# coralogix/arrow-ballista

Measured on AMD Instinct MI355X. Metric: tpch_sf100_q3_lineitem_rows_per_sec, higher is better.
Workload: dtype i128; 1 GPU; TPC-H SF100 q3 (BASELINE configs[2]): filter x3 + hash join customer|x|orders + hash join |x| lineitem + aggregate + sort, one task on 1 x MI355X; lineitem_rows=600037902, lineitem_rows_per_gpu=600037902, orders_rows_per_gpu=150009476, customer_rows_per_gpu=15000000, input=Arrow-physical columns resident in HBM, parallelism=single partition

## Files before the change

### arrow-ballista_amd/csrc/agg_compile.cpp

```cpp
#include "agg_compile.h"
#include <algorithm>
#include <cctype>
#include <cstdio>
#include <functional>

namespace gpuq {

gpuq_field_info make_field(const std::string& name, const DType& t, bool nullable) {
  gpuq_field_info f{};
  std::snprintf(f.name, sizeof(f.name), "%s", name.c_str());
  f.type = t.id; f.precision = t.p; f.scale = t.s; f.nullable = nullable;
  f.repr = (t.id == T_UTF8) ? GPUQ_REPR_PACKED15 : GPUQ_REPR_ARROW;
  f.width = (t.id == T_BOOL) ? 0 : type_width(t);
  return f;
}

KeySpec make_keyspec(const std::vector<int>& regs, const std::vector<DType>& types, bool null_word) {
  if (regs.size() > (size_t)MAX_KEYS) throw Unsupported("more than " + std::to_string(MAX_KEYS) + " key columns");
  KeySpec K{};
  K.n_keys = (int)regs.size(); K.null_word = null_word ? 1 : 0;
  int w = 0;
  for (size_t k = 0; k < regs.size(); ++k) {
    K.key_reg[k] = regs[k];
    const bool wide = types[k].id == T_DECIMAL128 || types[k].id == T_UTF8;
// ... 325 lines not shown
  {{"AVG"},                                     parts<Avg>(),         1,    false,  false,     false},
  {{"MIN"},                                     parts<MinMax>(),      1,    true,   false,     false},
  {{"MAX"},                                     parts<MinMax>(),      1,    false,  false,     false},
  {{"VARIANCE", "VAR", "VAR_SAMP"},             parts<Variance>(),    1,    false,  false,     false},
  {{"VARIANCE_POP", "VAR_POP"},                 parts<Variance>(),    1,    false,  true,      false},
  {{"STDDEV", "STDDEV_SAMP"},                   parts<Variance>(),    1,    false,  false,     true},
  {{"STDDEV_POP"},                              parts<Variance>(),    1,    false,  true,      true},
  {{"COVARIANCE", "COVAR", "COVAR_SAMP"},       parts<Covariance>(),  2,    false,  false,     false},
  {{"COVARIANCE_POP", "COVAR_POP"},             parts<Covariance>(),  2,    false,  true,      false},
  {{"CORRELATION", "CORR"},                     parts<Correlation>(), 2,    false,  false,     false},
};
const AggFn* find_agg_fn(const std::string& upper_name) {
  for (const AggFn& f : AGG_FNS) for (const char* n : f.names) if (upper_name == n) return &f;
  return nullptr;
}

}

AggCompiled compile_aggregate(const Schema& in, const Json& d) {
  AggCompiled R;
  R.mode = d.get_str("mode", "Single");
  const bool is_final = (R.mode == "Final" || R.mode == "FinalPartitioned");
  const bool emit_state = (R.mode == "Partial");
  if (!is_final && !emit_state && R.mode != "Single") throw std::runtime_error("unknown aggregate mode '" + R.mode + "'");
  R.strategy = d.get_str("strategy", "auto");
  R.expected_groups = d.get_i64("expected_groups", 0);
  Scan s(in);
  ExprCompiler& ec = s.ec;
  if (d.has("predicate")) ec.add_predicate(ec.from_json(d.at("predicate")));
  std::vector<NodeP> declared; std::vector<std::string> declared_names;
  if (d.has("group_expr")) for (const Json& g : d.at("group_expr").a) {
    declared.push_back(ec.from_json(g.at("expr"))); declared_names.push_back(g.get_str("name", "group" + std::to_string(declared.size() - 1)));
  }
  const GroupKeys keys(ec, declared, declared_names);
  R.refuse = keys.refuse;
  s.ungrouped = keys.nodes.empty();
  States states{ec, keys.declared(), in.fields.size()};
  std::vector<AggPlan> plans;
  for (const Json& a : d.at("aggr_expr").a) {
    s.fn = a.at("fn").str(); s.desc = &a;
    AggPlan pl; pl.name = a.get_str("name", s.fn);
    for (auto& ch : s.fn) ch = (char)std::toupper(ch);
    if (a.get_bool("distinct", false)) throw Unsupported("DISTINCT aggregates are not supported on device");
    pl.fn = find_agg_fn(s.fn);
    if (!is_final) {
      NodeP arg = a.has("expr") ? ec.from_json(a.at("expr")) : nullptr;
      if (a.has("filter") && !a.at("filter").is_null()) {
        NodeP p = ec.from_json(a.at("filter"));
        if (p->type.id != T_BOOL) throw std::runtime_error("aggregate FILTER must be boolean");
        if (!arg) arg = ec.lit_int(I64, 1);
        arg = ec.select(p, arg, ec.lit_null(arg->type));
        if (a.has("expr2")) throw Unsupported("FILTER on a two-argument aggregate");
      }
      if (!arg && !(pl.fn && pl.fn->args == 0)) throw std::runtime_error(s.fn + " needs an argument");
      if (!pl.fn) throw Unsupported("aggregate function " + s.fn);
      pl.fn->parts.from_args(s, pl, arg);
    } else {
      if (!pl.fn) throw Unsupported("aggregate function " + s.fn);
      pl.fn->parts.from_states(s, pl, states);
    }
    plans.push_back(pl);
  }
  std::vector<AccDef>& accs = s.accs;
  if (accs.empty()) s.count(nullptr);
  std::vector<int> key_slots, acc_slots(accs.size(), -1);
  for (auto& k : keys.nodes) key_slots.push_back(ec.add_output(k));
  for (size_t i = 0; i < accs.size(); ++i) if (accs[i].arg) acc_slots[i] = ec.add_output(accs[i].arg);
  R.prog = ec.finish();
  const int nk = (int)keys.nodes.size();
  R.agg.n_keys = nk; R.agg.n_accs = (int)accs.size();
  std::vector<int> kregs; bool any_null_key = false;
  for (int k = 0; k < nk; ++k) {
    const NodeP& n = keys.nodes[k];
    R.agg.key_reg[k] = R.prog.out_reg[key_slots[k]]; kregs.push_back(R.agg.key_reg[k]);
    R.key_types.push_back(n->type); any_null_key = any_null_key || n->nullable;
    if (n->type.id == T_BOOL || n->type.id == T_NULL) throw Unsupported("group-by key of type " + n->type.to_string());
  }
  for (size_t i = 0; i < accs.size(); ++i) {
    R.agg.acc_kind[i] = accs[i].kind; R.agg.acc_reg[i] = accs[i].arg ? R.prog.out_reg[acc_slots[i]] : 0;
    R.acc_types.push_back(accs[i].type);
    R.acc_bits.push_back(accs[i].arg ? R.prog.out_bits[acc_slots[i]] : 1);
  }
  R.keys = make_keyspec(kregs, R.key_types, any_null_key);

  for (int k = 0; k < nk; ++k) { Field f; f.name = keys.names[k]; f.type = keys.nodes[k]->type; f.nullable = keys.nodes[k]->nullable; f.raw128 = 1; R.post_schema.fields.push_back(f); }
  for (size_t i = 0; i < accs.size(); ++i) { Field f; f.name = "acc" + std::to_string(i); f.type = accs[i].type; f.nullable = false; f.raw128 = 1; R.post_schema.fields.push_back(f); }
  std::function<void(size_t, size_t, bool)> emit = [&](size_t lo, size_t hi, bool with_keys) {
    ExprCompiler pc(R.post_schema);
    std::vector<std::string> names; CompiledProgram cp;
    try {
      if (with_keys) keys.project(pc, names);
      Post p{pc, nk, accs, names};
      for (size_t pi = lo; pi < hi; ++pi) (emit_state ? plans[pi].fn->parts.states : plans[pi].fn->parts.value)(p, plans[pi]);
      cp = pc.finish();
    }
    catch (const Unsupported&) { throw; }
    catch (const std::runtime_error&) {
      if (hi - lo + (with_keys ? 1 : 0) <= 1) throw;
      if (with_keys && hi > lo) { emit(lo, lo, true); emit(lo, hi, false); }
      else { const size_t mid = lo + (hi - lo) / 2; emit(lo, mid, with_keys); emit(mid, hi, false); }
      return;
    }
    if (cp.out_reg.empty()) return;
    const int first_out = (int)R.out_fields.size();
    for (size_t i = 0; i < cp.out_type.size(); ++i) R.out_fields.push_back(make_field(names[i], cp.out_type[i], cp.out_nullable[i]));
    R.posts.push_back({std::move(cp), first_out});
  };
  emit(0, plans.size(), true);
  return R;
}

}
```

### arrow-ballista_amd/csrc/capi.cpp

```cpp
#include "../../include/gpuq.h"
#include "expr_compile.h"
#include "agg_compile.h"
#include "gpuq_kernels.h"
#include "jit_runtime.h"
#include "devbuf.h"
#include "gpuq_internal.h"
#include <hip/hip_runtime.h>
#include <algorithm>
#include <memory>
#include <mutex>
#include <cctype>
#include <cstdio>
#include <cstdlib>
#include <cstring>
#include <string>
#include <tuple>
#include <map>
#include <deque>
#include <functional>
#include <vector>

using namespace gpuq;

namespace {
// ... 316 lines not shown
      op->kind = K_SORT;
      ExprCompiler ec(op->in_schema);
      const auto& es = d.at("expr").a;
      if (es.empty() || es.size() > (size_t)MAX_SORT_KEYS) throw Unsupported("sort needs 1.." + std::to_string(MAX_SORT_KEYS) + " keys");
      std::vector<NodeP> ks;
      for (const Json& e : es) { NodeP n = ec.from_json(e.at("expr")); ks.push_back(n); ec.add_output(n); }
      op->prog = ec.finish(); upload_code(op->prog, op->code_dev);
      op->sort.n_keys = (int)ks.size();
      for (size_t k = 0; k < ks.size(); ++k) {
        const bool asc = es[k].get_bool("asc", true);
        op->sort.reg[k] = op->prog.out_reg[k]; op->sort.desc[k] = asc ? 0 : 1;
        op->sort.nulls_first[k] = es[k].get_bool("nulls_first", !asc) ? 1 : 0;
        op->sort.kind[k] = ks[k]->type.is_float() ? 1 : (ks[k]->type.id == T_UTF8 ? 2 : 0);
      }
      op->sort_key0 = ks[0]->type;
      op->fetch = d.get_i64("fetch", -1);
    } else if (kind == "partition") {
      op->kind = K_PARTITION;
      ExprCompiler ec(op->in_schema);
      std::vector<NodeP> ks;
      for (const Json& e : d.at("hash_expr").a) { NodeP n = ec.from_json(e); ks.push_back(n); ec.add_output(n); }
      if (ks.empty()) throw std::runtime_error("partition needs at least one hash expression");
      op->prog = ec.finish(); upload_code(op->prog, op->code_dev);
      std::vector<int> regs; for (size_t k = 0; k < ks.size(); ++k) { regs.push_back(op->prog.out_reg[k]); op->key_types.push_back(ks[k]->type); }
      op->keys = make_keyspec(regs, op->key_types, false);
      const i64 np = d.at("partition_count").i64();
      if (np < 1 || np > 65536) throw std::runtime_error("partition_count out of range (1..65536)");
      op->nparts = (uint32_t)np;
    } else throw std::runtime_error("unknown op '" + kind + "'");
}

int gpuq_op_create(gpuq_ctx* ctx, const char* json, gpuq_op** out) {
  gpuq_op* op = nullptr;
  int rc = guarded(ctx, [&]() {
    check_ctx(ctx);
    if (!json || !out) throw std::runtime_error("json/out is NULL");
    Json d = JsonParser(json).parse();
    op = new gpuq_op(); op->ctx = ctx;
    op->flags_dev.ensure(256); HIPCHECK(hipMemset(op->flags_dev.p, 0, 256));
    g_upload = true;
    compile_op(op, d);
    *out = op;
  });
  if (rc != GPUQ_OK) { delete op; if (out) *out = nullptr; }
  return rc;
}

static const char* op_name(int op) {
  static const char* n[] = {"NOP","IMM","MOV","ADD","SUB","MUL","MULW","NEG","DIV","MOD","EQ","NE","LT","LE","GT","GE","FADD","FSUB","FMUL","FDIV","FNEG","FSQRT",
    "FEQ","FNE","FLT","FLE","FGT","FGE","I2F","F2I","AND","OR","NOT","ISNULL","ISNOTNULL","SELECT","SHL","BOR","NULLIF0","COALESCE0"};
  return (op >= 0 && op < (int)(sizeof(n) / sizeof(n[0]))) ? n[op] : "?";
}
static std::string describe_program(const CompiledProgram& p, const Schema& sc) {
  std::string r = "{\"columns\":[";
  for (size_t i = 0; i < p.col_field.size(); ++i) { if (i) r += ","; r += "\"" + sc.fields[p.col_field[i]].name + "\""; }
  r += "],\"pred_reg\":" + std::to_string(p.pred_reg) + ",\"insns\":[";
  for (int i = 0; i < p.n_insns; ++i) {
    const DevInsn& in = p.code.insns[i];
    if (i) r += ",";
    r += std::string("\"") + op_name(in.op) + " r" + std::to_string(in.dst) + " r" + std::to_string(in.a) + " r" + std::to_string(in.b) + " #" + std::to_string(in.imm) + "\"";
  }
  r += "],\"out_reg\":[";
  for (size_t i = 0; i < p.out_reg.size(); ++i) { if (i) r += ","; r += std::to_string(p.out_reg[i]); }
  r += "],\"out_type\":[";
  for (size_t i = 0; i < p.out_type.size(); ++i) { if (i) r += ","; r += "\"" + p.out_type[i].to_string() + "\""; }
  return r + "]}";
}

int gpuq_compile_check(const char* json, char* buf, size_t cap) {
  gpuq_op* op = nullptr;
  int rc = guarded(nullptr, [&]() {
    if (!json) throw std::runtime_error("json is NULL");
    Json d = JsonParser(json).parse();
    op = new gpuq_op();
    g_upload = false;
    compile_op(op, d);
    g_upload = true;
    std::string r = "{\"program\":" + describe_program(op->prog, op->in_schema);
    if (op->kind == K_AGG) {
      r += ",\"post\":" + describe_program(op->posts.front().prog, op->post_schema) + ",\"post_programs\":" + std::to_string(op->posts.size()) + ",\"posts\":[";
      for (size_t i = 0; i < op->posts.size(); ++i) { if (i) r += ","; r += describe_program(op->posts[i].prog, op->post_schema); }
      r += "],\"acc_kinds\":[";
      for (int a = 0; a < op->agg.n_accs; ++a) { if (a) r += ","; r += std::to_string(op->agg.acc_kind[a]); }
      r += "]";
    }
    r += ",\"outputs\":[";
    for (size_t i = 0; i < op->out_fields.size(); ++i) {
      const gpuq_field_info& f = op->out_fields[i];
      if (i) r += ",";
      DType t; t.id = f.type; t.p = f.precision; t.s = f.scale;
      r += std::string("{\"name\":\"") + f.name + "\",\"type\":\"" + t.to_string() + "\",\"nullable\":" + (f.nullable ? "true" : "false") + "}";
    }
    r += "]}";
    if (buf && cap) { std::snprintf(buf, cap, "%s", r.c_str()); if (r.size() + 1 > cap) throw Capacity("describe buffer too small"); }
  });
  g_upload = true;
  delete op;
  return rc;
}
int gpuq_compile_jit_source(const char* json, int kernel_id, char* buf, size_t cap) {
  gpuq_op* op = nullptr;
  int rc = guarded(nullptr, [&]() {
    if (!json) throw std::runtime_error("json is NULL");
    Json d = JsonParser(json).parse();
    op = new gpuq_op();
    g_upload = false;
    compile_op(op, d);
    g_upload = true;
    std::string eval = op->prog.jit_src;
    if (kernel_id == GPUQ_SINK_AGG_TINY && op->kind == K_AGG) eval += agg_tiny_spec(op, (int)d.get_i64("jit_gmax", 4));
    const std::string src = jit_full_source(eval, kernel_id);
    if (src.size() + 1 > cap) throw Capacity("source needs " + std::to_string(src.size() + 1) + " bytes");
    std::memcpy(buf, src.c_str(), src.size() + 1);
  });
  g_upload = true;
  delete op;
  return rc;
}
void gpuq_op_free(gpuq_op* op) { delete op; }
int gpuq_op_num_outputs(gpuq_op* op) { return op ? (int)op->out_fields.size() : 0; }
int gpuq_op_output_field(gpuq_op* op, int i, gpuq_field_info* out) {
  if (!op || !out || i < 0 || i >= (int)op->out_fields.size()) return GPUQ_ERR_INVALID;
  *out = op->out_fields[i]; return GPUQ_OK;
}
int gpuq_op_check(gpuq_op* op, void* stream) {
  if (!op) return GPUQ_ERR_INVALID;
  return guarded(op->ctx, [&]() { check_ctx(op->ctx); const uint32_t f = read_flags(op, use_stream(stream)); if (f) { reset_flags(op, use_stream(stream)); raise_flags(f); } });
}
int gpuq_op_set_deferred(gpuq_op* op, int on) { if (!op) return GPUQ_ERR_INVALID; op->deferred = on != 0; op->defer_client = true; return GPUQ_OK; }
int gpuq_op_can_defer(gpuq_op* op) {
  if (!op) return 0;
  switch (op->kind) {
    case K_FILTER: case K_PROJECT: case K_JOIN_PROBE: return 1;
    case K_JOIN_BUILD: return op->learned.jb.valid ? 1 : 0;
    case K_AGG: return op->learned.ag.valid ? 1 : 0;
    case K_SORT: return op->learned.so.valid ? 1 : 0;
    default: return 0;
  }
}
int gpuq_ops_settle(gpuq_ctx* ctx, void* stream, gpuq_op* const* ops, int n_ops, const uint64_t* const* words, int n_words, uint64_t* words_out) {
  return guarded(ctx, [&]() {
    check_ctx(ctx);
    if (n_ops < 0 || n_words < 0 || (n_ops && !ops) || (n_words && (!words || !words_out))) throw std::runtime_error("settle: bad arguments");
    hipStream_t s = use_stream(stream);
    const int total = n_ops + n_words;
    struct Blocks { u64* host = nullptr; DevBuf dev; size_t cap = 0; };
    thread_local Blocks B;
    if ((size_t)total > B.cap) {
      if (B.host) (void)hipHostFree(B.host);
      B.cap = (size_t)std::max(total, 256); B.host = nullptr;
      HIPCHECK(hipHostMalloc((void**)&B.host, B.cap * 8, hipHostMallocDefault));
    }
    u64* dev = (u64*)B.dev.ensure(B.cap * 8);
    for (int base = 0; base < total; base += 64) {
      GatherWords g{}; g.n = std::min(64, total - base);
      for (int i = 0; i < g.n; ++i) { const int k = base + i; g.src[i] = k < n_ops ? (const u64*)ops[k]->flags_dev.p : (const u64*)words[k - n_ops]; if (!g.src[i]) throw std::runtime_error("settle: NULL word"); }
      launch_gather_words(s, g, dev + base);
    }
    HIPCHECK(hipGetLastError());
    if (total > 0) HIPCHECK(hipMemcpyAsync(B.host, dev, (size_t)total * 8, hipMemcpyDeviceToHost, s));
    HIPCHECK(hipStreamSynchronize(s));
    for (int i = 0; i < n_words; ++i) words_out[i] = B.host[n_ops + i];
    bool retry = false;
    for (int i = 0; i < n_ops; ++i) {
      const uint32_t f = (uint32_t)B.host[i];
      if (f) reset_flags(ops[i], s);
      static const bool trace = getenv("GPUQ_TRACE_DEFER") != nullptr;
      const uint32_t expected = ops[i]->learned.expect_flags;
      if (trace && (f & ~expected)) fprintf(stderr, "[gpuq] settle: operator %d of %d (kind %d) raised status 0x%x (expected 0x%x)\n", i, n_ops, (int)ops[i]->kind, f, expected);
      if (f & ~expected) { retry = true; ops[i]->learned.forget(); }
    }
    if (retry) throw Retry("an assumption of a deferred run did not hold");
  });
}
int gpuq_op_profile(gpuq_op* op, int enable, float* kernel_ms_out, int* launches_out) {
  if (!op) return GPUQ_ERR_INVALID;
  return guarded(op->ctx, [&]() {
    if (op->ev_pending) { float ms = 0; HIPCHECK(hipEventSynchronize(op->ev1)); HIPCHECK(hipEventElapsedTime(&ms, op->ev0, op->ev1)); op->kernel_ms += ms; op->ev_pending = false; }
    if (op->ev_total_pending) { float ms = 0; HIPCHECK(hipEventSynchronize(op->ev3)); HIPCHECK(hipEventElapsedTime(&ms, op->ev2, op->ev3)); op->total_ms += ms; op->ev_total_pending = false; }
    if (kernel_ms_out) *kernel_ms_out = op->kernel_ms;
    if (launches_out) *launches_out = op->launches;
    op->last_total_ms = op->total_ms;
    op->kernel_ms = 0; op->total_ms = 0; op->launches = 0; if (enable >= 0) op->profile = enable != 0;
  });
}
int gpuq_op_profile_total(gpuq_op* op, float* total_ms_out) {
  if (!op || !total_ms_out) return GPUQ_ERR_INVALID;
  *total_ms_out = op->last_total_ms;
  return GPUQ_OK;
}

int gpuq_filter_run(gpuq_op* op, void* stream, const gpuq_input* in, int payload_via, uint32_t* sel_out, uint64_t* count_out) {
  if (!op) return GPUQ_ERR_INVALID;
  return guarded(op->ctx, [&]() {
    check_ctx(op->ctx);
    if (op->kind != K_FILTER) throw std::runtime_error("not a filter operator");
    hipStream_t s = use_stream(stream);
    ProfTotal ptot(op, s);
    DevProgram P = bind_program(op->prog, op->in_schema, op->code_dev.as<DevCode>(), op->flags_dev.as<uint32_t>(), in);
    if (payload_via < 0 || payload_via > in->n_via) throw std::runtime_error("payload_via out of range");
    const i64 n = in->n_rows;
    if (n == 0) { if (count_out) HIPCHECK(hipMemsetAsync(count_out, 0, 8, s)); return; }
    const i64 nwords = (n + 63) >> 6;
    const i64 maxb = (i64)op->ctx->cus * 8;
    i64 wpb = (nwords + maxb - 1) / maxb; if (wpb < 16) wpb = 16;
    const int nblocks = (int)((nwords + wpb - 1) / wpb);
    u64* bitmap = (u64*)op->ws[0].ensure((size_t)nwords * 8);
    uint32_t* counts = (uint32_t*)op->ws[1].ensure((size_t)nblocks * 4 + 16);
    u64* total = count_out ? (u64*)count_out : (u64*)op->ws[2].ensure(8);
    { SinkJit jit(op, op->prog, GPUQ_SINK_FILTER_BITMAP, n); ProfScope ps(op, s); launch_filter_bitmap(s, jit.fn, P, n, bitmap, counts, nblocks, wpb); }
    launch_scan_block_counts(s, counts, nblocks, total);
    if (sel_out) launch_compact(s, bitmap, counts, nblocks, wpb, n, payload_via > 0 ? in->via[payload_via - 1] : nullptr, sel_out);
    HIPCHECK(hipGetLastError());
  });
}

int gpuq_project_run(gpuq_op* op, void* stream, const gpuq_input* in, gpuq_column* outs, int n_outs) {
  if (!op) return GPUQ_ERR_INVALID;
  return guarded(op->ctx, [&]() {
    check_ctx(op->ctx);
    if (op->kind != K_PROJECT) throw std::runtime_error("not a project operator");
    hipStream_t s = use_stream(stream);
    ProfTotal ptot(op, s);
    DevProgram P = bind_program(op->prog, op->in_schema, op->code_dev.as<DevCode>(), op->flags_dev.as<uint32_t>(), in);
    OutSpec O = make_outspec(op->prog, outs, n_outs, op->out_fields);
    for (int i = 0; i < n_outs; ++i) outs[i].length = in->n_rows;
    { SinkJit jit(op, op->prog, GPUQ_SINK_PROJECT, in->n_rows); ProfScope ps(op, s); launch_project(s, jit.fn, P, in->n_rows, O); }
    HIPCHECK(hipGetLastError());
    if (op->prog.checks_overflow && !op->deferred) { const uint32_t f = read_flags(op, s); if (f) { reset_flags(op, s); raise_flags(f); } }
  });
}

static u64 agg_slot_pct(const bool from_last_run) {
  static const long env = []() { const char* e = std::getenv("GPUQ_AGG_SLOT_PCT"); const long x = e ? std::atol(e) : 0; return (x >= 110 && x <= 800) ? x : 0; }();
  return env ? (u64)env : (from_last_run ? 130u : 200u);
}
static int aggregate_run_impl(gpuq_op* op, void* stream, const gpuq_input* in, gpuq_column* outs, int n_outs, int64_t cap, int64_t* n_groups_out, const uint64_t** ndev_out) {
  if (!op) return GPUQ_ERR_INVALID;
  if (ndev_out) *ndev_out = nullptr;
  return guarded(op->ctx, [&]() {
    check_ctx(op->ctx);
    if (op->kind != K_AGG) throw std::runtime_error("not an aggregate operator");
    if (!op->refuse.empty()) throw Unsupported(op->refuse);
    hipStream_t s = use_stream(stream);
    ProfTotal ptot(op, s);
    DevProgram P = bind_program(op->prog, op->in_schema, op->code_dev.as<DevCode>(), op->flags_dev.as<uint32_t>(), in);
    const i64 n = in->n_rows;
    const int nk = op->agg.n_keys, na = op->agg.n_accs, kstride = nk > 0 ? nk : 1;
    uint32_t ng = 0;
    AggOut raw{};
    auto alloc_raw = [&](i64 rcap) {
      raw.cap = (int32_t)rcap;
      raw.keys = (u64*)op->ws[0].ensure((size_t)rcap * kstride * 16);
      raw.key_nulls = (uint32_t*)op->ws[1].ensure((size_t)rcap * 4);
      raw.cells = (u64*)op->ws[2].ensure((size_t)rcap * na * 16);
      raw.n_groups = op->flags_dev.as<uint32_t>() + 2;
      HIPCHECK(hipMemsetAsync(raw.n_groups, 0, 8, s));
    };
    auto read_ng = [&]() { uint32_t v[3] = {0, 0, 0}; read_status(op, s, v, 3); return v[2]; };
    if (n_outs != (int)op->out_fields.size()) throw std::runtime_error("expected " + std::to_string(op->out_fields.size()) + " output columns, got " + std::to_string(n_outs));
    bool posted = false;
    auto run_post = [&](uint32_t rows, const uint32_t* rows_dev) {
      const size_t colbytes = (size_t)std::max<uint32_t>(rows, 1) * 16, vbytes = ((size_t)rows + 63) / 64 * 8 + 8;
      char* soa_mem = (char*)op->ws[6].ensure((size_t)(nk + na) * colbytes + (size_t)nk * vbytes);
      AggSoA soa{};
      std::vector<gpuq_column> pcols(nk + na);
      for (int k = 0; k < nk; ++k) {
        soa.key_col[k] = (ulonglong2*)(soa_mem + (size_t)k * colbytes);
        soa.key_valid[k] = (u64*)(soa_mem + (size_t)(nk + na) * colbytes + (size_t)k * vbytes);
        const DType& t = op->key_types[k];
        pcols[k] = gpuq_column{t.id, t.p, t.s, 0, soa.key_col[k], nullptr, op->post_schema.fields[k].nullable ? (const uint8_t*)soa.key_valid[k] : nullptr, (int64_t)rows};
      }
      for (int a = 0; a < na; ++a) {
        soa.acc_col[a] = (ulonglong2*)(soa_mem + (size_t)(nk + a) * colbytes);
        const DType& t = op->acc_types[a];
        pcols[nk + a] = gpuq_column{t.id, t.p, t.s, 0, soa.acc_col[a], nullptr, nullptr, (int64_t)rows};
      }
      launch_agg_emit(s, raw, nk, na, rows, soa, rows_dev);
      gpuq_input pin{}; pin.cols = pcols.data(); pin.n_cols = nk + na; pin.n_rows = rows; pin.n_via = 0;
      for (auto& pc : op->posts) {
        DevProgram PP = bind_program(pc.prog, op->post_schema, pc.code.as<DevCode>(), op->flags_dev.as<uint32_t>(), &pin);
        PP.n_dev = (const u64*)rows_dev;
        const int no = (int)pc.prog.out_reg.size();
        std::vector<gpuq_field_info> fi(op->out_fields.begin() + pc.first_out, op->out_fields.begin() + pc.first_out + no);
        OutSpec O = make_outspec(pc.prog, outs + pc.first_out, no, fi);
        { SinkJit jit(op, pc.prog, GPUQ_SINK_PROJECT, rows); launch_project(s, jit.fn, PP, rows, O); }
      }
    };
    auto launch_tiny = [&](const int gmax, const bool reset) {
      int nb = 0; const size_t wsb = agg_tiny_workspace_bytes(gmax, nk, na, &nb);
      void* wsp = op->ws[4].ensure(wsb);
      alloc_raw(64);
      if (reset) reset_flags(op, s);
      const std::string spec = agg_tiny_spec(op, gmax);
      { SinkJit jit(op, op->prog, GPUQ_SINK_AGG_TINY, n, spec); ProfScope ps(op, s); launch_agg_tiny(s, jit.fn, P, n, op->agg, gmax, wsp); }
      launch_agg_tiny_merge(s, P, n, op->agg, gmax, wsp, raw);
    };
    HashTable T{};
    T.key_words = op->keys.key_words; T.slot_words = 1 + T.key_words + 2 * na;
    auto launch_table = [&](const u64 est, const u64 slot_pct, const bool use_lds, const bool reset) {
      T.n_slots = next_pow2(est * slot_pct / 100);
      T.slots = (u64*)op->ws[5].ensure((size_t)T.n_slots * T.slot_words * 8);
      launch_ht_init(s, T, &op->agg);
      if (reset) reset_flags(op, s);
      if (use_lds) {
        int n_fsum = 0; for (int a = 0; a < na; ++a) n_fsum += op->agg.acc_kind[a] == ACC_FSUM;
        u64* fstage = nullptr;
        const size_t fbytes = (size_t)T.n_slots * (size_t)n_fsum * (size_t)agg_lds_grid(n) * 8;
        if (n_fsum > 0 && fbytes <= ((size_t)256 << 20)) { fstage = (u64*)op->ws[8].ensure(fbytes); HIPCHECK(hipMemsetAsync(fstage, 0, fbytes, s)); }
        SinkJit jit(op, op->prog, GPUQ_SINK_AGG_LDS, n); ProfScope ps(op, s); launch_agg_lds(s, jit.fn, P, n, op->keys, op->agg, T, fstage, n_fsum);
      }
      else { SinkJit jit(op, op->prog, GPUQ_SINK_AGG_HASH, n); ProfScope ps(op, s); launch_agg_hash(s, jit.fn, P, n, op->keys, op->agg, T); }
    };
    auto run_radix = [&](const std::string& strat, const i64 known_groups) -> bool {
      const int slot_words = 1 + op->keys.key_words + 2 * na;
      uint32_t capslots = 64; while ((size_t)capslots * 2 * slot_words * 8 <= 60 * 1024) capslots *= 2;
      if ((size_t)capslots * slot_words * 8 <= 60 * 1024 && n < (1ll << 31)) {
        const u64 est = op->expected_groups > 0 ? (u64)op->expected_groups : (known_groups > 0 ? (u64)known_groups + (u64)known_groups / 4 : (u64)n);
        const u64 per_bucket = std::max<u64>(1, (u64)capslots / 2);
        u64 nbk = next_pow2(std::max<u64>(1, (est + per_bucket - 1) / per_bucket)); if (nbk > (1ull << 24)) nbk = 1ull << 24;
        if (n >= (1ll << 20) && nbk < 2048) nbk = 2048;
        int bits = 0; while ((1ull << bits) < nbk) ++bits;
        DevBuf b_bid, b_bid2, b_ids, b_hist, b_look, b_bounds;
        u64* bid = (u64*)b_bid.ensure((size_t)n * 8); u64* bid2 = (u64*)b_bid2.ensure((size_t)n * 8);
        uint32_t* ids = (uint32_t*)b_ids.ensure((size_t)n * 4 + 16);
        u64* ghist = (u64*)b_hist.ensure((size_t)sort_max_passes() * 256 * 8);
        const size_t lwb = onesweep_ws_bytes(n);
        void* lws = b_look.ensure(lwb);
        uint32_t* bounds = (uint32_t*)b_bounds.ensure((size_t)(nbk + 2) * 4);
        reset_flags(op, s);
        { SinkJit jit(op, op->prog, GPUQ_SINK_AGG_BUCKET_ID, n); launch_agg_bucket_id(s, jit.fn, P, n, op->keys, nbk - 1, bid, nullptr); }
        const int npass = std::max(1, (bits + 7) / 8);
        launch_radix_ghist(s, bid, n, 32, npass, ghist);
        for (int p = 0; p < npass; ++p) {
          launch_onesweep_pass(s, bid, nullptr, n, 32 + 8 * p, ghist + (size_t)p * 256, lws, lwb, bid2, ids, p + 1 == npass ? 2 : 0);
          std::swap(bid, bid2);
        }
        launch_bucket_bounds(s, bid, n, nbk, bounds, 32);
        alloc_raw((i64)std::min<u64>((u64)std::max<i64>(n, 1), std::max<u64>(est + est / 4, 1ull << 20)));
        { SinkJit jit(op, op->prog, GPUQ_SINK_AGG_BUCKET, n); ProfScope ps(op, s); launch_agg_bucket(s, jit.fn, P, op->keys, op->agg, ids, bounds, (uint32_t)nbk, capslots, slot_words, raw); }
        HIPCHECK(hipGetLastError());
        uint32_t fw[4] = {0, 0, 0, 0};
        read_status(op, s, fw, 4);
        if (fw[0] & ~(FLAG_TABLE_FULL | FLAG_GROUP_OVERFLOW)) { reset_flags(op, s); raise_flags(fw[0] & ~(FLAG_TABLE_FULL | FLAG_GROUP_OVERFLOW)); }
        if (!(fw[0] & (FLAG_TABLE_FULL | FLAG_GROUP_OVERFLOW))) { ng = fw[2]; return true; }
        if (strat == "radix" && op->expected_groups > 0 && est < (u64)n) throw Capacity("radix aggregate: a bucket overflowed; raise expected_groups or use strategy hash/auto");
        reset_flags(op, s);
      } else if (strat == "radix") throw Unsupported("radix aggregate: the group state does not fit an LDS table");
      return false;
    };
    auto finish_on_device = [&]() {
      run_post((uint32_t)raw.cap, raw.n_groups);
      HIPCHECK(hipGetLastError());
      for (int i = 0; i < n_outs; ++i) outs[i].length = raw.cap;
      if (n_groups_out) *n_groups_out = raw.cap;
      *ndev_out = (const uint64_t*)raw.n_groups;
    };
    auto& L = op->learned;
    if (ndev_out && op->deferred && L.ag.valid) {
      if (L.ag.path == 1) {
        if (cap >= 64) { launch_tiny(L.ag.gmax, false); finish_on_device(); return; }
      } else if (L.ag.path == 2) {
        const u64 est = std::min<u64>(std::max<u64>(L.ag.est, 64), (u64)(L.ag.groups + L.ag.groups / 4 + 64));
        const i64 rcap = std::min<i64>(L.ag.groups + L.ag.groups / 4 + 1024, cap);
        if (rcap >= 1 && rcap <= 0x7FFFFFFFll) {
          launch_table(est, agg_slot_pct(true), L.ag.use_lds, false);
          alloc_raw(rcap);
          launch_agg_hash_extract(s, op->keys, op->agg, T, raw, op->flags_dev.as<uint32_t>());
          finish_on_device();
          return;
        }
      }
    }
    if (in->n_rows_dev) throw std::runtime_error("aggregate: a device-side row count needs a deferred operator with a completed synchronous run (gpuq_op_can_defer)");
    L.ag.valid = false;
    int path_done = 0, gmax_done = 0; u64 est_done = 0; bool lds_done = false;
    bool done = false;
    std::string strat = op->strategy;
    if (nk == 0) strat = "tiny";
    if (strat == "auto" && n <= 16384) strat = "hash";
    i64 known_groups = op->expected_groups > 0 ? op->expected_groups : L.ag.groups;
    bool many_groups = false;
    if (strat == "auto" && nk > 0 && known_groups < 0 && n >= (1ll << 20)) {
      const i64 nsample = 1ll << 20, stride = std::max<i64>(1, n / nsample);
      const u64 nbits = 1ull << 24;
      uint32_t* bm = (uint32_t*)op->ws[7].ensure(nbits / 8 + 64);
      unsigned long long* cnt = (unsigned long long*)((char*)bm + nbits / 8);
      HIPCHECK(hipMemsetAsync(bm, 0, nbits / 8 + 64, s));
      launch_key_sample(s, P, n, op->keys, stride, nsample, bm, nbits, cnt + 1);
      launch_popcount_bits(s, (const uint8_t*)bm, (i64)nbits, cnt);
      unsigned long long* pd = (unsigned long long*)op->pinned();
      unsigned long long host2[2] = {0, 0};
      unsigned long long* dst = pd ? pd : host2;
      HIPCHECK(hipMemcpyAsync(dst, cnt, 16, hipMemcpyDeviceToHost, s));
      HIPCHECK(hipStreamSynchronize(s));
      const i64 distinct = (i64)dst[0], passed = (i64)dst[1];
      if (passed >= 4096) {
        if (distinct * 4 <= passed) known_groups = std::max<i64>(1, distinct);
        else many_groups = true;
      }
    }
    if (strat == "auto" && nk > 0 && (many_groups || known_groups > (i64)agg_tiny_max_groups(na))) {
    } else if (strat == "auto" || strat == "tiny") {
      const int fit_big = agg_tiny_max_groups(na);
      if (fit_big < 1) { if (strat == "tiny") throw Unsupported("too many accumulators for the LDS aggregate"); }
      else {
        int fit_small = 0; for (int g = 1; g <= fit_big; ++g) { int nb; (void)nb; if ((size_t)g * na * 2048 + 4096 <= 64 * 1024) fit_small = g; }
        std::vector<int> tries;
        if (nk == 0) tries = {1};
        else { if (fit_small > 4) { tries.push_back(4); } if (fit_small >= 2) tries.push_back(fit_small); if (fit_big > fit_small) tries.push_back(fit_big); }
        if (nk > 0 && known_groups > 0) while (tries.size() > 1 && (i64)tries.front() < known_groups) tries.erase(tries.begin());
        for (int gmax : tries) {
          launch_tiny(gmax, true);
          HIPCHECK(hipGetLastError());
          const bool ahead = (i64)raw.cap <= cap;
          if (ahead) run_post((uint32_t)raw.cap, raw.n_groups);
          uint32_t fw[4] = {0, 0, 0, 0};
          read_status(op, s, fw, 4);
          const uint32_t f = fw[0];
          if (f & ~FLAG_GROUP_OVERFLOW) { reset_flags(op, s); raise_flags(f & ~FLAG_GROUP_OVERFLOW); }
          if (!(f & FLAG_GROUP_OVERFLOW)) { ng = fw[2]; done = true; posted = ahead; path_done = 1; gmax_done = gmax; break; }
        }
        if (!done && strat == "tiny") throw Capacity("more groups than the LDS aggregate holds; use strategy hash/auto");
      }
    }
    const bool remembered_hash = op->expected_groups <= 0 && L.ag.path == 2;
    if (!done && (strat == "radix" || (strat == "auto" && !remembered_hash && ((n >= (1ll << 22) && op->expected_groups >= (1ll << 20)) ||
                                                            (n >= (1ll << 20) && known_groups >= 4096))))) { done = run_radix(strat, known_groups); if (done) path_done = 3; }
    if (!done) {
      const i64 known = known_groups >= 0 ? (op->expected_groups > 0 ? known_groups : std::max<i64>(known_groups + known_groups / 4, 64)) : -1;
      u64 est = known > 0 ? (u64)std::min<i64>(known, std::max<i64>(n, 1)) : (u64)std::min<i64>(std::max<i64>(n, 1), 1ll << 24);
      if (est < 64) est = 64;
      const uint32_t lslots = agg_lds_slots(T);
      const bool use_lds = strat == "lds" || (strat == "auto" && lslots > 0 && n >= (1ll << 17) && known > 0 && known <= (i64)lslots * 4);
      if (strat == "lds" && !lslots) throw Unsupported("lds aggregate: the group state does not fit an LDS table");
      for (;;) {
        launch_table(est, agg_slot_pct(known_groups >= 0 && op->expected_groups <= 0 && est == (u64)known), use_lds, true);
        HIPCHECK(hipGetLastError());
        const uint32_t f = (n <= (1ll << 20) && est >= (u64)n) ? 0u : read_flags(op, s);
        if (f & FLAG_TABLE_FULL) { if (est >= (u64)std::max<i64>(n, 1024)) throw std::runtime_error("hash aggregate: table full at maximum size"); est = std::min<u64>(est * 4, (u64)std::max<i64>(n, 1024)); continue; }
        if (f) { reset_flags(op, s); raise_flags(f); }
        break;
      }
      path_done = 2; est_done = est; lds_done = use_lds;
      if (n <= (1ll << 20)) {
        alloc_raw(std::max<i64>(n, 1));
        launch_agg_hash_extract(s, op->keys, op->agg, T, raw, op->flags_dev.as<uint32_t>());
        HIPCHECK(hipGetLastError());
        const bool ahead = (i64)raw.cap <= cap;
        if (ahead) run_post((uint32_t)raw.cap, raw.n_groups);
        uint32_t fw[4] = {0, 0, 0, 0};
        read_status(op, s, fw, 4);
        if (fw[0]) { reset_flags(op, s); raise_flags(fw[0]); }
        ng = fw[2];
        posted = ahead;
      } else {
        bool done = false;
        if (L.ag.groups > 0) {
          alloc_raw(L.ag.groups + L.ag.groups / 4 + 1024);
          launch_agg_hash_extract(s, op->keys, op->agg, T, raw, op->flags_dev.as<uint32_t>());
          HIPCHECK(hipGetLastError());
          uint32_t fw[4] = {0, 0, 0, 0};
          read_status(op, s, fw, 4);
          ng = fw[2];
          if (fw[0] & ~FLAG_GROUP_OVERFLOW) { reset_flags(op, s); raise_flags(fw[0]); }
          done = !(fw[0] & FLAG_GROUP_OVERFLOW);
          if (!done) { reset_flags(op, s); HIPCHECK(hipMemsetAsync(raw.n_groups, 0, 4, s)); }
        } else {
          alloc_raw(1);
          raw.cap = 0;
          launch_agg_hash_extract(s, op->keys, op->agg, T, raw, op->flags_dev.as<uint32_t>());
          ng = read_ng();
          reset_flags(op, s);
        }
        if (!done) {
          alloc_raw(std::max<i64>(ng, 1));
          launch_agg_hash_extract(s, op->keys, op->agg, T, raw, op->flags_dev.as<uint32_t>());
          HIPCHECK(hipGetLastError());
          ng = read_ng();
        }
      }
    }
    L.ag = {path_done == 1 || path_done == 2, path_done, gmax_done, est_done, lds_done, (i64)ng};
    if (L.ag.valid) L.expect_flags = 0;
    if (n_groups_out) *n_groups_out = ng;
    if ((i64)ng > cap) throw Capacity("aggregate produced " + std::to_string(ng) + " groups, output capacity is " + std::to_string(cap));
    for (int i = 0; i < n_outs; ++i) outs[i].length = ng;
    if (!posted) {
      run_post(ng, nullptr);
      HIPCHECK(hipGetLastError());
      HIPCHECK(hipStreamSynchronize(s));
    }
  });
}

int gpuq_aggregate_run(gpuq_op* op, void* stream, const gpuq_input* in, gpuq_column* outs, int n_outs, int64_t cap, int64_t* n_groups_out) {
  return aggregate_run_impl(op, stream, in, outs, n_outs, cap, n_groups_out, nullptr);
}
int gpuq_aggregate_run_deferred(gpuq_op* op, void* stream, const gpuq_input* in, gpuq_column* outs, int n_outs, int64_t cap, int64_t* n_bound_out, const uint64_t** n_groups_dev_out) {
  if (!n_groups_dev_out) return GPUQ_ERR_INVALID;
  return aggregate_run_impl(op, stream, in, outs, n_outs, cap, n_bound_out, n_groups_dev_out);
}

namespace {
bool probe_keys_local(gpuq_op* op, hipStream_t s, const DevProgram& P, i64 n, const HashTable& T) {
  u64* c = (u64*)op->ws[7].ensure(32);
  HIPCHECK(hipMemsetAsync(c, 0, 16, s));
  const i64 nwords = (n + 63) >> 6;
  const i64 nsample = std::min<i64>(nwords, 4096);
  launch_join_locality(s, P, n, op->keys, T, nwords / nsample, nsample, c);
  HIPCHECK(hipGetLastError());
  u64 got[2] = {0, 0};
  HIPCHECK(hipMemcpyAsync(got, c, 16, hipMemcpyDeviceToHost, s));
  HIPCHECK(hipStreamSynchronize(s));
  return got[0] == 0 || got[1] * 2 >= got[0];
}
}
static int join_build_impl(gpuq_op* op, void* stream, const gpuq_input* in, int payload_via, int64_t build_rows_bound, gpuq_join_table* semi_table,
                           uint32_t* semi_hits_out, uint64_t* rows_out, gpuq_join_table** out) {
  if (!op) return GPUQ_ERR_INVALID;
  gpuq_join_table* t = nullptr;
  int rc = guarded(op->ctx, [&]() {
    check_ctx(op->ctx);
    if (op->kind != K_JOIN_BUILD) throw std::runtime_error("not a join_build operator");
    if (!out) throw std::runtime_error("out is NULL");
    hipStream_t s = use_stream(stream);
    ProfTotal ptot(op, s);
    SemiProbe semi{}; const SemiProbe* semi_p = nullptr;
    if (semi_table) {
      if (!op->has_semi) throw std::runtime_error("join build: the descriptor has no \"semi_on\" keys");
      if (semi_table->has_dups) throw std::runtime_error("join build: the semi table holds duplicate keys (a row could survive more than once)");
      if (op->semi_keys.n_keys != semi_table->keys.n_keys || op->semi_keys.key_words != semi_table->keys.key_words) throw std::runtime_error("semi keys do not match the semi table's keys (count / width)");
      for (int k = 0; k < op->semi_keys.n_keys; ++k) if (op->semi_keys.key_wide[k] != semi_table->keys.key_wide[k]) throw std::runtime_error("semi key " + std::to_string(k) + " width class differs from the table's key; cast one side");
      if (payload_via != 0) throw std::runtime_error("join build over a semi table: payload_via must be 0 (the build row is the position)");
      semi.T = semi_table->T; semi.K = op->semi_keys; semi.null_eq = semi_table->null_eq; semi.on = 1; semi.hit_out = semi_hits_out; semi.rows_out = (u64*)rows_out;
      semi_p = &semi;
    } else if (op->has_semi) throw std::runtime_error("join build: this operator was compiled with \"semi_on\" keys: call gpuq_join_build_run_semi");
    DevProgram P = bind_program(op->prog, op->in_schema, op->code_dev.as<DevCode>(), op->flags_dev.as<uint32_t>(), in);
    if (payload_via < 0 || payload_via > in->n_via) throw std::runtime_error("payload_via out of range");
    const i64 n = in->n_rows;
    if (build_rows_bound < n && payload_via == 0) build_rows_bound = n;
    if (build_rows_bound < 0 || build_rows_bound > 0xFFFFFFFEll) throw std::runtime_error("build_rows_bound out of range");
    t = new gpuq_join_table(); t->ctx = op->ctx; t->keys = op->keys; t->null_eq = op->null_eq; t->bound = build_rows_bound;
    t->T.key_words = op->keys.key_words; t->T.slot_words = 1 + t->T.key_words;
    static const bool spec_on = []() { const char* e = getenv("GPUQ_JOIN_SPECULATE"); return !(e && e[0] == '0'); }();
    const int dense_mode = op->ctx->join_dense; const i64 dense_ratio = op->ctx->join_dense_ratio;
    const bool narrow_key = dense_mode && n > 0 && op->keys.n_keys == 1 && !op->keys.key_wide[0] && !op->keys.null_word;
    auto semi_spec = [&](const HashTable& T2, const uint32_t* present_) -> std::string {
      if (!semi_p) return std::string();
      const KeySpec& A = op->semi_keys; const KeySpec& B = op->keys;
      const bool narrow = A.n_keys == 1 && A.key_words == 1 && !A.null_word && B.n_keys == 1 && B.key_words == 1 && !B.null_word;
      if (narrow && T2.dense && !present_ && payload_via == 0)
        return "#define GPUQ_JIT_SEMI 2\nconstexpr int JIT_KEY_REG0 = " + std::to_string(A.key_reg[0]) + ";\nconstexpr int JIT_KEY2_REG = " + std::to_string(B.key_reg[0]) + ";\n";
      return "#define GPUQ_JIT_SEMI 1\n";
    };
    auto attempt = [&](const int mode) -> bool {
    const bool guess = mode == 1, memo = mode == 2;
    auto& jb = op->learned.jb;
    bool dense = false, sparse_bits = false; i64 kmin = 0; u64 krange = 0;
    if (memo) { dense = jb.dense; sparse_bits = jb.sparse_bits; kmin = jb.kmin; krange = jb.krange; }
// ... 987 lines not shown
```

### arrow-ballista_amd/csrc/gpuq_kernels.h

```cpp
#pragma once
#include "gpuq_dev.h"
#ifndef GPUQ_JIT
#include <type_traits>
#include "devbuf.h"
#endif

namespace gpuq {

constexpr int MAX_OUTS = 16;
struct OutCol {
  void* data;
  u64* validity;
  int32_t reg;
  int32_t cls;
};
struct OutSpec { int32_t n_out; int32_t pad; OutCol cols[MAX_OUTS]; };

constexpr int MAX_ACCS = 12;
constexpr int MAX_KEYS = 4;
enum AccKind : int32_t { ACC_SUM = 0, ACC_COUNT = 1, ACC_COUNT_STAR = 2, ACC_MIN = 3, ACC_MAX = 4, ACC_FSUM = 5, ACC_FMIN = 6, ACC_FMAX = 7 };
struct AggSpec {
  int32_t n_keys, n_accs;
  int32_t key_reg[MAX_KEYS];
  int32_t acc_kind[MAX_ACCS];
  int32_t acc_reg[MAX_ACCS];
};

struct AggOut {
  u64* keys; uint32_t* key_nulls; u64* cells; uint32_t* n_groups; int32_t cap; int32_t pad;
};



constexpr int MAX_KW = 2 * MAX_KEYS + 1;
struct KeySpec {
  int32_t n_keys;
  int32_t key_reg[MAX_KEYS];
  int32_t key_wide[MAX_KEYS];
  int32_t null_word;
  int32_t key_words;
  int32_t word_reg[MAX_KW];
  int32_t word_half[MAX_KW];
};
struct HashTable {
  u64* slots;
  u64 n_slots;
  int32_t slot_words;
  int32_t key_words;
  uint32_t* dense;
  i64 dense_min;
  u64 dense_range;
  uint32_t* dense_bits;
};
struct SemiProbe { HashTable T; KeySpec K; int32_t null_eq; int32_t on; uint32_t* hit_out; u64* rows_out; };
enum JoinType : int32_t { JT_INNER = 0, JT_LEFT = 1, JT_RIGHT = 2, JT_FULL = 3, JT_LEFT_SEMI = 4, JT_LEFT_ANTI = 5, JT_RIGHT_SEMI = 6, JT_RIGHT_ANTI = 7 };


constexpr uint32_t NIL = 0xFFFFFFFFu;
__device__ __forceinline__ uint32_t tag_of(u64 h) { return (uint32_t)(h >> 32) | 2u; }

__device__ __forceinline__ u64 acc_identity(const int kind, const int half) {
  switch (kind) {
    case ACC_MIN: return half ? 0 : 0x7FFFFFFFFFFFFFFFull;
    case ACC_MAX: return half ? ~0ull : 0x8000000000000000ull;
    case ACC_FMIN: return half ? 0 : 0x7FF0000000000000ull;
    case ACC_FMAX: return half ? 0 : 0xFFF0000000000000ull;
    default: return 0;
  }
}
__device__ __forceinline__ u64 slot_word_identity(const AggSpec& A, const int w, const int cell0) {
  const int a = (w - cell0) >> 1;
  return (w >= cell0 && a < A.n_accs) ? acc_identity(A.acc_kind[a], (w - cell0) & 1) : 0;
}
__device__ __forceinline__ void lds_table_init(u64* slots, const uint32_t cap, const int slot_words, const int cell0, const AggSpec& A, const uint32_t nthreads) {
  for (uint32_t i = threadIdx.x; i < cap * (uint32_t)slot_words; i += nthreads) slots[i] = slot_word_identity(A, (int)(i % (uint32_t)slot_words), cell0);
}
__device__ __forceinline__ bool acc_operand(const AggSpec& A, const int a, GPUQ_REGS_CPARAM, u64& vlo, u64& vhi) {
  const int kind = A.acc_kind[a];
  vlo = 1; vhi = 0;
  if (kind == ACC_COUNT_STAR) return true;
  const int r = __builtin_amdgcn_readfirstlane(A.acc_reg[a]);
  if (kind != ACC_COUNT) { vlo = rlo[r]; vhi = rhi[r]; }
  return !((rnulls >> r) & 1);
}
__device__ __forceinline__ bool acc_wide_minmax(const int kind, const u64 vlo, const u64 vhi) {
  return (kind == ACC_MIN || kind == ACC_MAX) && (i64)vhi != ((i64)vlo >> 63);
}
__device__ __forceinline__ void acc_combine(const int kind, u64& lo, u64& hi, const u64 olo, const u64 ohi) {
  switch (kind) {
    case ACC_SUM: case ACC_COUNT: case ACC_COUNT_STAR: { const u64 s = lo + olo; hi = hi + ohi + (s < lo ? 1 : 0); lo = s; break; }
    case ACC_MIN: if ((i64)olo < (i64)lo) lo = olo; break;
    case ACC_MAX: if ((i64)olo > (i64)lo) lo = olo; break;
    case ACC_FSUM: lo = (u64)__double_as_longlong(__longlong_as_double((i64)lo) + __longlong_as_double((i64)olo)); break;
    case ACC_FMIN: if (f64_total_key(olo) < f64_total_key(lo)) lo = olo; break;
    case ACC_FMAX: if (f64_total_key(olo) > f64_total_key(lo)) lo = olo; break;
    default: break;
  }
}
template <int SCOPE>
__device__ __forceinline__ void acc_fold(u64* c, const int kind, const u64 vlo, const u64 vhi) {
  switch (kind) {
    case ACC_COUNT: case ACC_COUNT_STAR: if (vlo) __hip_atomic_fetch_add(c, vlo, __ATOMIC_RELAXED, SCOPE); break;
    case ACC_SUM: {
      if (!(vlo | vhi)) break;
      const u64 old = __hip_atomic_fetch_add(c, vlo, __ATOMIC_RELAXED, SCOPE);
      const u64 carry = (old + vlo < old) ? 1 : 0;
      if (vhi + carry) __hip_atomic_fetch_add(c + 1, vhi + carry, __ATOMIC_RELAXED, SCOPE);
      break;
    }
    case ACC_MIN: __hip_atomic_fetch_min((i64*)c, (i64)vlo, __ATOMIC_RELAXED, SCOPE); break;
    case ACC_MAX: __hip_atomic_fetch_max((i64*)c, (i64)vlo, __ATOMIC_RELAXED, SCOPE); break;
    case ACC_FSUM: unsafeAtomicAdd((double*)c, __longlong_as_double((i64)vlo)); break;
    case ACC_FMIN: case ACC_FMAX: {
      u64 cur = __hip_atomic_load(c, __ATOMIC_RELAXED, SCOPE);
      for (;;) {
        const bool better = (kind == ACC_FMIN) ? (f64_total_key(vlo) < f64_total_key(cur)) : (f64_total_key(vlo) > f64_total_key(cur));
        if (!better || __hip_atomic_compare_exchange_strong(c, &cur, vlo, __ATOMIC_RELAXED, __ATOMIC_RELAXED, SCOPE)) break;
      }
      break;
    }
    default: break;
  }
}
__device__ __forceinline__ u64 acc_result_hi(const int kind, const u64 lo, const u64 hi) {
  return (kind == ACC_MIN || kind == ACC_MAX) ? (u64)((i64)lo >> 63) : hi;
// ... 57 lines not shown
  int32_t n_keys;
  int32_t reg[MAX_SORT_KEYS];
  int32_t desc[MAX_SORT_KEYS];
  int32_t nulls_first[MAX_SORT_KEYS];
  int32_t kind[MAX_SORT_KEYS];
};
constexpr int SORT_MAX_PASSES = 16;
struct SortPack {
  u64 base_lo[MAX_SORT_KEYS], base_hi[MAX_SORT_KEYS];
  int32_t shift[MAX_SORT_KEYS];
  int32_t null_bit[MAX_SORT_KEYS];
  int32_t rshift[MAX_SORT_KEYS];
  int32_t vbits[MAX_SORT_KEYS];
  int32_t check;
  int32_t total_bits;
};

struct AggSoA {
  ulonglong2* key_col[MAX_KEYS]; u64* key_valid[MAX_KEYS];
  ulonglong2* acc_col[MAX_ACCS];
};



struct GatherWords { int32_t n; int32_t pad; const u64* src[64]; };

#define GPUQ_SINK_FILTER_BITMAP 1
#define GPUQ_SINK_PROJECT 2
#define GPUQ_SINK_AGG_TINY 3
#define GPUQ_SINK_AGG_HASH 4
#define GPUQ_SINK_JOIN_BUILD 5
#define GPUQ_SINK_JOIN_PROBE 6
#define GPUQ_SINK_JOIN_PROBE_UNIQUE 7
#define GPUQ_SINK_SORT_MINMAX 8
#define GPUQ_SINK_SORT_PACK 9
#define GPUQ_SINK_PART_PID 10
#define GPUQ_SINK_AGG_BUCKET_ID 11
#define GPUQ_SINK_AGG_BUCKET 12
#define GPUQ_SINK_AGG_LDS 13
#define GPUQ_SINK_JOIN_KEYRANGE 14
#define GPUQ_SINK_RJ_PACK 15

#ifndef GPUQ_JIT
struct SinkInfo { int id; const char* file; const char* entry; };
constexpr SinkInfo GPUQ_SINKS[] = {
    {GPUQ_SINK_FILTER_BITMAP, "kernels_scan.hip", "gpuq_jit_filter_bitmap"},
    {GPUQ_SINK_PROJECT, "kernels_scan.hip", "gpuq_jit_project"},
    {GPUQ_SINK_AGG_TINY, "kernels_scan.hip", "gpuq_jit_agg_tiny"},
    {GPUQ_SINK_AGG_HASH, "kernels_hash.hip", "gpuq_jit_agg_hash"},
    {GPUQ_SINK_JOIN_BUILD, "kernels_hash.hip", "gpuq_jit_join_build"},
    {GPUQ_SINK_JOIN_PROBE, "kernels_hash.hip", "gpuq_jit_join_probe"},
    {GPUQ_SINK_JOIN_PROBE_UNIQUE, "kernels_hash.hip", "gpuq_jit_join_probe_unique"},
    {GPUQ_SINK_SORT_MINMAX, "kernels_sort.hip", "gpuq_jit_sort_minmax"},
    {GPUQ_SINK_SORT_PACK, "kernels_sort.hip", "gpuq_jit_sort_pack"},
    {GPUQ_SINK_PART_PID, "kernels_sort.hip", "gpuq_jit_part_pid"},
    {GPUQ_SINK_AGG_BUCKET_ID, "kernels_hash.hip", "gpuq_jit_agg_bucket_id"},
    {GPUQ_SINK_AGG_BUCKET, "kernels_hash.hip", "gpuq_jit_agg_bucket"},
    {GPUQ_SINK_AGG_LDS, "kernels_hash.hip", "gpuq_jit_agg_lds"},
    {GPUQ_SINK_JOIN_KEYRANGE, "kernels_hash.hip", "gpuq_jit_join_keyrange"},
    {GPUQ_SINK_RJ_PACK, "kernels_hash.hip", "gpuq_jit_rj_pack"},
};
void launch_gather_words(hipStream_t s, const GatherWords& g, u64* out);
void set_num_cus(int n);
int num_cus();
void launch_filter_bitmap(hipStream_t s, void* jit_fn, const DevProgram& P, i64 n, u64* bitmap, uint32_t* block_counts, int nblocks, i64 words_per_block);
void launch_scan_block_counts(hipStream_t s, uint32_t* block_counts, int nblocks, u64* total_out);
void launch_compact(hipStream_t s, const u64* bitmap, const uint32_t* block_offsets, int nblocks, i64 words_per_block, i64 n,
                    const uint32_t* sel_in, uint32_t* sel_out);
void launch_project(hipStream_t s, void* jit_fn, const DevProgram& P, i64 n, const OutSpec& O);
int agg_tiny_max_groups(int n_accs);
size_t agg_tiny_workspace_bytes(int gmax, int n_keys, int n_accs, int* nblocks_out);
void launch_agg_tiny(hipStream_t s, void* jit_fn, const DevProgram& P, i64 n, const AggSpec& A, int gmax, void* workspace);
void launch_agg_tiny_merge(hipStream_t s, const DevProgram& P, i64 n, const AggSpec& A, int gmax, void* workspace, const AggOut& out);
void launch_ht_init(hipStream_t s, const HashTable& T, const AggSpec* A);
void launch_agg_hash(hipStream_t s, void* jit_fn, const DevProgram& P, i64 n, const KeySpec& K, const AggSpec& A, const HashTable& T);
void launch_key_sample(hipStream_t s, const DevProgram& P, i64 n, const KeySpec& K, i64 stride, i64 nsample, uint32_t* bitmap, u64 nbits, unsigned long long* passed);
uint32_t agg_lds_slots(const HashTable& T);
int agg_lds_grid(i64 n);
void launch_agg_lds(hipStream_t s, void* jit_fn, const DevProgram& P, i64 n, const KeySpec& K, const AggSpec& A, const HashTable& T, u64* fstage, int n_fsum);
void launch_agg_bucket_id(hipStream_t s, void* jit_fn, const DevProgram& P, i64 n, const KeySpec& K, u64 bucket_mask, u64* bid, uint32_t* ids);
void launch_bucket_bounds(hipStream_t s, const u64* sorted_bid, i64 n, u64 nbuckets, uint32_t* bounds, int shift);
void launch_agg_bucket(hipStream_t s, void* jit_fn, const DevProgram& P, const KeySpec& K, const AggSpec& A, const uint32_t* ids, const uint32_t* bounds, uint32_t nbuckets,
                       uint32_t cap, int slot_words, const AggOut& out);
void launch_agg_hash_extract(hipStream_t s, const KeySpec& K, const AggSpec& A, const HashTable& T, const AggOut& out, uint32_t* flags);
bool launch_join_build(hipStream_t s, void* jit_fn, const DevProgram& P, i64 n, const KeySpec& K, const HashTable& T, uint32_t* next, uint32_t* present,
                       int payload_via, int null_equals_null, const SemiProbe* semi = nullptr);
void launch_join_keyrange(hipStream_t s, void* jit_fn, const DevProgram& P, i64 n, const KeySpec& K, int null_equals_null, u64* out, i64 wstep = 1);
void launch_join_probe_unique(hipStream_t s, void* jit_fn, const DevProgram& P, i64 n, const KeySpec& K, const HashTable& T, int join_type, int null_equals_null, int payload_via,
                              uint32_t* seg_build, uint32_t* seg_probe, uint32_t* seg_counts, int nsegs, i64 wpw, uint32_t* visited);
void launch_copy_segments(hipStream_t s, const uint32_t* seg_build, const uint32_t* seg_probe, const uint32_t* seg_offsets, int nsegs, i64 wpw, i64 n,
                          const u64* total, uint32_t* out_build, uint32_t* out_probe, u64 out_cap, uint32_t* flags);
void launch_join_locality(hipStream_t s, const DevProgram& P, i64 n, const KeySpec& K, const HashTable& T, i64 stride, i64 nsample, u64* out);
struct RjGeomHost { uint32_t nparts, shift; i64 tile; int32_t nblocks; };
void rj_geometry(i64 n, u64 range, int slice_log2, RjGeomHost* g);
size_t rj_hist_entries(const RjGeomHost& g);
void launch_rj_partition(hipStream_t s, void* jit_fn, const DevProgram& P, i64 n, const KeySpec& K, const HashTable& T, int payload_via, const RjGeomHost& g,
                         u64* rec, u64* rec_out, int32_t* hist, void* scan_ws, size_t scan_ws_bytes);
int rj_probe_geometry(i64 n, i64* wpw_out);
void launch_rj_probe(hipStream_t s, const u64* rec, const int32_t* n_live, const HashTable& T, int join_type, uint32_t* seg_build, uint32_t* seg_probe,
                     uint32_t* seg_counts, int nblocks, i64 wpw);
void launch_bitmap_select(hipStream_t s, const u64* present, const u64* visited, int matched, i64 nwords, i64 n, u64* bitmap,
                          uint32_t* block_counts, int nblocks, i64 wpb);
void launch_join_probe(hipStream_t s, void* jit_fn, const DevProgram& P, i64 n, const KeySpec& K, const HashTable& T, const uint32_t* next,
                       int join_type, int payload_via, int null_equals_null, uint32_t* out_build, uint32_t* out_probe,
                       u64 out_cap, u64* out_count, uint32_t* visited);
int sort_minmax_blocks(i64 n);
void launch_sort_minmax(hipStream_t s, void* jit_fn, const DevProgram& P, i64 n, const SortSpec& S, u64* out, int nblocks, i64 wstep = 1);
int sort_max_passes();
void launch_sort_pack(hipStream_t s, void* jit_fn, const DevProgram& P, i64 n, const SortSpec& S, const SortPack& K, u64* key_lo, u64* key_hi, uint32_t* ids, u64* hist, int hist_passes);
void launch_part_pid(hipStream_t s, void* jit_fn, const DevProgram& P, i64 n, const KeySpec& K, uint32_t nparts, u64* pid_out, uint32_t* ids);
void launch_part_offsets(hipStream_t s, const u64* pid, i64 n, uint32_t nparts, uint32_t* counts_ws, u64* offsets_out, int shift);
void launch_counts_to_ghist(hipStream_t s, const uint32_t* counts, uint32_t np, u64* ghist);
void launch_gather_u64(hipStream_t s, const u64* src, const uint32_t* idx, i64 n, u64* dst);
int sort_small_max();
int sort_direct_max();
void launch_sort_direct(hipStream_t s, const DevProgram& P, i64 n, const SortSpec& S, uint32_t* perm);
void launch_sort_small(hipStream_t s, const u64* klo, const u64* khi, const uint32_t* ids, i64 n, uint32_t* out);
size_t onesweep_ws_bytes(i64 n);
int onesweep_max_passes();
size_t merge_splits_entries(i64 max_len, int n_pairs);
void launch_merge_pairs(hipStream_t s, const u64* klo, const u64* khi, const uint32_t* ids, const i64* pairs, int n_pairs, i64 max_len, i64* splits,
                        u64* klo_out, u64* khi_out, uint32_t* ids_out);
void launch_radix_ghist(hipStream_t s, const u64* keys, i64 n, int shift0, int npasses, u64* ghist);
void launch_onesweep_pass(hipStream_t s, const u64* keys, const uint32_t* vals, i64 n, int shift, u64* gexcl, void* ws, size_t ws_bytes,
                          u64* keys_out, uint32_t* vals_out, int ids_only );
void launch_agg_emit(hipStream_t s, const AggOut& raw, int n_keys, int n_accs, uint32_t n_groups, const AggSoA& soa, const uint32_t* n_groups_dev = nullptr);
void launch_concat_bitmap(hipStream_t s, u64* dst, i64 dst_bit_offset, const uint8_t* src, i64 src_bit_offset, i64 n_bits);
void launch_unpack_utf8_lengths(hipStream_t s, const ulonglong2* packed, i64 n, int32_t* lens_out, uint32_t* too_long);
constexpr int LIKE_MAX_TOKENS = 256;
constexpr int LIKE_MAX_SEGS = 8;
struct LikePattern {
  int32_t n; int32_t regex_mode; uint16_t tok[LIKE_MAX_TOKENS];
  int32_t n_seg, anchored_start, anchored_end, pad;
  int32_t seg_off[LIKE_MAX_SEGS], seg_len[LIKE_MAX_SEGS];
  unsigned long long seg_first8[LIKE_MAX_SEGS], seg_mask8[LIKE_MAX_SEGS];
};
void launch_like_utf8(hipStream_t s, const uint8_t* data, const int32_t* offsets, const uint8_t* validity, const uint32_t* idx, i64 n, const LikePattern& pat, int negated,
                      u64* bits_out, u64* valid_out);
void launch_mark_rows(hipStream_t s, const uint32_t* rows, i64 n, uint8_t* bitmap);
void launch_utf8_compare(hipStream_t s, const uint8_t* adata, const int32_t* aoffs, const uint8_t* avalid, const uint32_t* aidx, const uint8_t* bdata, const int32_t* boffs,
                         const uint8_t* bvalid, const uint32_t* bidx, int32_t blen, i64 n, int op, u64* bits_out, u64* valid_out);
void launch_sort_decode(hipStream_t s, const u64* recs, int rec_shift, i64 n, const SortPack& K, int desc, int nulls_first, int width, void* out, u64* valid_out);
void launch_cross_pairs(hipStream_t s, i64 n_left, i64 n_right, uint32_t* left_rows, uint32_t* right_rows);
void launch_offsets_rebase(hipStream_t s, const int32_t* src, i64 n, int32_t delta, int32_t* dst);
void launch_take_utf8_lengths(hipStream_t s, const int32_t* offsets, const uint8_t* validity, const uint32_t* idx, i64 n, int32_t* lens, u64* valid_out);
void launch_take_utf8_bytes(hipStream_t s, const uint8_t* data, const int32_t* offsets, const uint32_t* idx, i64 n, const int32_t* out_offsets, uint8_t* out, i64 total_bytes);
void launch_unpack_utf8_bytes(hipStream_t s, const ulonglong2* packed, i64 n, const int32_t* offsets, uint8_t* data_out);
void launch_exclusive_scan_i32(hipStream_t s, int32_t* data, i64 n, void* workspace, size_t ws_bytes);
size_t exclusive_scan_ws_bytes(i64 n);
struct Lz4Block { int64_t src; int64_t slot; int32_t len; int32_t pad; };
constexpr int LZ4_UNIT_BLOCK = 0, LZ4_UNIT_STORED = 1, LZ4_UNIT_FRAME_BLOCKS = 2;
constexpr int LZ4_UNIT_BLOCK_CHECKSUM = 1;
struct Lz4Unit { int64_t src, dst, src_len, dst_len; int32_t mode, flags; };
constexpr int64_t LZ4_BLOCK_BYTES = 65536;
inline int64_t lz4_slot_bytes(int64_t len) { return ((len + len / 255 + 16) + 15) & ~(int64_t)15; }
void launch_lz4_compress(hipStream_t s, const uint8_t* src, uint8_t* slots, const Lz4Block* blocks, int n_blocks, int32_t* csize);
void launch_lz4_layout(hipStream_t s, const Lz4Block* blocks, const int32_t* csize, const int32_t* buf_first_block, int n_buffers, int64_t* buf_off, int64_t* buf_len,
                       int64_t* blk_dst);
void launch_lz4_pack(hipStream_t s, const uint8_t* src, const uint8_t* slots, const Lz4Block* blocks, int n_blocks, const int32_t* csize, const int32_t* blk_buffer,
                     const int32_t* buf_first_block, const int64_t* buf_off, const int64_t* buf_len, const int64_t* blk_dst, uint8_t* body);
void launch_lz4_decode(hipStream_t s, const uint8_t* src, int64_t src_bytes, uint8_t* dst, const Lz4Unit* units, int n_units, uint32_t* status);
struct Utf8Piece { const int32_t* tmp; int64_t n; int32_t* dst; int64_t at, dl, start, used; int32_t first, pad; };
void launch_utf8_piece_starts(hipStream_t s, Utf8Piece* pieces, int n_pieces, uint32_t* gap);
void launch_utf8_piece_offsets(hipStream_t s, const Utf8Piece* pieces, int n_pieces, int64_t max_rows);
void launch_utf8_piece_validate(hipStream_t s, const Utf8Piece* pieces, int n_pieces, int64_t max_rows, uint32_t* status);
void launch_utf8_piece_compact(hipStream_t s, const Utf8Piece* pieces, int n_pieces, int64_t max_bytes, const uint8_t* from, uint8_t* to);
struct UnpackJob { int64_t src, dst, src_len, dst_len, raw_prefix; int32_t mode, pad; int64_t s_off, c_off, f_off, p_base; };
// ... 58 lines not shown
```

### arrow-ballista_amd/csrc/kernels_hash.hip

```cpp
#include "gpuq_kernels.h"

namespace gpuq {

constexpr int HBLOCK = 256;
constexpr int HWAVES = HBLOCK / 64;

__device__ __forceinline__ int hlane() { return threadIdx.x & 63; }
__device__ __forceinline__ int hwave() { return threadIdx.x >> 6; }

__device__ __forceinline__ u64 a_load(const u64* p) { return __hip_atomic_load(p, __ATOMIC_RELAXED, __HIP_MEMORY_SCOPE_AGENT); }
__device__ __forceinline__ void a_store(u64* p, u64 v) { __hip_atomic_store(p, v, __ATOMIC_RELAXED, __HIP_MEMORY_SCOPE_AGENT); }
__device__ __forceinline__ u64 a_cas(u64* p, u64 expected, u64 desired) {
  __hip_atomic_compare_exchange_strong(p, &expected, desired, __ATOMIC_RELAXED, __ATOMIC_RELAXED, __HIP_MEMORY_SCOPE_AGENT);
  return expected;
}
__device__ __forceinline__ u64 a_add(u64* p, u64 v) { return __hip_atomic_fetch_add(p, v, __ATOMIC_RELAXED, __HIP_MEMORY_SCOPE_AGENT); }

__device__ __forceinline__ bool make_key(const KeySpec& K, GPUQ_REGS_CPARAM, u64 (&kw)[MAX_KW], u64& hash) {
  uint32_t knull = 0;
  u64 h = 0x243F6A8885A308D3ull;
#pragma unroll
  for (int k = 0; k < MAX_KEYS; ++k) {
    if (k < K.n_keys) {
      const int r = __builtin_amdgcn_readfirstlane(K.key_reg[k]);
      const bool isn = (rnulls >> r) & 1;
      const u64 lo = isn ? 0 : rlo[r], hi = isn ? 0 : rhi[r];
      knull |= (uint32_t)isn << k;
      h = hash_combine(h, lo, K.key_wide[k] ? hi : 0, isn);
    }
  }
#pragma unroll
  for (int q = 0; q < MAX_KW; ++q) {
    kw[q] = 0;
    if (q < K.key_words) {
      const int half = __builtin_amdgcn_readfirstlane(K.word_half[q]);
      if (half == 2) kw[q] = knull;
      else {
        const int r = __builtin_amdgcn_readfirstlane(K.word_reg[q]);
        const bool isn = (rnulls >> r) & 1;
        const u64 vl = rlo[r], vh = rhi[r];
        const u64 v = (vl & ((u64)half - 1)) | (vh & (0 - (u64)half));
        kw[q] = isn ? 0 : v;
      }
    }
  }
  hash = h;
  return knull != 0;
}

__device__ __forceinline__ u64 ht_find_or_insert(const HashTable& T, const u64 (&kw)[MAX_KW], u64 h, uint32_t payload, bool& inserted) {
  const u64 mask = T.n_slots - 1;
  u64 s = h & mask;
  const uint32_t tag = tag_of(h);
  inserted = false;
  u64 probes = 0;
  while (probes < T.n_slots) {
    u64* slot = T.slots + s * (u64)T.slot_words;
    u64 w0 = a_load(slot);
    uint32_t st = (uint32_t)w0;
    if (st == 0u) {
      const u64 old = a_cas(slot, 0ull, 1ull);
      if (old == 0ull) {
#pragma unroll
        for (int q = 0; q < MAX_KW; ++q) if (q < T.key_words) a_store(slot + 1 + q, kw[q]);
        asm volatile("s_waitcnt vmcnt(0)" ::: "memory");
        a_store(slot, ((u64)payload << 32) | tag);
        inserted = true;
        return s;
      }
      st = (uint32_t)old;
    }
    if (st == 1u) { __builtin_amdgcn_s_sleep(1); continue; }
    if (st == tag) {
      bool eq = true;
#pragma unroll
      for (int q = 0; q < MAX_KW; ++q) if (q < T.key_words) eq = eq && (a_load(slot + 1 + q) == kw[q]);
      if (eq) return s;
    }
    s = (s + 1) & mask;
    ++probes;
  }
  return ~0ull;
}

__device__ __forceinline__ bool ht_find(const HashTable& T, const u64 (&kw)[MAX_KW], u64 h, uint32_t& payload) {
  const u64 mask = T.n_slots - 1;
  u64 s = h & mask;
  const uint32_t tag = tag_of(h);
  for (u64 probes = 0; probes < T.n_slots; ++probes) {
    const u64* slot = T.slots + s * (u64)T.slot_words;
    u64 w0, k0 = 0;
    if (T.slot_words == 2) { const ulonglong2 v = *(const ulonglong2*)slot; w0 = v.x; k0 = v.y; }
    else w0 = slot[0];
    const uint32_t st = (uint32_t)w0;
    if (st == 0u) return false;
    if (st == tag) {
      bool eq = true;
      if (T.slot_words == 2) eq = (k0 == kw[0]);
      else {
#pragma unroll
        for (int q = 0; q < MAX_KW; ++q) if (q < T.key_words) eq = eq && (slot[1 + q] == kw[q]);
      }
      if (eq) { payload = (uint32_t)(w0 >> 32); return true; }
    }
    s = (s + 1) & mask;
  }
  return false;
}

#ifndef GPUQ_JIT
__global__ void __launch_bounds__(HBLOCK) k_ht_init(const HashTable T, const AggSpec A, const int has_agg) {
  const u64 total = T.n_slots * (u64)T.slot_words;
  const int cell0 = 1 + T.key_words;
  for (u64 i = (u64)blockIdx.x * HBLOCK + threadIdx.x; i < total; i += (u64)gridDim.x * HBLOCK) {
    T.slots[i] = has_agg ? slot_word_identity(A, (int)(i % (u64)T.slot_words), cell0) : 0;
  }
}
#endif

#ifndef GPUQ_ROWS_U
#define GPUQ_ROWS_U 2
#endif
template <int MAXC, class Body>
__device__ __forceinline__ void for_rows_in_flight(const DevProgram& P, const i64 n, const i64 w_first, const i64 w_stride, Body body, const i64 w_end = -1) {
  const i64 nw_all = (n + 63) >> 6;
  const i64 nwords = (w_end >= 0 && w_end < nw_all) ? w_end : nw_all;
#ifdef GPUQ_JIT
  constexpr int U = GPUQ_ROWS_U;
  for (i64 w0 = w_first; w0 < nwords; w0 += w_stride * U) {
    JitPre jq[U]; JitRaw jw[U]; i64 posc[U]; bool ex[U];
#pragma unroll
    for (int u = 0; u < U; ++u) {
      const i64 w = w0 + (i64)u * w_stride;
      const i64 pos = (w << 6) + hlane();
      ex[u] = w < nwords && pos < n;
      posc[u] = ex[u] ? pos : n - 1;
      gpuq_jit_pre(P, posc[u], jq[u]);
    }
#pragma unroll
    for (int u = 0; u < U; ++u) gpuq_jit_load(P, posc[u], jq[u], jw[u]);
#pragma unroll
    for (int u = 0; u < U; ++u) {
      const i64 w = w0 + (i64)u * w_stride;
      if (w >= nwords) break;
      GPUQ_REGS_DECL;
      const bool pass = gpuq_jit_compute(P, posc[u], jw[u], GPUQ_REGS);
      body(w, (w << 6) + hlane(), ex[u] && pass, GPUQ_REGS);
    }
  }
#else
  for (i64 w = w_first; w < nwords; w += w_stride) {
    const i64 pos = (w << 6) + hlane();
    bool active = pos < n;
    GPUQ_REGS_DECL;
    if (active) active = GPUQ_EVAL(MAXC, P, pos);
    body(w, pos, active, GPUQ_REGS);
  }
#endif
}

template <int MAXC>
__device__ __forceinline__ void k_agg_hash_body(const DevProgram P, const i64 n_arg, const KeySpec K, const AggSpec A, const HashTable T) {
  const i64 n = rows_of(P, n_arg);
  const i64 nwords = (n + 63) >> 6;
  const int cell0 = 1 + T.key_words;
  bool combine = true;
  for (int a = 0; a < A.n_accs; ++a) combine = combine && A.acc_kind[a] != ACC_FMIN && A.acc_kind[a] != ACC_FMAX;
  const int lane = hlane();
  for_rows_in_flight<MAXC>(P, n, (i64)blockIdx.x * HWAVES + hwave(), (i64)gridDim.x * HWAVES, [&](const i64, const i64, const bool active, GPUQ_REGS_PARAM) {
    if (__ballot(active) == 0) return;
    u64 kw[MAX_KW]; u64 h = 0;
#pragma unroll
    for (int q = 0; q < MAX_KW; ++q) kw[q] = 0;
    if (active) make_key(K, GPUQ_REGS, kw, h);
    bool head = true;
    if (combine) {
      const int pa = __shfl_up((int)active, 1);
      const u64 ph = __shfl_up(h, 1);
      bool eq = (pa != 0) & (lane > 0) & (ph == h);
#pragma unroll
      for (int q = 0; q < MAX_KW; ++q) { const u64 pk = __shfl_up(kw[q], 1); if (q < T.key_words) eq = eq & (pk == kw[q]); }
      head = !(active & eq);
    }
    const int nh = __shfl_down((int)head, 1);
    const bool next_head = (lane == 63) | (nh != 0);
    const bool tail = active & next_head;
    u64 s = ~0ull;
    if (tail) {
      bool inserted;
      s = ht_find_or_insert(T, kw, h, 0u, inserted);
      if (s == ~0ull) atomicOr(P.flags, FLAG_TABLE_FULL);
    }
    u64* cells = T.slots + (s == ~0ull ? 0 : s) * (u64)T.slot_words + cell0;
    const bool upd = tail && s != ~0ull;
    for (int a = 0; a < A.n_accs; ++a) {
      const int kind = A.acc_kind[a];
      u64 vlo, vhi;
      bool any = acc_operand(A, a, GPUQ_REGS, vlo, vhi) && active;
      const bool wide = any && acc_wide_minmax(kind, vlo, vhi);
      if (__ballot(wide)) { if (wide) atomicOr(P.flags, FLAG_WIDE_MINMAX); continue; }
      if (!any) { vlo = acc_identity(kind, 0); vhi = acc_identity(kind, 1); }
      if (combine) {
        bool f = head;
#pragma unroll
        for (int off = 1; off < 64; off <<= 1) {
          const u64 ulo = __shfl_up(vlo, off), uhi = __shfl_up(vhi, off);
          const bool uf = __shfl_up((int)f, off) != 0, uany = __shfl_up((int)any, off) != 0;
          if (lane >= off && !f) {
            acc_combine(kind, vlo, vhi, ulo, uhi);
            any = any || uany;
            f = uf;
          }
        }
      }
      if (upd && any) acc_fold<__HIP_MEMORY_SCOPE_AGENT>(cells + 2 * a, kind, vlo, vhi);
    }
  });
}
#ifndef GPUQ_JIT
template <int MAXC>
__global__ void __launch_bounds__(HBLOCK) k_agg_hash(const DevProgram P, const i64 n, const KeySpec K, const AggSpec A, const HashTable T) { k_agg_hash_body<MAXC>(P, n, K, A, T); }
#elif GPUQ_JIT_KERNEL == GPUQ_SINK_AGG_HASH
extern "C" __global__ void __launch_bounds__(HBLOCK) gpuq_jit_entry(const DevProgram P, const i64 n, const KeySpec K, const AggSpec A, const HashTable T) { k_agg_hash_body<0>(P, n, K, A, T); }
#endif

#ifndef GPUQ_JIT
__global__ void __launch_bounds__(HBLOCK) k_agg_hash_extract(const KeySpec K, const AggSpec A, const HashTable T, const AggOut out,
                                                             uint32_t* __restrict__ flags) {
  constexpr int XSUB = 16;
  const int cell0 = 1 + T.key_words;
  const u64 chunk_slots = 64ull * XSUB;
  const u64 nchunks = (T.n_slots + chunk_slots - 1) / chunk_slots;
  const u64 wave0 = (u64)blockIdx.x * HWAVES + hwave(), nwaves = (u64)gridDim.x * HWAVES;
  const u64 ltmask = (1ull << hlane()) - 1;
  for (u64 c = wave0; c < nchunks; c += nwaves) {
    u64 masks[XSUB]; uint32_t total = 0;
#pragma unroll
    for (int j = 0; j < XSUB; ++j) {
      const u64 s = c * chunk_slots + (u64)j * 64 + hlane();
      const bool live = s < T.n_slots && ((uint32_t)T.slots[s * (u64)T.slot_words]) >= 2u;
      masks[j] = __ballot(live); total += (uint32_t)__popcll(masks[j]);
    }
    if (total == 0) continue;
    uint32_t base = 0;
    if (hlane() == 0) base = atomicAdd(out.n_groups, total);
    base = __shfl(base, 0);
    if (out.cap == 0) continue;
    if (base + total > (uint32_t)out.cap && hlane() == 0) atomicOr(flags, FLAG_GROUP_OVERFLOW);
#pragma unroll
    for (int j = 0; j < XSUB; ++j) {
      const u64 m = masks[j];
      if ((m >> hlane()) & 1) {
        const u64 s = c * chunk_slots + (u64)j * 64 + hlane();
        const u64* slot = T.slots + s * (u64)T.slot_words;
        const uint32_t g = base + (uint32_t)__popcll(m & ltmask);
        if (g < (uint32_t)out.cap) emit_group(slot, cell0, K, A, out, g);
      }
      base += (uint32_t)__popcll(m);
    }
  }
}
#endif

template <int MAXC>
__device__ __forceinline__ void k_agg_bucket_id_body(const DevProgram P, const i64 n_arg, const KeySpec K, const u64 bucket_mask,
                                                         u64* __restrict__ bid, uint32_t* __restrict__ ids) {
  const i64 n = rows_of(P, n_arg);
  const i64 nwords = (n + 63) >> 6;
  for (i64 w = (i64)blockIdx.x * HWAVES + hwave(); w < nwords; w += (i64)gridDim.x * HWAVES) {
    const i64 pos = (w << 6) + hlane();
    if (pos >= n) continue;
    GPUQ_REGS_DECL;
    const bool pass = GPUQ_EVAL(MAXC, P, pos);
    u64 kw[MAX_KW]; u64 h = 0;
#pragma unroll
    for (int q = 0; q < MAX_KW; ++q) kw[q] = 0;
    if (pass) make_key(K, GPUQ_REGS, kw, h);
    if (!ids) bid[pos] = ((h & bucket_mask) << 32) | (u64)(pass ? (uint32_t)pos : NIL);
    else { bid[pos] = h & bucket_mask; ids[pos] = pass ? (uint32_t)pos : NIL; }
  }
}
#ifndef GPUQ_JIT
template <int MAXC>
__global__ void __launch_bounds__(HBLOCK) k_agg_bucket_id(const DevProgram P, const i64 n, const KeySpec K, const u64 bucket_mask,
                                                          u64* __restrict__ bid, uint32_t* __restrict__ ids) { k_agg_bucket_id_body<MAXC>(P, n, K, bucket_mask, bid, ids); }
__global__ void __launch_bounds__(HBLOCK) k_bucket_bounds(const u64* __restrict__ sorted_bid, const i64 n, const u64 nbuckets, uint32_t* __restrict__ bounds, const int shift) {
  for (u64 b = (u64)blockIdx.x * HBLOCK + threadIdx.x; b <= nbuckets; b += (u64)gridDim.x * HBLOCK) {
    i64 lo = 0, hi = n;
    while (lo < hi) { const i64 mid = (lo + hi) >> 1; if ((sorted_bid[mid] >> shift) < b) lo = mid + 1; else hi = mid; }
    bounds[b] = (uint32_t)lo;
  }
}
#elif GPUQ_JIT_KERNEL == GPUQ_SINK_AGG_BUCKET_ID
extern "C" __global__ void __launch_bounds__(HBLOCK) gpuq_jit_entry(const DevProgram P, const i64 n, const KeySpec K, const u64 bucket_mask,
                                                          u64* __restrict__ bid, uint32_t* __restrict__ ids) { k_agg_bucket_id_body<0>(P, n, K, bucket_mask, bid, ids); }
#endif

#ifndef GPUQ_JIT
template <int MAXC>
__global__ void __launch_bounds__(HBLOCK) k_key_sample(const DevProgram P, const i64 n, const KeySpec K, const i64 stride, const i64 nsample,
                                                       unsigned int* __restrict__ bitmap, const u64 bit_mask, unsigned long long* __restrict__ passed) {
  __shared__ unsigned int block_passed;
  if (threadIdx.x == 0) block_passed = 0;
  __syncthreads();
  const i64 nwords = (nsample + 63) >> 6;
  for (i64 w = (i64)blockIdx.x * HWAVES + hwave(); w < nwords; w += (i64)gridDim.x * HWAVES) {
    const i64 i = (w << 6) + hlane();
    i64 pos = i * stride; if (pos >= n) pos = n - 1;
    bool active = i < nsample;
    GPUQ_REGS_DECL;
    if (active) active = GPUQ_EVAL(MAXC, P, pos);
    const u64 m = __ballot(active);
    if (m && hlane() == 0) atomicAdd(&block_passed, (unsigned int)__popcll(m));
    if (!active) continue;
    u64 kw[MAX_KW]; u64 h = 0;
#pragma unroll
    for (int q = 0; q < MAX_KW; ++q) kw[q] = 0;
    make_key(K, GPUQ_REGS, kw, h);
    const u64 bit = mix64(h) & bit_mask;
    const unsigned int want = 1u << (bit & 31);
    if (!(__hip_atomic_load(bitmap + (bit >> 5), __ATOMIC_RELAXED, __HIP_MEMORY_SCOPE_AGENT) & want)) atomicOr(bitmap + (bit >> 5), want);
  }
  __syncthreads();
  if (threadIdx.x == 0 && block_passed) atomicAdd(passed, (unsigned long long)block_passed);
}
#endif

constexpr uint32_t LDS_PROBES = 32;

template <int MAXC>
__device__ __forceinline__ void k_agg_lds_body(const DevProgram P, const i64 n_arg, const KeySpec K, const AggSpec A, const HashTable T, const uint32_t lcap,
                                               u64* __restrict__ fstage, const int n_fsum) {
  const i64 n = rows_of(P, n_arg);
  extern __shared__ __attribute__((aligned(16))) u64 lslots[];
  __shared__ uint32_t lfull;
  const int key_words = K.key_words;
  const int lw = T.slot_words + 1, lcell0 = 2 + key_words, gcell0 = 1 + key_words;
  lds_table_init(lslots, lcap, lw, lcell0, A, HBLOCK);
  if (threadIdx.x == 0) lfull = 0;
// ... 883 lines not shown
#pragma unroll
      for (int u = 0; u < U; ++u) { const u64 idx = r[u] >> 32; bw[u] = act[u] ? dbits[idx >> 5] : 0u; }
#pragma unroll
      for (int u = 0; u < U; ++u) { const u64 idx = r[u] >> 32; hit[u] = NIL; if (act[u] && ((bw[u] >> (idx & 31)) & 1u)) hit[u] = dense[idx]; }
    } else {
#pragma unroll
      for (int u = 0; u < U; ++u) { hit[u] = NIL; if (act[u]) hit[u] = dense[r[u] >> 32]; }
    }
#pragma unroll
    for (int u = 0; u < U; ++u) cnt += emit_pairs(act[u] && hit[u] != NIL, hit[u], (uint32_t)r[u], seg_base, cnt, join_type == JT_RIGHT_SEMI ? nullptr : seg_build, seg_probe);
  }
  if (hlane() == 0) seg_counts[seg] = cnt;
}
#endif

#ifndef GPUQ_JIT
template <int MAXC>
__global__ void __launch_bounds__(HBLOCK) k_join_locality(const DevProgram P, const i64 n, const KeySpec K, const HashTable T, const i64 stride, const i64 nsample,
                                                          u64* __restrict__ out) {
  const int kr = __builtin_amdgcn_readfirstlane(K.key_reg[0]);
  u64 pairs = 0, near = 0;
  for (i64 sidx = (i64)blockIdx.x * HWAVES + hwave(); sidx < nsample; sidx += (i64)gridDim.x * HWAVES) {
    const i64 pos = ((sidx * stride) << 6) + hlane();
    bool active = pos < n;
    GPUQ_REGS_DECL;
    if (active) active = GPUQ_EVAL(MAXC, P, pos);
    active = active && !((rnulls >> kr) & 1);
    const u64 idx = active ? rlo[kr] - (u64)T.dense_min : 0;
    active = active && idx < T.dense_range;
    const u64 nidx = __shfl_down(idx, 1);
    const int nact = __shfl_down((int)active, 1);
    const bool pair = active && nact && hlane() < 63;
    const u64 d = nidx > idx ? nidx - idx : idx - nidx;
    pairs += (u64)__popcll(__ballot(pair));
    near += (u64)__popcll(__ballot(pair && d < (1ull << 14)));
  }
  if (hlane() == 0 && pairs) { atomicAdd((unsigned long long*)out, (unsigned long long)pairs); atomicAdd((unsigned long long*)out + 1, (unsigned long long)near); }
}
#endif

#ifndef GPUQ_JIT
static int hgrid(i64 n, int blocks_per_cu) {
  const i64 nwords = (n + 63) >> 6;
  i64 need = (nwords + HWAVES - 1) / HWAVES;
  if (need < 1) need = 1;
  const i64 cap = (i64)num_cus() * blocks_per_cu;
  return (int)(need < cap ? need : cap);
}

void launch_ht_init(hipStream_t s, const HashTable& T, const AggSpec* A) {
  AggSpec dummy{};
  const u64 total = T.n_slots * (u64)T.slot_words;
  u64 need = (total + HBLOCK - 1) / HBLOCK;
  const u64 cap = (u64)num_cus() * 16;
  const int grid = (int)(need < cap ? (need ? need : 1) : cap);
  hipLaunchKernelGGL(k_ht_init, dim3(grid), dim3(HBLOCK), 0, s, T, A ? *A : dummy, A ? 1 : 0);
}
void launch_agg_hash(hipStream_t s, void* jit_fn, const DevProgram& P, i64 n, const KeySpec& K, const AggSpec& A, const HashTable& T) {
  if (n <= 0) return;
  launch_sink(jit_fn, P.n_cols, GPUQ_PICK(k_agg_hash), dim3(hgrid(n, 8)), dim3(HBLOCK), 0, s, P, n, K, A, T);
}
void launch_key_sample(hipStream_t s, const DevProgram& P, i64 n, const KeySpec& K, i64 stride, i64 nsample, uint32_t* bitmap, u64 nbits, unsigned long long* passed) {
  if (n <= 0 || nsample <= 0) return;
  launch_sink(nullptr, P.n_cols, GPUQ_PICK(k_key_sample), dim3(hgrid(nsample, 8)), dim3(HBLOCK), 0, s, P, n, K, stride, nsample, bitmap, nbits - 1, passed);
}
uint32_t agg_lds_slots(const HashTable& T) {
  const size_t bytes = (size_t)(T.slot_words + 1) * 8;
  uint32_t cap = 1; while ((size_t)cap * 2 * bytes <= 32768) cap *= 2;
  return cap >= 128 ? cap : 0;
}
int agg_lds_grid(i64 n) { return hgrid(n, 4); }
void launch_agg_lds(hipStream_t s, void* jit_fn, const DevProgram& P, i64 n, const KeySpec& K, const AggSpec& A, const HashTable& T, u64* fstage, int n_fsum) {
  if (n <= 0) return;
  const uint32_t lcap = agg_lds_slots(T);
  const size_t lds = (size_t)lcap * (T.slot_words + 1) * 8;
  const int grid = agg_lds_grid(n);
  launch_sink(jit_fn, P.n_cols, GPUQ_PICK(k_agg_lds), dim3(grid), dim3(HBLOCK), lds, s, P, n, K, A, T, lcap, fstage, n_fsum);
  if (fstage && n_fsum > 0) {
    const u64 items = T.n_slots * (u64)n_fsum;
    const u64 need = (items + HWAVES - 1) / HWAVES, cap = (u64)num_cus() * 8;
    hipLaunchKernelGGL(k_fsum_stage_reduce, dim3((unsigned)(need < cap ? (need ? need : 1) : cap)), dim3(HBLOCK), 0, s, T, A, (const u64*)fstage, n_fsum, (uint32_t)grid);
  }
}
void launch_agg_hash_extract(hipStream_t s, const KeySpec& K, const AggSpec& A, const HashTable& T, const AggOut& out, uint32_t* flags) {
  u64 need = (T.n_slots + (u64)HBLOCK * 16 - 1) / ((u64)HBLOCK * 16);
  const u64 cap = (u64)num_cus() * 16;
  const int grid = (int)(need < cap ? (need ? need : 1) : cap);
  hipLaunchKernelGGL(k_agg_hash_extract, dim3(grid), dim3(HBLOCK), 0, s, K, A, T, out, flags);
}
void launch_agg_bucket_id(hipStream_t s, void* jit_fn, const DevProgram& P, i64 n, const KeySpec& K, u64 bucket_mask, u64* bid, uint32_t* ids) {
  if (n <= 0) return;
  launch_sink(jit_fn, P.n_cols, GPUQ_PICK(k_agg_bucket_id), dim3(hgrid(n, 8)), dim3(HBLOCK), 0, s, P, n, K, bucket_mask, bid, ids);
}
void launch_bucket_bounds(hipStream_t s, const u64* sorted_bid, i64 n, u64 nbuckets, uint32_t* bounds, int shift) {
  const u64 need = (nbuckets + 1 + HBLOCK - 1) / HBLOCK;
  hipLaunchKernelGGL(k_bucket_bounds, dim3((unsigned)(need < 4096 ? need : 4096)), dim3(HBLOCK), 0, s, sorted_bid, n, nbuckets, bounds, shift);
}
void launch_agg_bucket(hipStream_t s, void* jit_fn, const DevProgram& P, const KeySpec& K, const AggSpec& A, const uint32_t* ids, const uint32_t* bounds, uint32_t nbuckets,
                       uint32_t cap, int slot_words, const AggOut& out) {
  const size_t lds = (size_t)cap * slot_words * 8;
  u64 grid = nbuckets; const u64 gcap = (u64)num_cus() * 8; if (grid > gcap) grid = gcap; if (grid < 1) grid = 1;
  launch_sink(jit_fn, P.n_cols, GPUQ_PICK(k_agg_bucket), dim3((unsigned)grid), dim3(HBLOCK), lds, s, P, K, A, ids, bounds, nbuckets, cap, slot_words, out);
}
bool launch_join_build(hipStream_t s, void* jit_fn, const DevProgram& P, i64 n, const KeySpec& K, const HashTable& T, uint32_t* next, uint32_t* present,
                       int payload_via, int null_equals_null, const SemiProbe* semi) {
  if (n <= 0) return true;
  SemiProbe S{}; if (semi) S = *semi;
  if (semi && !jit_fn && P.n_cols > 8) return false;
  const auto semi_pick = [](auto M) { return &k_join_build<(decltype(M)::value < 8 ? decltype(M)::value : 8), true>; };
  const auto plain_pick = [](auto M) { return &k_join_build<decltype(M)::value, false>; };
  const dim3 grid(hgrid(n, 8)), block(HBLOCK);
  if (semi) launch_sink(jit_fn, P.n_cols, semi_pick, grid, block, 0, s, P, n, K, T, next, present, payload_via, null_equals_null, S);
  else launch_sink(jit_fn, P.n_cols, plain_pick, grid, block, 0, s, P, n, K, T, next, present, payload_via, null_equals_null, S);
  return true;
}

#ifndef GPUQ_JIT
__global__ void __launch_bounds__(HBLOCK) k_bitmap_select(const u64* __restrict__ present, const u64* __restrict__ visited, const int matched,
                                                          const i64 nwords, const i64 n, u64* __restrict__ bitmap,
                                                          uint32_t* __restrict__ block_counts, const i64 wpb) {
  __shared__ uint32_t wc[HWAVES];
  const i64 w0 = (i64)blockIdx.x * wpb;
  i64 w1 = w0 + wpb; if (w1 > nwords) w1 = nwords;
  uint32_t cnt = 0;
  for (i64 w = w0 + threadIdx.x; w < w1; w += HBLOCK) {
    u64 m = present[w] & (matched ? visited[w] : ~visited[w]);
    if (w == nwords - 1 && (n & 63)) m &= (1ull << (n & 63)) - 1;
    bitmap[w] = m; cnt += (uint32_t)__popcll(m);
  }
  for (int off = 32; off > 0; off >>= 1) cnt += __shfl_xor(cnt, off);
  if (hlane() == 0) wc[hwave()] = cnt;
  __syncthreads();
  if (threadIdx.x == 0) { uint32_t t = 0; for (int k = 0; k < HWAVES; ++k) t += wc[k]; block_counts[blockIdx.x] = t; }
}
#endif
void launch_bitmap_select(hipStream_t s, const u64* present, const u64* visited, int matched, i64 nwords, i64 n, u64* bitmap,
                          uint32_t* block_counts, int nblocks, i64 wpb) {
  hipLaunchKernelGGL(k_bitmap_select, dim3(nblocks), dim3(HBLOCK), 0, s, present, visited, matched, nwords, n, bitmap, block_counts, wpb);
}
void launch_join_probe(hipStream_t s, void* jit_fn, const DevProgram& P, i64 n, const KeySpec& K, const HashTable& T, const uint32_t* next,
                       int join_type, int payload_via, int null_equals_null, uint32_t* out_build, uint32_t* out_probe,
                       u64 out_cap, u64* out_count, uint32_t* visited) {
  if (n <= 0) return;
  launch_sink(jit_fn, P.n_cols, GPUQ_PICK(k_join_probe), dim3(hgrid(n, 8)), dim3(HBLOCK), 0, s, P, n, K, T, next, join_type, payload_via, null_equals_null, out_build, out_probe,
              out_cap, out_count, visited);
}

void launch_join_keyrange(hipStream_t s, void* jit_fn, const DevProgram& P, i64 n, const KeySpec& K, int null_equals_null, u64* out, i64 wstep) {
  if (n <= 0) return;
  if (wstep < 1) wstep = 1;
  const int grid = hgrid((n + wstep - 1) / wstep, 8);
  launch_sink(jit_fn, P.n_cols, GPUQ_PICK(k_join_keyrange), dim3(grid), dim3(HBLOCK), 0, s, P, n, K, null_equals_null, out, wstep);
}
void launch_join_probe_unique(hipStream_t s, void* jit_fn, const DevProgram& P, i64 n, const KeySpec& K, const HashTable& T, int join_type, int null_equals_null, int payload_via,
                              uint32_t* seg_build, uint32_t* seg_probe, uint32_t* seg_counts, int nsegs, i64 wpw, uint32_t* visited) {
  const int nblocks = (nsegs + HWAVES - 1) / HWAVES;
  launch_sink(jit_fn, P.n_cols, GPUQ_PICK(k_join_probe_unique), dim3(nblocks), dim3(HBLOCK), 0, s, P, n, K, T, join_type, null_equals_null, payload_via, seg_build, seg_probe, seg_counts,
              nsegs, wpw, visited);
}
void launch_copy_segments(hipStream_t s, const uint32_t* seg_build, const uint32_t* seg_probe, const uint32_t* seg_offsets, int nsegs, i64 wpw, i64 n,
                          const u64* total, uint32_t* out_build, uint32_t* out_probe, u64 out_cap, uint32_t* flags) {
  (void)n;
  i64 need = ((i64)nsegs + HWAVES - 1) / HWAVES; const i64 cap = (i64)num_cus() * 8;
  hipLaunchKernelGGL(k_copy_segments, dim3((unsigned)(need < cap ? (need ? need : 1) : cap)), dim3(HBLOCK), 0, s, seg_build, seg_probe, seg_offsets, nsegs, wpw, total,
                     out_build, out_probe, out_cap, flags);
}

void launch_join_locality(hipStream_t s, const DevProgram& P, i64 n, const KeySpec& K, const HashTable& T, i64 stride, i64 nsample, u64* out) {
  if (n <= 0 || nsample <= 0) return;
  const int grid = (int)std::min<i64>((nsample + HWAVES - 1) / HWAVES, (i64)num_cus() * 4);
  launch_sink(nullptr, P.n_cols, GPUQ_PICK(k_join_locality), dim3(grid), dim3(HBLOCK), 0, s, P, n, K, T, stride < 1 ? 1 : stride, nsample, out);
// ... 36 lines not shown
```

### arrow-ballista_amd/csrc/plan_exec.cpp

```cpp
#include "../../include/gpuq.h"
#include "devbuf.h"
#include "expr_compile.h"
#include "json.h"
#include <algorithm>
#include <atomic>
#include <thread>
#include <cerrno>
#include <chrono>
#include <random>
#include <sys/stat.h>
#include <functional>
#include <cstdio>
#include <cstring>
#include <map>
#include <memory>
#include <set>
#include <string>
#include <vector>

using namespace gpuq;

namespace {

constexpr uint32_t NULL_ROW_ID = 0xFFFFFFFFu;
typedef std::shared_ptr<DevBuf> BufP;

Json jstr(const std::string& s) { Json j; j.kind = Json::STR; j.s = s; return j; }
Json jnum(long long v) { Json j; j.kind = Json::NUM; j.s = std::to_string(v); return j; }
Json jbool(bool b) { Json j; j.kind = Json::BOOL; j.b = b; return j; }
Json jarr(std::vector<Json> a = {}) { Json j; j.kind = Json::ARR; j.a = std::move(a); return j; }
Json jobj(std::vector<std::pair<std::string, Json>> o = {}) { Json j; j.kind = Json::OBJ; j.o = std::move(o); return j; }
Json jcol(const std::string& name, int index) { return jobj({{"column", jobj({{"name", jstr(name)}, {"index", jnum(index)}})}}); }
Json jand(const Json& l, const Json& r) { return jobj({{"binary_expr", jobj({{"l", l}, {"r", r}, {"op", jstr("AND")}})}}); }

struct PField { std::string name; Json type; bool nullable = true; };
typedef std::vector<PField> PSchema;

int type_id_of(const Json& t, int& p, int& s) { DType d = dtype_from_json(t); p = d.p; s = d.s; return d.id; }
Json type_json_of(int tid, int p, int s) {
  switch (tid) {
    case T_BOOL: return jstr("Boolean"); case T_INT32: return jstr("Int32"); case T_INT64: return jstr("Int64"); case T_DATE32: return jstr("Date32");
    case T_FLOAT64: return jstr("Float64"); case T_UTF8: return jstr("Utf8"); case T_UINT32: return jstr("UInt32"); case T_UINT64: return jstr("UInt64");
    case T_INT8: return jstr("Int8"); case T_INT16: return jstr("Int16"); case T_UINT8: return jstr("UInt8"); case T_UINT16: return jstr("UInt16");
    case T_FLOAT32: return jstr("Float32"); case T_DATE64: return jstr("Date64");
    case T_DECIMAL128: return jobj({{"Decimal128", jarr({jnum(p), jnum(s)})}});
    case T_TIMESTAMP: { static const char* u[4] = {"Second", "Millisecond", "Microsecond", "Nanosecond"}; return jobj({{"Timestamp", jarr({jstr(u[p & 3]), Json()})}}); }
  }
  throw std::runtime_error("plan: type id " + std::to_string(tid) + " has no name");
}

struct PCol { std::string name; Json type; bool nullable = true; gpuq_column c{}; };
struct PTable {
  std::vector<PCol> cols; int64_t n = 0;
  std::vector<const uint32_t*> via; std::vector<int> sides; bool dense = false;
  std::vector<BufP> keep;
  int64_t record_cap = 0;
  const uint64_t* n_dev = nullptr; BufP n_keep;
  bool is_view() const { return !via.empty(); }
  void own(const PTable& o) { keep.insert(keep.end(), o.keep.begin(), o.keep.end()); }
  void count_from(const PTable& o) { n_dev = o.n_dev; n_keep = o.n_keep; }
};

Json table_fields(const PTable& t) {
  Json f = jarr();
  for (size_t i = 0; i < t.cols.size(); ++i) {
    const PCol& c = t.cols[i];
    std::vector<std::pair<std::string, Json>> o = {{"name", jstr(c.name)}, {"type", c.type}, {"nullable", jbool(c.nullable)}, {"side", jnum(t.sides[i])}};
    if (c.c.repr == GPUQ_REPR_PACKED15) o.push_back({"raw128", jnum(1)});
    if (t.sides[i] > 0 && t.dense) o.push_back({"dense", jnum(1)});
    f.a.push_back(jobj(o));
  }
  return f;
}
PSchema plain_schema(const PTable& t) {
  PSchema s;
  for (size_t i = 0; i < t.cols.size(); ++i) s.push_back({t.cols[i].name, t.cols[i].type, t.cols[i].nullable || (t.sides[i] > 0 && !t.dense)});
  return s;
}
std::string table_sig(const PTable& t) {
  std::string r = std::to_string(t.via.size()) + (t.dense ? "d" : "s");
  for (size_t i = 0; i < t.cols.size(); ++i)
    r += "|" + t.cols[i].name + ":" + t.cols[i].type.dump() + (t.cols[i].nullable ? "?" : "") + std::to_string(t.sides[i]) + "r" + std::to_string(t.cols[i].c.repr);
  return r;
}

Json rewrite_columns(const Json& e, const std::function<Json(const Json&)>& fn) {
  if (e.is_obj()) {
    if (e.o.size() == 1 && e.o[0].first == "column" && e.o[0].second.is_obj() && e.o[0].second.find("name")) return fn(e.o[0].second);
    Json r = jobj();
    for (auto& kv : e.o) r.o.emplace_back(kv.first, rewrite_columns(kv.second, fn));
    return r;
  }
  if (e.is_arr()) { Json r = jarr(); for (auto& v : e.a) r.a.push_back(rewrite_columns(v, fn)); return r; }
  return e;
}
typedef std::map<std::string, Json> ColMap;
Json inline_projection(const Json& e, const ColMap* m) {
  if (!m) return e;
  return rewrite_columns(e, [&](const Json& c) { auto it = m->find(c.at("name").str()); return it != m->end() ? it->second : jobj({{"column", c}}); });
}
template <class Names> Json rebind(const Json& e, const Names& names) {
  return rewrite_columns(e, [&](const Json& c) {
    const std::string& n = c.at("name").str();
    for (size_t i = 0; i < names.size(); ++i) if (names[i] == n) return jcol(n, (int)i);
    throw std::runtime_error("plan: column '" + n + "' not found in the input schema");
  });
}
std::vector<std::string> names_of(const PTable& t) { std::vector<std::string> v; for (auto& c : t.cols) v.push_back(c.name); return v; }
bool has_like(const Json& e) {
  if (e.is_obj()) { for (auto& kv : e.o) if (kv.first == "like_expr" || has_like(kv.second)) return true; return false; }
  if (e.is_arr()) { for (auto& v : e.a) if (has_like(v)) return true; }
  return false;
}
Json lower_long_string_eq(const Json& e) {
  if (e.is_obj()) {
    if (e.o.size() == 1 && e.o[0].first == "binary_expr" && e.o[0].second.is_obj()) {
      const Json& b = e.o[0].second;
      const std::string op = b.get_str("op", "");
      if ((op == "=" || op == "!=" || op == "Eq" || op == "NotEq") && b.find("l") && b.find("r")) {
        auto is_col = [](const Json& v) { return v.is_obj() && v.o.size() == 1 && v.o[0].first == "column"; };
        auto long_lit = [](const Json& v) {
          if (!(v.is_obj() && v.o.size() == 1 && v.o[0].first == "literal" && v.o[0].second.is_obj())) return false;
          const Json& l = v.o[0].second;
          return l.get_str("type", "") == "Utf8" && l.find("value") && !l.at("value").is_null() && l.at("value").str().size() > 15;
        };
        const Json* c = nullptr; const Json* l = nullptr;
        if (is_col(b.at("l")) && long_lit(b.at("r"))) { c = &b.at("l"); l = &b.at("r"); }
        else if (is_col(b.at("r")) && long_lit(b.at("l"))) { c = &b.at("r"); l = &b.at("l"); }
        if (c) {
          std::string pat;
          for (char ch : l->o[0].second.at("value").str()) { if (ch == '%' || ch == '_') pat += '\\'; pat += ch; }
          return jobj({{"like_expr", jobj({{"negated", jbool(op == "!=" || op == "NotEq")}, {"case_insensitive", jbool(false)}, {"expr", *c},
                                           {"pattern", jobj({{"literal", jobj({{"type", jstr("Utf8")}, {"value", jstr(pat)}})}})}})}});
        }
      }
    }
    Json r = jobj();
    for (auto& kv : e.o) r.o.emplace_back(kv.first, lower_long_string_eq(kv.second));
    return r;
  }
  if (e.is_arr()) { Json r = jarr(); for (auto& v : e.a) r.a.push_back(lower_long_string_eq(v)); return r; }
  return e;
}
// ... 234 lines not shown
    c.c.type = T_BOOL; c.c.repr = GPUQ_REPR_ARROW; c.c.data = bits->p; c.c.validity = valid ? (const uint8_t*)valid->p : nullptr; c.c.length = t.n;
    out.cols.push_back(c); out.sides.push_back(0);
    out.keep.push_back(bits); if (valid) out.keep.push_back(valid);
  }
  return out;
}

bool is_long_string_failure(const std::exception& e) { return std::string(e.what()).find("longer than 15 bytes reached") != std::string::npos; }
int long_key_column(const PTable& t, const Json& e) {
  if (!(e.is_obj() && e.o.size() == 1 && e.o[0].first == "column" && e.o[0].second.is_obj() && e.o[0].second.find("name"))) return -1;
  const std::string& n = e.o[0].second.at("name").str();
  for (size_t i = 0; i < t.cols.size(); ++i)
    if (t.cols[i].name == n) return (t.cols[i].c.type == T_UTF8 && t.cols[i].c.repr == GPUQ_REPR_ARROW) ? (int)i : -1;
  return -1;
}
struct Utf8DictGuard { gpuq_utf8_dict* d = nullptr; ~Utf8DictGuard() { if (d) gpuq_utf8_dict_free(d); } };
void append_code_column(Exec& x, PTable& t, int ci, gpuq_utf8_dict* dict, bool insert, const std::string& name) {
  const PCol& c = t.cols[(size_t)ci]; const int sd = t.sides[(size_t)ci];
  const size_t nb = (size_t)((t.n + 63) / 64) * 8 + 8;
  BufP codes = dev_alloc((size_t)std::max<int64_t>(t.n, 1) * 8 + 16), valid = dev_alloc(nb);
  HIPCHECK(hipMemsetAsync(valid->p, 0, nb, (hipStream_t)x.stream));
  const int rc = gpuq_utf8_intern(dict, x.stream, &c.c, sd > 0 ? t.via[(size_t)sd - 1] : nullptr, t.n, insert ? 1 : 0, (int64_t*)codes->p, (uint8_t*)valid->p);
  check(x, rc);
  PCol k; k.name = name; k.type = jstr("Int64"); k.nullable = true;
  k.c.type = T_INT64; k.c.repr = GPUQ_REPR_ARROW; k.c.data = codes->p; k.c.validity = (const uint8_t*)valid->p; k.c.length = t.n;
  t.cols.push_back(k); t.sides.push_back(0); t.keep.push_back(codes); t.keep.push_back(valid); t.record_cap = 0;
}
void strip_code_columns(PTable& t) {
  for (size_t i = t.cols.size(); i-- > 0;)
    if (t.cols[i].name.rfind("__code_", 0) == 0) { t.cols.erase(t.cols.begin() + (long)i); t.sides.erase(t.sides.begin() + (long)i); t.record_cap = 0; }
}

template <class F> auto retry_long_cmp(const int tag, F&& run) -> decltype(run(tag, false)) {
  try { return run(tag, false); }
  catch (const Unsupported& e) { if (!is_long_string_failure(e)) throw; }
  return run(tag + 64, true);
}
static PTable project_impl(Exec& x, const PTable& t_in, const std::vector<Json>& exprs_in, const std::vector<std::string>& names, const void* site, int tag, const bool long_cmp) {
  std::vector<Json> exprs = exprs_in;
  bool any_like = false; for (auto& e : exprs) any_like = any_like || has_like(e);
  PTable t_res = t_in; if (any_like || long_cmp) resolve(x, t_res);
  PTable t = lower_like(x, t_res, exprs);
  if (long_cmp) t = lower_strcmp(x, t, exprs);
  gpuq_op* op = cached_op(x, site, tag, table_sig(t), [&]() {
    Json ex = jarr();
    const auto nm = names_of(t);
    for (size_t i = 0; i < exprs.size(); ++i) ex.a.push_back(jobj({{"expr", rebind(exprs[i], nm)}, {"name", jstr(names[i])}}));
    return jobj({{"op", jstr("project")}, {"input", jobj({{"fields", table_fields(t)}})}, {"exprs", ex}});
  });
  const bool deferred = prep(x, op, t);
  std::vector<gpuq_column> carr;
  PTable out = alloc_outputs(op, t.n, carr);
  out.count_from(t);
  InputC ic; make_input(t, ic);
  check(x, gpuq_project_run(op, x.stream, &ic.in, carr.data(), (int)carr.size()));
  if (deferred) return out;
  bool has_utf8 = false, computed = false;
  for (auto& c : t.cols) has_utf8 = has_utf8 || c.c.type == T_UTF8;
  for (auto& e : exprs) computed = computed || !(e.is_obj() && e.o.size() == 1 && (e.o[0].first == "column" || e.o[0].first == "literal"));
  if (has_utf8 && computed) check(x, gpuq_op_check(op, x.stream));
  return out;
}
PTable project(Exec& x, const PTable& t_in, const std::vector<Json>& exprs_in, const std::vector<std::string>& names, const void* site, int tag) {
  return retry_long_cmp(tag, [&](int tg, bool long_cmp) { return project_impl(x, t_in, exprs_in, names, site, tg, long_cmp); });
}

const uint32_t* take_u32(Exec& x, const uint32_t* vec, int64_t vec_len, const uint32_t* idx, int64_t n, std::vector<BufP>& keep, const PTable* count = nullptr) {
  PTable src; src.n = n; src.via.push_back(idx); src.sides.push_back(1);
  if (count) src.count_from(*count);
  PCol c; c.name = "v"; c.type = jstr("UInt32"); c.nullable = false; c.c.type = T_UINT32; c.c.data = vec; c.c.length = vec_len;
  src.cols.push_back(c);
  static const int take_site = 0;
  const Json v = jcol("v", 0);
  const Json e = jobj({{"case_", jobj({{"expr", Json()}, {"when_then_expr", jarr({jobj({{"when_expr", jobj({{"is_null_expr", jobj({{"expr", v}})}})},
                      {"then_expr", jobj({{"literal", jobj({{"type", jstr("UInt32")}, {"value", jstr(std::to_string(NULL_ROW_ID))}})}})}})})}, {"else_expr", v}})}});
  PTable out = project(x, src, {e}, {"v"}, &take_site, 0);
  keep.insert(keep.end(), out.keep.begin(), out.keep.end());
  return (const uint32_t*)out.cols[0].c.data;
}

PTable materialize(Exec& x, const PTable& t, bool force = false);

void prune_columns(PTable& t, const std::set<std::string>& keep) {
  for (size_t i = t.cols.size(); i-- > 0;)
    if (!keep.count(t.cols[i].name)) { t.cols.erase(t.cols.begin() + (long)i); t.sides.erase(t.sides.begin() + (long)i); t.record_cap = 0; }
}
PTable select_view(Exec& x, const PTable& t, const uint32_t* idx, int64_t n, const BufP& idx_owner, const PTable* count = nullptr) {
  PTable out; out.n = n; out.own(t); if (idx_owner) out.keep.push_back(idx_owner);
  if (count) out.count_from(*count);
  if (!t.is_view()) {
    out.cols = t.cols; out.via = {idx}; out.sides.assign(t.cols.size(), 1);
    return out;
  }
  bool has0 = false; for (int s : t.sides) has0 = has0 || s == 0;
  if ((int)t.via.size() + (has0 ? 1 : 0) > 3) {
    PTable m = materialize(x, t);
    out.own(m); out.cols = m.cols; out.via = {idx}; out.sides.assign(m.cols.size(), 1);
    return out;
  }
  out.cols = t.cols;
  if (has0) out.via.push_back(idx);
  for (const uint32_t* v : t.via) out.via.push_back(take_u32(x, v, t.n, idx, n, out.keep, count));
  const int shift = has0 ? 1 : 0;
  for (int s : t.sides) out.sides.push_back(s == 0 ? 1 : s + shift);
  return out;
}

PCol take_utf8(Exec& x, const PCol& c, const uint32_t* idx, int64_t n, bool nullable, std::vector<BufP>& keep) {
  BufP offs = dev_alloc((size_t)(n + 4) * 4), valid = dev_alloc((size_t)((n + 63) / 64) * 8 + 8);
  int64_t dl = 0;
  int rc = gpuq_take_utf8(x.ctx, x.stream, &c.c, idx, n, (int32_t*)offs->p, (uint8_t*)valid->p, nullptr, 0, &dl);
  if (rc != GPUQ_OK && rc != GPUQ_ERR_CAPACITY) check(x, rc);
  BufP data = dev_alloc((size_t)dl + 16);
  if (dl > 0) check(x, gpuq_take_utf8(x.ctx, x.stream, &c.c, idx, n, (int32_t*)offs->p, (uint8_t*)valid->p, (uint8_t*)data->p, dl + 16, &dl));
  PCol o = c;
  o.nullable = nullable; o.c.repr = GPUQ_REPR_ARROW; o.c.data = data->p; o.c.offsets = (const int32_t*)offs->p;
  o.c.validity = nullable ? (const uint8_t*)valid->p : nullptr; o.c.length = n;
  keep.push_back(offs); keep.push_back(data); keep.push_back(valid);
  return o;
}

PTable materialize(Exec& x, const PTable& t_in, bool force) {
  if (!t_in.is_view() && !force) return t_in;
  const bool pack_strings = force;
  PTable t = t_in;
  if (t.n_dev) {
    bool strings = force;
    for (auto& c : t.cols) strings = strings || (c.c.offsets && !pack_strings);
    if (strings) resolve(x, t);
  }
  PTable out; out.n = t.n; out.count_from(t);
  out.cols.resize(t.cols.size()); out.sides.assign(t.cols.size(), 0);
  std::vector<size_t> fixed;
  for (size_t i = 0; i < t.cols.size(); ++i) {
    const PCol& c = t.cols[i];
    if (c.c.offsets && !pack_strings) {
      if (!t.is_view()) out.cols[i] = c;
      else out.cols[i] = take_utf8(x, c, t.sides[i] > 0 ? t.via[(size_t)t.sides[i] - 1] : nullptr, t.n, c.nullable || (t.sides[i] > 0 && !t.dense), out.keep);
    } else fixed.push_back(i);
  }
  for (size_t a = 0; a < fixed.size(); a += 12) {
    PTable sub; sub.n = t.n; sub.via = t.via; sub.dense = t.dense; sub.count_from(t);
    std::vector<Json> ex; std::vector<std::string> nm;
    const size_t hi = std::min(a + 12, fixed.size());
    for (size_t k = a; k < hi; ++k) { sub.cols.push_back(t.cols[fixed[k]]); sub.sides.push_back(t.sides[fixed[k]]); }
    for (size_t i = 0; i < sub.cols.size(); ++i) { ex.push_back(jcol(sub.cols[i].name, (int)i)); nm.push_back(sub.cols[i].name); }
    static const int mat_site = 0;
    gpuq_op* op = cached_op(x, &mat_site, 0, table_sig(sub), [&]() {
      Json exj = jarr();
      for (size_t i = 0; i < ex.size(); ++i) exj.a.push_back(jobj({{"expr", ex[i]}, {"name", jstr(nm[i])}}));
      return jobj({{"op", jstr("project")}, {"input", jobj({{"fields", table_fields(sub)}})}, {"exprs", exj}});
    });
    prep(x, op, sub);
    if (!sub.n_dev && t.n_dev) { t.n = sub.n; t.count_from(sub); out.n = sub.n; out.count_from(sub); }
    std::vector<gpuq_column> carr;
    PTable part = alloc_outputs(op, sub.n, carr);
    InputC ic; make_input(sub, ic);
    check(x, gpuq_project_run(op, x.stream, &ic.in, carr.data(), (int)carr.size()));
    for (size_t k = a; k < hi; ++k) out.cols[fixed[k]] = part.cols[k - a];
    out.own(part);
  }
  out.own(t);
  return out;
}

static int64_t filter_sel_impl(Exec& x, const PTable& source_in, const Json& predicate_in, const void* site, int tag, BufP& sel_out, const bool long_cmp) {
// ... 100 lines not shown
      groups.push_back(jarr({jobj({{"expr", jcol(name, (int)w.cols.size() - 1)}, {"asc", jbool(asc)}, {"nulls_first", jbool(s.get_bool("nulls_first", !asc))}})}));
    }
  }
  flush();
  PermOut out;
  for (size_t gi = groups.size(); gi-- > 0;) {
    if (!out.p) { BufP p = sort_perm(x, w, groups[gi], site, tag * 64 + 8 + (int)gi); out.p = (const uint32_t*)p->p; out.keep.push_back(p); continue; }
    PTable view = select_view(x, w, out.p, w.n, nullptr);
    BufP p2 = sort_perm(x, view, groups[gi], site, tag * 64 + 8 + (int)gi);
    out.keep.push_back(p2);
    for (auto& b : view.keep) out.keep.push_back(b);
    out.p = take_u32(x, out.p, w.n, (const uint32_t*)p2->p, w.n, out.keep);
  }
  for (auto& b : w.keep) out.keep.push_back(b);
  return out;
}

static bool is_wide_sort_key(const std::exception& e) { return std::string(e.what()).find("composite sort key needs") != std::string::npos; }
PTable sort_table(Exec& x, const PTable& t_in, const Json& sort_exprs, int64_t fetch, const void* site, int tag) {
  PTable t = t_in; bool wide = false;
  try {
    SortedKey sk;
    if (sort_exprs.a.size() == 1 && !t.is_view() && t.n >= (1 << 20)) {
      const Json& e = sort_exprs.a[0].at("expr");
      if (e.is_obj() && e.o.size() == 1 && e.o[0].first == "column" && e.o[0].second.find("name")) {
        const std::string& nm = e.o[0].second.at("name").str();
        for (size_t i = 0; i < t.cols.size(); ++i) if (t.cols[i].name == nm) {
          const int ty = t.cols[i].c.type;
          if (ty == T_INT8 || ty == T_INT16 || ty == T_INT32 || ty == T_INT64 || ty == T_UINT8 || ty == T_UINT16 || ty == T_UINT32 || ty == T_DATE32 || ty == T_DATE64 ||
              ty == T_TIMESTAMP || ty == T_DECIMAL128) sk.col = (int)i;
          break;
        }
      }
    }
    BufP perm = sort_perm(x, t, sort_exprs, site, tag, sk.col >= 0 ? &sk : nullptr);
    const int64_t k = (fetch < 0 || fetch > t.n) ? t.n : fetch;
    PTable out = select_view(x, t, (const uint32_t*)perm->p, k, perm, t.n_dev ? &t : nullptr);
    if (sk.decoded) {
      PCol& kc = out.cols[(size_t)sk.col];
      kc.c.data = sk.data->p; kc.c.validity = sk.valid ? (const uint8_t*)sk.valid->p : nullptr; kc.c.length = k;
      kc.nullable = sk.valid != nullptr;
      out.sides[(size_t)sk.col] = 0;
      out.keep.push_back(sk.data); if (sk.valid) out.keep.push_back(sk.valid);
      out.record_cap = 0;
    }
    return out;
  } catch (const Unsupported& e) { if (!is_long_string_failure(e) && !is_wide_sort_key(e)) throw; wide = is_wide_sort_key(e); }
  resolve(x, t);
  const int64_t k = (fetch < 0 || fetch > t.n) ? t.n : fetch;
  PermOut po = sort_perm_long(x, t, sort_exprs, site, tag, wide ? 1 : 4);
  PTable out = select_view(x, t, po.p, k, nullptr);
  for (auto& b : po.keep) out.keep.push_back(b);
  return out;
}

PTable concat_tables(Exec& x, std::vector<PTable> parts);

PTable merge_table(Exec& x, const PTable& t_in, const std::vector<int64_t>& run_offsets, const Json& sort_exprs, int64_t fetch, const void* site, int tag) {
  if (run_offsets.size() <= 2) return sort_table(x, t_in, sort_exprs, fetch, site, tag);
  PTable t = t_in; resolve(x, t);
  gpuq_op* op = cached_op(x, site, tag, table_sig(t), [&]() {
    const auto nm = names_of(t);
    Json ex = jarr();
    for (auto& s : sort_exprs.a) {
      const bool asc = s.get_bool("asc", true);
      ex.a.push_back(jobj({{"expr", rebind(s.at("expr"), nm)}, {"asc", jbool(asc)}, {"nulls_first", jbool(s.get_bool("nulls_first", !asc))}}));
    }
    return jobj({{"op", jstr("sort")}, {"input", jobj({{"fields", table_fields(t)}})}, {"expr", ex}});
  });
  BufP perm = dev_alloc((size_t)std::max<int64_t>(t.n, 1) * 4 + 16);
  InputC ic; make_input(t, ic);
  check(x, gpuq_merge_run(op, x.stream, &ic.in, run_offsets.data(), (int)run_offsets.size() - 1, (uint32_t*)perm->p));
  const int64_t k = (fetch < 0 || fetch > t.n) ? t.n : fetch;
  return select_view(x, t, (const uint32_t*)perm->p, k, perm);
}

struct Metrics { int64_t output_rows = 0, elapsed_ns = 0; };
struct PNode {
  std::string kind; Metrics m; int id = 0;
  std::string label(const char* what) const { return std::string(what) + "_n" + std::to_string(id); }
  virtual ~PNode() {}
  virtual std::vector<PNode*> children() { return {}; }
  virtual int partitions() { auto c = children(); return c.empty() ? 1 : c[0]->partitions(); }
  virtual PSchema schema() { auto c = children(); if (c.empty()) throw std::runtime_error("plan: node without a schema"); return c[0]->schema(); }
  virtual PTable execute(int part, Exec& x) = 0;
  typedef std::set<std::string> Names;
  virtual void require(const Names* need) { (void)need; for (PNode* c : children()) c->require(nullptr); }
  PTable timed(Exec& x, std::chrono::steady_clock::time_point t0, PTable t) {
    m.elapsed_ns += std::chrono::duration_cast<std::chrono::nanoseconds>(std::chrono::steady_clock::now() - t0).count();
    m.output_rows += t.n;
    if (t.n_dev) x.fixes.push_back({t.n_dev, t.n, &m.output_rows, t.n_keep});
    return t;
  }
};
typedef std::unique_ptr<PNode> PNodeP;
PNodeP build_node(const Json& j);

struct MemoryExec : PNode {
  PSchema schema_; std::vector<int> parts; bool dense = false;
  PSchema schema() override { return schema_; }
  int partitions() override { return (int)parts.size(); }
  PTable execute(int part, Exec& x) override {
    if (part < 0 || part >= (int)parts.size()) throw std::runtime_error("MemoryExec: partition out of range");
    const int slot = parts[(size_t)part];
    if (slot < 0 || slot >= x.n_inputs) throw std::runtime_error("MemoryExec: input " + std::to_string(slot) + " was not supplied");
    const gpuq_input& in = x.inputs[slot];
    if (in.n_cols != (int)schema_.size()) throw std::runtime_error("MemoryExec: input has " + std::to_string(in.n_cols) + " columns, schema_ has " + std::to_string(schema_.size()));
    PTable t; t.n = in.n_rows; t.dense = dense;
    for (int k = 0; k < in.n_via; ++k) t.via.push_back(in.via[k]);
    for (int i = 0; i < in.n_cols; ++i) {
      PCol c; c.name = schema_[(size_t)i].name; c.type = schema_[(size_t)i].type; c.nullable = schema_[(size_t)i].nullable; c.c = in.cols[i];
      int p, s; const int tid = type_id_of(c.type, p, s);
      if (c.c.type != tid) throw std::runtime_error("MemoryExec: column '" + c.name + "' does not have the declared type");
      t.cols.push_back(c);
    }
    t.sides = sides.empty() ? std::vector<int>(t.cols.size(), in.n_via > 0 ? 1 : 0) : sides;
    m.output_rows += t.n;
    return t;
  }
  std::vector<int> sides;
};

Json schema_fields(const PSchema& s) {
  Json f = jarr();
  for (auto& c : s) f.a.push_back(jobj({{"name", jstr(c.name)}, {"type", c.type}, {"nullable", jbool(c.nullable)}, {"side", jnum(0)}}));
  return f;
}
std::vector<std::string> schema_names(const PSchema& s) { std::vector<std::string> v; for (auto& c : s) v.push_back(c.name); return v; }
Json type_json_from_string(const std::string& t) {
  if (t.rfind("Decimal128", 0) == 0) {
    long long p = 38, sc = 0; std::sscanf(t.c_str(), "Decimal128(%lld, %lld)", &p, &sc);
    if (t.find(',') != std::string::npos && t.find(", ") == std::string::npos) std::sscanf(t.c_str(), "Decimal128(%lld,%lld)", &p, &sc);
    return jobj({{"Decimal128", jarr({jnum(p), jnum(sc)})}});
  }
  return jstr(t);
}
PSchema compiled_outputs(const Json& desc) {
  std::vector<char> buf(1 << 20);
  const int rc = gpuq_compile_check(desc.dump().c_str(), buf.data(), buf.size());
  if (rc != GPUQ_OK) { const char* m = gpuq_last_error(nullptr); throw std::runtime_error(std::string("plan schema: ") + (m ? m : "descriptor does not compile")); }
  const Json r = JsonParser(buf.data()).parse();
  PSchema out;
  for (auto& o : r.at("outputs").a) out.push_back({o.at("name").str(), type_json_from_string(o.at("type").str()), o.get_bool("nullable", true)});
  return out;
}

void collect_columns(const Json& e, std::set<std::string>& out) {
  (void)rewrite_columns(e, [&](const Json& c) { out.insert(c.at("name").str()); return jobj({{"column", c}}); });
}
struct PassThrough : PNode {
  PNodeP input;
  std::vector<PNode*> children() override { return {input.get()}; }
  void require(const Names* need) override { input->require(need); }
  PTable execute(int part, Exec& x) override { return input->execute(part, x); }
};

struct FilterExec : PNode {
  PNodeP input; Json predicate;
  std::vector<PNode*> children() override { return {input.get()}; }
  void require(const Names* need) override { if (!need) { input->require(nullptr); return; } Names n = *need; collect_columns(predicate, n); input->require(&n); }
  PTable execute(int part, Exec& x) override;
};
struct ProjectionExec : PNode {
  PNodeP input; std::vector<Json> exprs; std::vector<std::string> names;
  std::vector<PNode*> children() override { return {input.get()}; }
  void require(const Names*) override { Names n; for (auto& e : exprs) collect_columns(e, n); input->require(&n); }
  PSchema schema() override {
    const PSchema in = input->schema(); const auto nm = schema_names(in);
    std::vector<Json> ex = exprs;
    for (auto& e : ex) e = rewrite_like(e, [&](const Json& v) { return jobj({{"is_not_null_expr", jobj({{"expr", jobj({{"not_expr", jobj({{"expr", jobj({{"is_null_expr", jobj({{"expr", v.at("expr")}})}})}})}})}})}}); });
    Json exj = jarr();
    for (size_t i = 0; i < ex.size(); ++i) exj.a.push_back(jobj({{"expr", rebind(ex[i], nm)}, {"name", jstr(names[i])}}));
    PSchema out = compiled_outputs(jobj({{"op", jstr("project")}, {"input", jobj({{"fields", schema_fields(in)}})}, {"exprs", exj}}));
    for (size_t i = 0; i < exprs.size() && i < out.size(); ++i) if (has_like(exprs[i])) out[i].nullable = true;
    return out;
  }
  PTable execute(int part, Exec& x) override;
};

struct Fused { PNode* src = nullptr; bool has_pred = false; Json pred; bool has_map = false; ColMap map; };
Fused fuse(PNode* n) {
  if (auto* p = dynamic_cast<PassThrough*>(n)) return fuse(p->input.get());
  if (auto* f = dynamic_cast<FilterExec*>(n)) {
    if (has_like(f->predicate)) { Fused r; r.src = n; return r; }
    Fused r = fuse(f->input.get());
    const Json mine = inline_projection(f->predicate, r.has_map ? &r.map : nullptr);
    r.pred = r.has_pred ? jand(r.pred, mine) : mine; r.has_pred = true;
    return r;
  }
  if (auto* p = dynamic_cast<ProjectionExec*>(n)) {
    for (auto& e : p->exprs) if (has_like(e)) { Fused r; r.src = n; return r; }
    Fused r = fuse(p->input.get());
    ColMap nm;
    for (size_t i = 0; i < p->exprs.size(); ++i) nm[p->names[i]] = inline_projection(p->exprs[i], r.has_map ? &r.map : nullptr);
    r.map = std::move(nm); r.has_map = true;
    return r;
  }
  Fused r; r.src = n; return r;
}

PTable FilterExec::execute(int part, Exec& x) {
  Fused f;
  if (has_like(predicate)) {
    f = fuse(input.get());
    const Json mine = inline_projection(predicate, f.has_map ? &f.map : nullptr);
    f.pred = f.has_pred ? jand(f.pred, mine) : mine; f.has_pred = true;
  } else f = fuse(this);
  PTable t = f.src->execute(part, x);
  auto t0 = std::chrono::steady_clock::now();
  if (!f.has_map) return timed(x, t0, filter_table(x, t, f.pred, this, 0));
  PTable v = filter_table(x, t, f.pred, this, 0);
  std::vector<Json> ex; std::vector<std::string> nm;
  for (auto& kv : f.map) { nm.push_back(kv.first); ex.push_back(kv.second); }
  return timed(x, t0, project(x, v, ex, nm, this, 1));
}
PTable ProjectionExec::execute(int part, Exec& x) {
  Fused f = fuse(input.get());
  PTable t = f.src->execute(part, x);
  auto t0 = std::chrono::steady_clock::now();
  if (f.has_pred) t = filter_table(x, t, f.pred, this, 0);
  std::vector<Json> ex;
  for (auto& e : exprs) ex.push_back(inline_projection(e, f.has_map ? &f.map : nullptr));
  std::vector<int> pick;
  for (auto& e : ex) {
    int ci = -1;
    if (e.is_obj() && e.o.size() == 1 && e.o[0].first == "column" && e.o[0].second.is_obj() && e.o[0].second.find("name")) {
      const std::string& n = e.o[0].second.at("name").str();
      for (size_t i = 0; i < t.cols.size(); ++i) if (t.cols[i].name == n) { ci = (int)i; break; }
    }
    if (ci < 0) { pick.clear(); break; }
    pick.push_back(ci);
  }
  if (!pick.empty() && pick.size() == ex.size()) {
    PTable out; out.n = t.n; out.via = t.via; out.dense = t.dense; out.keep = t.keep; out.count_from(t);
    for (size_t i = 0; i < pick.size(); ++i) { PCol c = t.cols[(size_t)pick[i]]; c.name = names[i]; out.cols.push_back(c); out.sides.push_back(t.sides[(size_t)pick[i]]); }
    return timed(x, t0, out);
  }
  return timed(x, t0, project(x, t, ex, names, this, 1));
}

struct AggregateExec : PNode {
  PNodeP input; std::string mode, strategy = "auto"; Json group_expr, aggr_expr; int64_t expected_groups = 0, output_capacity = 0;
  std::vector<PNode*> children() override { return {input.get()}; }
  void require(const Names*) override {
    if (mode == "Final" || mode == "FinalPartitioned") { input->require(nullptr); return; }
    Names n;
    for (auto& g : group_expr.a) collect_columns(g.at("expr"), n);
    for (auto& a : aggr_expr.a) for (const char* k : {"expr", "expr2", "filter"}) if (a.has(k)) collect_columns(a.at(k), n);
    input->require(&n);
  }
  PSchema schema() override {
    const PSchema in = input->schema(); const auto nm = schema_names(in);
    Json ge = jarr(), ae = jarr();
    for (auto& g : group_expr.a) ge.a.push_back(jobj({{"expr", rebind(g.at("expr"), nm)}, {"name", g.at("name")}}));
    for (auto& a : aggr_expr.a) {
      std::vector<std::pair<std::string, Json>> o = {{"fn", a.at("fn")}, {"name", a.at("name")}};
      for (const char* k : {"expr", "expr2", "filter"}) if (a.has(k)) o.push_back({k, rebind(a.at(k), nm)});
      ae.a.push_back(jobj(o));
    }
    PSchema out = compiled_outputs(jobj({{"op", jstr("aggregate")}, {"mode", jstr(mode)}, {"input", jobj({{"fields", schema_fields(in)}})}, {"strategy", jstr("hash")},
                                         {"group_expr", ge}, {"aggr_expr", ae}}));
    if (mode == "Final" || mode == "FinalPartitioned" || mode == "Single")
      for (size_t i = group_expr.a.size(); i < out.size(); ++i) out[i].nullable = true;
    return out;
  }
  PTable execute(int part, Exec& x) override {
    const bool final_ = mode == "Final" || mode == "FinalPartitioned";
    Fused f; if (final_) f.src = input.get(); else f = fuse(input.get());
    PTable t = f.src->execute(part, x);
    auto t0 = std::chrono::steady_clock::now();
    bool many_string_keys = false;
    if (group_expr.a.size() > 4) {
      const ColMap* cm0 = f.has_map ? &f.map : nullptr;
      for (auto& g : group_expr.a) if (long_key_column(t, inline_projection(g.at("expr"), cm0)) >= 0) many_string_keys = true;
    }
    if (!many_string_keys) {
      try { return timed(x, t0, run(x, t, f, false)); }
      catch (const Unsupported& e) { if (!is_long_string_failure(e)) throw; }
    }
    resolve(x, t);
    try { return timed(x, t0, run(x, t, f, true)); }
    catch (const Unsupported& e) { if (!is_long_string_failure(e) || !f.has_pred) throw; }
    Fused f2 = f; f2.has_pred = false;
    PTable t2 = filter_table(x, t, f.pred, this, 9);
    return timed(x, t0, run(x, t2, f2, true));
  }
  PTable run(Exec& x, PTable t, const Fused& f, const bool long_keys) {
    const ColMap* cm0 = f.has_map ? &f.map : nullptr;
    std::vector<Json> gexprs; std::vector<int> coded;
    Utf8DictGuard dicts[8]; int nd = 0;
    const PTable t_src = t;
    for (auto& g : group_expr.a) {
      Json e = inline_projection(g.at("expr"), cm0); int ci = -1;
      if (long_keys && (ci = long_key_column(t_src, e)) >= 0 && nd < 8) {
        const std::string nm = "__code_" + std::to_string(gexprs.size());
        check(x, gpuq_utf8_dict_create(x.ctx, x.stream, std::min<int64_t>(t_src.n, t_src.cols[(size_t)ci].c.length), &dicts[nd].d));
        append_code_column(x, t, ci, dicts[nd].d, true, nm); ++nd;
        e = jobj({{"column", jobj({{"name", jstr(nm)}})}});
        if (group_expr.a.size() > 4) e = jobj({{"cast", jobj({{"expr", e}, {"arrow_type", jstr("UInt32")}})}});
      } else ci = -1;
      gexprs.push_back(e); coded.push_back(ci);
    }
    gpuq_op* op = cached_op(x, this, long_keys ? 6 : 0, table_sig(t), [&]() {
    const auto nm = names_of(t);
    const ColMap* cm = f.has_map ? &f.map : nullptr;
    Json ge = jarr(), ae = jarr();
    for (size_t k = 0; k < group_expr.a.size(); ++k) ge.a.push_back(jobj({{"expr", rebind(gexprs[k], nm)}, {"name", group_expr.a[k].at("name")}}));
    for (auto& a : aggr_expr.a) {
      std::vector<std::pair<std::string, Json>> o = {{"fn", a.at("fn")}, {"name", a.at("name")}};
      for (const char* k : {"expr", "expr2", "filter"}) if (a.has(k)) o.push_back({k, rebind(inline_projection(a.at(k), cm), nm)});
      ae.a.push_back(jobj(o));
    }
    std::vector<std::pair<std::string, Json>> d = {{"op", jstr("aggregate")}, {"mode", jstr(mode)}, {"input", jobj({{"fields", table_fields(t)}})},
                                                   {"strategy", jstr(strategy)}, {"group_expr", ge}, {"aggr_expr", ae}};
    if (f.has_pred) d.push_back({"predicate", rebind(f.pred, nm)});
    if (expected_groups) d.push_back({"expected_groups", jnum(expected_groups)});
    return jobj(d);
    });
    const bool deferred = !long_keys && prep(x, op, t);
    if (!deferred) resolve(x, t);
    int64_t cap = output_capacity > 0 ? output_capacity : (group_expr.a.empty() ? 4096 : std::max<int64_t>(4096, std::min<int64_t>(t.n, 1ll << 22)));
    if (output_capacity <= 0 && expected_groups > 0) cap = std::max<int64_t>(cap, std::min<int64_t>(t.n, expected_groups + expected_groups / 4));
    InputC ic; make_input(t, ic);
    if (deferred) {
      std::vector<gpuq_column> carr;
      PTable out = alloc_outputs(op, cap, carr);
      int64_t bound = 0; const uint64_t* ndev = nullptr;
      check(x, gpuq_aggregate_run_deferred(op, x.stream, &ic.in, carr.data(), (int)carr.size(), cap, &bound, &ndev));
      out.n = bound; for (auto& c : out.cols) c.c.length = bound;
      if (ndev) {
        BufP cnt = dev_alloc(16);
        HIPCHECK(hipMemcpyAsync(cnt->p, ndev, 8, hipMemcpyDeviceToDevice, (hipStream_t)x.stream));
        out.n_dev = (const uint64_t*)cnt->p; out.n_keep = cnt;
      }
      return out;
    }
    for (;;) {
      std::vector<gpuq_column> carr;
      PTable out = alloc_outputs(op, cap, carr);
      int64_t ng = 0;
      const int rc = gpuq_aggregate_run(op, x.stream, &ic.in, carr.data(), (int)carr.size(), cap, &ng);
      ++x.host_syncs;
      if (rc == GPUQ_ERR_CAPACITY && ng > cap) { cap = ng; continue; }
      check(x, rc);
      out.n = ng; for (auto& c : out.cols) c.c.length = ng;
      for (size_t k = 0; k < coded.size(); ++k) {
        if (coded[k] < 0) continue;
        BufP rows = dev_alloc((size_t)std::max<int64_t>(ng, 1) * 4 + 16);
        check(x, gpuq_utf8_code_rows(x.ctx, x.stream, &out.cols[k].c, ng, (uint32_t*)rows->p));
        const PCol& src = t_src.cols[(size_t)coded[k]];
        PCol sc = take_utf8(x, src, (const uint32_t*)rows->p, ng, true, out.keep);
        sc.name = out.cols[k].name; out.cols[k] = sc; out.record_cap = 0;
        HIPCHECK(hipStreamSynchronize((hipStream_t)x.stream));
      }
      return out;
    }
  }
};

struct SortExec : PNode {
  PNodeP input; Json expr; int64_t fetch = -1; bool merge_all = false;
  std::vector<PNode*> children() override { return {input.get()}; }
  void require(const Names* need) override { if (!need) { input->require(nullptr); return; } Names n = *need; for (auto& s : expr.a) collect_columns(s.at("expr"), n); input->require(&n); }
  int partitions() override { return merge_all ? 1 : input->partitions(); }
  PTable execute(int part, Exec& x) override {
    PTable t;
    if (merge_all && input->partitions() != 1) {
      std::vector<PTable> in; std::vector<int64_t> offs{0};
      for (int p = 0; p < input->partitions(); ++p) { in.push_back(input->execute(p, x)); resolve(x, in.back()); offs.push_back(offs.back() + in.back().n); }
      auto t0 = std::chrono::steady_clock::now();
      t = concat_tables(x, std::move(in));
      return timed(x, t0, merge_table(x, t, offs, expr, fetch, this, 1));
    }
    t = input->execute(part, x);
    auto t0 = std::chrono::steady_clock::now();
    return timed(x, t0, sort_table(x, t, expr, fetch, this, 0));
  }
};

struct HashJoinExec : PNode {
  PNodeP left, right; Json on; std::string join_type = "Inner", partition_mode = "CollectLeft"; bool null_equals_null = false; bool has_filter = false; Json filter;
  std::vector<PNode*> children() override { return {left.get(), right.get()}; }
  bool out_need_all = true; Names out_need;
  void require(const Names* need) override {
    out_need_all = need == nullptr; if (need) out_need = *need;
    if (!need) { left->require(nullptr); right->require(nullptr); return; }
    Names n = *need;
    for (auto& o : on.a) { collect_columns(o.at("left"), n); collect_columns(o.at("right"), n); }
    if (has_filter) collect_columns(filter, n);
    left->require(&n); right->require(&n);
  }
  int partitions() override { return right->partitions(); }
  PSchema schema() override {
    PSchema l = left->schema(), r = right->schema();
    const std::string& jt = join_type;
    if (jt == "LeftSemi" || jt == "LeftAnti") return l;
    if (jt == "RightSemi" || jt == "RightAnti") return r;
    if (jt == "Right" || jt == "Full") for (auto& c : l) c.nullable = true;
    if (jt == "Left" || jt == "Full") for (auto& c : r) c.nullable = true;
    l.insert(l.end(), r.begin(), r.end());
    return l;
  }
  struct Side { PTable t; bool has_pred = false; Json pred; };
  Side side(PNode* plan, int part, Exec& x) {
    Fused f = fuse(plan);
    Side s;
    if (f.has_map) { s.t = plan->execute(part, x); return s; }
    s.t = f.src->execute(part, x); s.has_pred = f.has_pred; s.pred = f.pred;
    return s;
  }
  int64_t last_pairs = -1;
  PTable join_view(Exec& x, const PTable& lt, const PTable& rt, const uint32_t* ob, const uint32_t* opb, int64_t k, const BufP& ob_own, const BufP& opb_own, const PTable* count = nullptr) {
    PTable lv = select_view(x, lt, ob, k, ob_own, count), rv = select_view(x, rt, opb, k, opb_own, count);
    if (lv.via.size() + rv.via.size() > 3) {
      if (lv.via.size() >= rv.via.size()) lv = materialize(x, lv); else rv = materialize(x, rv);
    }
    PTable out; out.n = k; out.own(lv); out.own(rv);
    if (count) out.count_from(*count);
    out.cols = lv.cols; out.via = lv.via; out.sides = lv.sides;
    const int shift = (int)lv.via.size();
    for (size_t i = 0; i < rv.cols.size(); ++i) { out.cols.push_back(rv.cols[i]); out.sides.push_back(rv.sides[i] == 0 ? 0 : rv.sides[i] + shift); }
    for (auto v : rv.via) out.via.push_back(v);
    return out;
  }
  int64_t marked_rows(Exec& x, const uint32_t* rows, int64_t k, int64_t n, bool want_marked, int tag, BufP& out) {
    const size_t nb = (size_t)((n + 63) / 64) * 8 + 8;
    BufP bits = dev_alloc(nb);
    HIPCHECK(hipMemsetAsync(bits->p, 0, nb, (hipStream_t)x.stream));
    check(x, gpuq_mark_rows(x.ctx, x.stream, rows, k, (uint8_t*)bits->p));
    PTable t; t.n = n; t.keep.push_back(bits);
    PCol c; c.name = "m"; c.type = jstr("Boolean"); c.nullable = false; c.c.type = T_BOOL; c.c.repr = GPUQ_REPR_ARROW; c.c.data = bits->p; c.c.length = n;
    t.cols.push_back(c); t.sides.push_back(0);
    const Json m = jcol("m", 0);
    return filter_sel(x, t, want_marked ? m : jobj({{"not_expr", jobj({{"expr", m}})}}), this, tag, out);
  }
  PTable residual_join(Exec& x, const PTable& lt, const PTable& rt, const PTable& pairs, const BufP& ob, const BufP& opb, int64_t k) {
    hipStream_t s = (hipStream_t)x.stream;
    BufP sel; const int64_t k2 = filter_sel(x, pairs, filter, this, 2, sel);
    std::vector<BufP> keep{ob, opb, sel};
    const uint32_t* ob2 = k2 ? take_u32(x, (const uint32_t*)ob->p, k, (const uint32_t*)sel->p, k2, keep) : (const uint32_t*)ob->p;
    const uint32_t* opb2 = k2 ? take_u32(x, (const uint32_t*)opb->p, k, (const uint32_t*)sel->p, k2, keep) : (const uint32_t*)opb->p;
    const std::string& jt = join_type;
    auto with_keep = [&](PTable t) { for (auto& b : keep) t.keep.push_back(b); return t; };
    if (jt == "LeftSemi" || jt == "LeftAnti") { BufP rows; const int64_t m = marked_rows(x, ob2, k2, lt.n, jt == "LeftSemi", 5, rows); return with_keep(select_view(x, lt, (const uint32_t*)rows->p, m, rows)); }
    if (jt == "RightSemi" || jt == "RightAnti") { BufP rows; const int64_t m = marked_rows(x, opb2, k2, rt.n, jt == "RightSemi", 6, rows); return with_keep(select_view(x, rt, (const uint32_t*)rows->p, m, rows)); }
    BufP lrows, rrows; int64_t ml = 0, mr = 0;
    if (jt == "Left" || jt == "Full") ml = marked_rows(x, ob2, k2, lt.n, false, 5, lrows);
    if (jt == "Right" || jt == "Full") mr = marked_rows(x, opb2, k2, rt.n, false, 6, rrows);
    const int64_t k3 = k2 + ml + mr;
    BufP ob3 = dev_alloc((size_t)std::max<int64_t>(k3, 1) * 4 + 16), opb3 = dev_alloc((size_t)std::max<int64_t>(k3, 1) * 4 + 16);
    uint32_t* a = (uint32_t*)ob3->p; uint32_t* b = (uint32_t*)opb3->p;
    if (k2) { HIPCHECK(hipMemcpyAsync(a, ob2, (size_t)k2 * 4, hipMemcpyDeviceToDevice, s)); HIPCHECK(hipMemcpyAsync(b, opb2, (size_t)k2 * 4, hipMemcpyDeviceToDevice, s)); }
    if (ml) { HIPCHECK(hipMemcpyAsync(a + k2, lrows->p, (size_t)ml * 4, hipMemcpyDeviceToDevice, s)); HIPCHECK(hipMemsetAsync(b + k2, 0xFF, (size_t)ml * 4, s)); }
    if (mr) { HIPCHECK(hipMemsetAsync(a + k2 + ml, 0xFF, (size_t)mr * 4, s)); HIPCHECK(hipMemcpyAsync(b + k2 + ml, rrows->p, (size_t)mr * 4, hipMemcpyDeviceToDevice, s)); }
    HIPCHECK(hipStreamSynchronize(s));
    return join_view(x, lt, rt, a, b, k3, ob3, opb3);
  }
  PTable execute(int part, Exec& x) override {
    Side L, R;
    HashJoinExec* inner = chain_inner();
    if (inner) {
      const int lpart = partition_mode == "Partitioned" ? part : 0;
      Side Li, Ri; inner->sides(lpart, x, Li, Ri);
      R = side(right.get(), part, x);
      auto t0 = std::chrono::steady_clock::now();
      Chain ch;
      if (chain_build(x, inner, Li, Ri, ch)) {
        struct Guard { gpuq_join_table* t; ~Guard() { if (t) gpuq_join_table_free(t); } } guard{ch.table};
        Side Lv; Lv.t = ch.view;
        return timed(x, t0, join_sides(x, Lv, R, false, &ch));
      }
      auto t1 = std::chrono::steady_clock::now();
      L.t = inner->timed(x, t1, inner->join_sides(x, Li, Ri, false));
    } else sides(part, x, L, R);
    auto t0 = std::chrono::steady_clock::now();
    try { return timed(x, t0, join_sides(x, L, R, false)); }
    catch (const Unsupported& e) { if (!is_long_string_failure(e)) throw; }
    resolve(x, L.t); resolve(x, R.t);
    PTable out;
    try { out = join_sides(x, L, R, true); }
    catch (const Unsupported& e) {
      if (!is_long_string_failure(e) || !(L.has_pred || R.has_pred)) throw;
      if (L.has_pred) { L.t = filter_table(x, L.t, L.pred, this, 41); L.has_pred = false; }
      if (R.has_pred) { R.t = filter_table(x, R.t, R.pred, this, 42); R.has_pred = false; }
      strip_code_columns(L.t); strip_code_columns(R.t);
      out = join_sides(x, L, R, true);
    }
    strip_code_columns(out);
    return timed(x, t0, out);
  }
  void sides(int part, Exec& x, Side& L, Side& R) {
    const int lpart = partition_mode == "Partitioned" ? part : 0;
    if (partition_mode != "Partitioned" && left->partitions() != 1) {
      std::vector<PTable> in; for (int p = 0; p < left->partitions(); ++p) in.push_back(left->execute(p, x));
      L.t = concat_tables(x, std::move(in));
    } else L = side(left.get(), lpart, x);
    R = side(right.get(), part, x);
  }
  struct Chain { gpuq_join_table* table = nullptr; PTable view; bool deferred = false; };
  static bool is_plain_column(const Json& e, std::string& name) {
    if (!(e.is_obj() && e.o.size() == 1 && e.o[0].first == "column" && e.o[0].second.is_obj() && e.o[0].second.find("name"))) return false;
    name = e.o[0].second.at("name").str(); return true;
  }
  int chain_checked = 0;
  HashJoinExec* chain_inner() {
    static const bool on_env = []() { const char* e = getenv("GPUQ_JOIN_CHAIN"); return !(e && e[0] == '0'); }();
// ... 47 lines not shown
      if (Ri.has_pred) bd.push_back({"predicate", rebind(Ri.pred, rn)});
      return jobj(bd);
    });
    bool deferred = x.deferred && last_pairs >= 0 && gpuq_op_can_defer(bop1) && gpuq_op_can_defer(bop2);
    if (deferred) deferred = use_deferred(x, bop1) && use_deferred(x, bop2);
    if (!deferred) { use_sync(x, bop1); use_sync(x, bop2); resolve(x, Li.t); resolve(x, Ri.t); }
    InputC lic, ric; make_input(Li.t, lic); make_input(Ri.t, ric);
    gpuq_join_table* t1 = nullptr;
    check(x, gpuq_join_build_run(bop1, x.stream, &lic.in, 0, Li.t.n, &t1));
    struct Guard { gpuq_join_table* t; ~Guard() { if (t) gpuq_join_table_free(t); } } g1{t1};
    if (!deferred) x.host_syncs += 2;
    if (gpuq_join_table_has_duplicates(t1)) return false;
    bool want_hits = in->out_need_all;
    for (auto& c : Li.t.cols) want_hits = want_hits || in->out_need.count(c.name) > 0;
    BufP hits = want_hits ? dev_alloc((size_t)std::max<int64_t>(Ri.t.n, 1) * 4 + 16) : nullptr, rows = dev_alloc(16);
    gpuq_join_table* t2 = nullptr;
    check(x, gpuq_join_build_run_semi(bop2, x.stream, &ric.in, 0, Ri.t.n, t1, want_hits ? (uint32_t*)hits->p : nullptr, (uint64_t*)rows->p, &t2));
    ch.table = t2; ch.deferred = deferred;
    if (deferred) { in->m.output_rows += Ri.t.n; x.fixes.push_back({(const uint64_t*)rows->p, Ri.t.n, &in->m.output_rows, rows}); }
    else { in->m.output_rows += (int64_t)read_u64(x, rows->p); x.host_syncs += 2; }
    PTable v; v.n = Ri.t.n; v.count_from(Ri.t); v.own(Ri.t);
    if (want_hits) {
      v.own(Li.t); v.keep.push_back(hits);
      v.via.push_back((const uint32_t*)hits->p);
      for (auto p : Ri.t.via) v.via.push_back(p);
      for (size_t i = 0; i < Li.t.cols.size(); ++i) { v.cols.push_back(Li.t.cols[i]); v.sides.push_back(1); }
      for (size_t i = 0; i < Ri.t.cols.size(); ++i) { v.cols.push_back(Ri.t.cols[i]); v.sides.push_back(Ri.t.sides[i] == 0 ? 0 : Ri.t.sides[i] + 1); }
    } else { v.via = Ri.t.via; v.cols = Ri.t.cols; v.sides = Ri.t.sides; v.dense = Ri.t.dense; }
    ch.view = v;
    return true;
  }
  PTable join_sides(Exec& x, Side L, Side R, const bool long_keys, Chain* chain = nullptr) {
    if (!out_need_all) {
      Names keep = out_need;
      for (auto& o : on.a) { collect_columns(o.at("left"), keep); collect_columns(o.at("right"), keep); }
      if (has_filter) collect_columns(filter, keep);
      if (L.has_pred) collect_columns(L.pred, keep);
      if (R.has_pred) collect_columns(R.pred, keep);
      prune_columns(L.t, keep); prune_columns(R.t, keep);
    }
    const bool residual = has_filter && join_type != "Inner";
    const std::string jt = residual ? std::string("Inner") : join_type;
    if (residual) {
      resolve(x, L.t); resolve(x, R.t);
      if (L.has_pred) { L.t = filter_table(x, L.t, L.pred, this, 3); L.has_pred = false; }
      if (R.has_pred) { R.t = filter_table(x, R.t, R.pred, this, 4); R.has_pred = false; }
      resolve(x, L.t); resolve(x, R.t);
    }
    Json on_eff = on;
    Utf8DictGuard dicts[8]; int nd = 0;
    if (long_keys) {
      if (null_equals_null) throw Unsupported("null_equals_null with Utf8 join keys longer than 15 bytes");
      for (size_t k = 0; k < on_eff.a.size() && nd < 8; ++k) {
        const int li = long_key_column(L.t, on.a[k].at("left")), ri = long_key_column(R.t, on.a[k].at("right"));
        if (li < 0 || ri < 0) continue;
        const std::string nm = "__code_" + std::to_string(k);
        check(x, gpuq_utf8_dict_create(x.ctx, x.stream, std::min<int64_t>(L.t.n, L.t.cols[(size_t)li].c.length), &dicts[nd].d));
        append_code_column(x, L.t, li, dicts[nd].d, true, nm + "l");
        append_code_column(x, R.t, ri, dicts[nd].d, false, nm + "r");
        ++nd;
        on_eff.a[k] = jobj({{"left", jobj({{"column", jobj({{"name", jstr(nm + "l")}})}})}, {"right", jobj({{"column", jobj({{"name", jstr(nm + "r")}})}})}});
      }
    }
    gpuq_op* bop = chain ? nullptr : cached_op(x, this, long_keys ? 7 : 0, table_sig(L.t), [&]() {
      const auto ln = names_of(L.t);
      Json lk = jarr();
      for (auto& o : on_eff.a) lk.a.push_back(rebind(o.at("left"), ln));
      const bool side_rows = jt == "Left" || jt == "Full" || jt == "LeftSemi" || jt == "LeftAnti";
      std::vector<std::pair<std::string, Json>> bd = {{"op", jstr("join_build")}, {"input", jobj({{"fields", table_fields(L.t)}})}, {"on", lk}, {"null_equals_null", jbool(null_equals_null)},
                                                     {"build_side_rows", jbool(side_rows)}, {"label", jstr(label("build"))}};
      if (L.has_pred) bd.push_back({"predicate", rebind(L.pred, ln)});
      return jobj(bd);
    });
    gpuq_op* pop = cached_op(x, this, long_keys ? 8 : 1, table_sig(R.t), [&]() {
      const auto rn = names_of(R.t);
      Json rk = jarr();
      for (auto& o : on_eff.a) rk.a.push_back(rebind(o.at("right"), rn));
      std::vector<std::pair<std::string, Json>> pd = {{"op", jstr("join_probe")}, {"input", jobj({{"fields", table_fields(R.t)}})}, {"on", rk}, {"join_type", jstr(jt)},
                                                     {"null_equals_null", jbool(null_equals_null)}, {"label", jstr(label("probe"))}};
      if (R.has_pred) pd.push_back({"predicate", rebind(R.pred, rn)});
      return jobj(pd);
    });
    const bool plain = !long_keys && !residual && !has_filter && (jt == "Inner" || jt == "Right" || jt == "RightSemi" || jt == "RightAnti");
    bool deferred = false;
    if (chain) deferred = chain->deferred && plain && use_deferred(x, pop);
    else if (plain && x.deferred && last_pairs >= 0 && gpuq_op_can_defer(bop)) deferred = use_deferred(x, bop) && use_deferred(x, pop);
    if (!deferred) { if (bop) use_sync(x, bop); use_sync(x, pop); resolve(x, L.t); resolve(x, R.t); }
    InputC lic, ric; make_input(L.t, lic); make_input(R.t, ric);
    gpuq_join_table* jtab = chain ? chain->table : nullptr;
    if (!chain) {
      check(x, gpuq_join_build_run(bop, x.stream, &lic.in, 0, L.t.n, &jtab));
      if (!deferred) x.host_syncs += 2;
    }
    struct Guard { gpuq_join_table* t; ~Guard() { if (t) gpuq_join_table_free(t); } } guard{chain ? nullptr : jtab};
    const bool lout = jt == "Left" || jt == "Full";
    const int64_t extra_cap = lout ? L.t.n : 0;
    int64_t cap = std::max<int64_t>(R.t.n, 1) + extra_cap;
    BufP cnt = dev_alloc(16), ob, opb; int64_t k = 0;
    if (deferred) {
      cap = gpuq_join_table_has_duplicates(jtab) ? last_pairs + last_pairs / 8 + 4096 : std::min<int64_t>(cap, last_pairs + last_pairs / 8 + 4096);
      { static const bool trace = getenv("GPUQ_TRACE_DEFER") != nullptr; if (trace) fprintf(stderr, "[gpuq] deferred %s join: build bound %lld, probe bound %lld, pair capacity %lld (last run %lld pairs), dups %d\n", jt.c_str(), (long long)L.t.n, (long long)R.t.n, (long long)cap, (long long)last_pairs, gpuq_join_table_has_duplicates(jtab)); }
      ob = dev_alloc((size_t)cap * 4 + 16); opb = dev_alloc((size_t)cap * 4 + 16);
      const bool pairs = jt == "Inner" || jt == "Right";
      check(x, gpuq_join_probe_run(pop, x.stream, jtab, &ric.in, 0, pairs ? (uint32_t*)ob->p : nullptr, (uint32_t*)opb->p, (uint64_t)cap, (uint64_t*)cnt->p));
      PTable c; c.n_dev = (const uint64_t*)cnt->p; c.n_keep = cnt;
      if (!pairs) return select_view(x, R.t, (const uint32_t*)opb->p, cap, opb, &c);
      return join_view(x, L.t, R.t, (const uint32_t*)ob->p, (const uint32_t*)opb->p, cap, ob, opb, &c);
    }
    for (;;) {
      ob = dev_alloc((size_t)cap * 4 + 16); opb = dev_alloc((size_t)cap * 4 + 16);
      check(x, gpuq_join_probe_run(pop, x.stream, jtab, &ric.in, 0, (uint32_t*)ob->p, (uint32_t*)opb->p, (uint64_t)(cap - extra_cap), (uint64_t*)cnt->p));
      k = (int64_t)read_u64(x, cnt->p);
      const int rc = gpuq_op_check(pop, x.stream);
      ++x.host_syncs;
      if (rc == GPUQ_ERR_CAPACITY) { cap = k + extra_cap + 1; continue; }
      check(x, rc);
      break;
    }
    if (plain) last_pairs = k;
    if (jt == "LeftSemi" || jt == "LeftAnti" || lout) {
      BufP extra = dev_alloc(16);
      if (!lout) {
        BufP rows = dev_alloc((size_t)std::max<int64_t>(L.t.n, 1) * 4 + 16);
        check(x, gpuq_join_build_side_rows(jtab, x.stream, jt == "LeftSemi" ? 1 : 0, (uint32_t*)rows->p, (uint64_t*)extra->p));
        const int64_t mrows = (int64_t)read_u64(x, extra->p);
        return select_view(x, L.t, (const uint32_t*)rows->p, mrows, rows);
      }
      check(x, gpuq_join_build_side_rows(jtab, x.stream, 0, (uint32_t*)ob->p + k, (uint64_t*)extra->p));
      const int64_t mrows = (int64_t)read_u64(x, extra->p);
      if (mrows > 0) HIPCHECK(hipMemsetAsync((uint32_t*)opb->p + k, 0xFF, (size_t)mrows * 4, (hipStream_t)x.stream));
      k += mrows;
    }
    if (jt == "RightSemi" || jt == "RightAnti") return select_view(x, R.t, (const uint32_t*)opb->p, k, opb);
    PTable out = join_view(x, L.t, R.t, (const uint32_t*)ob->p, (const uint32_t*)opb->p, k, ob, opb);
    if (residual) return residual_join(x, L.t, R.t, out, ob, opb, k);
    if (has_filter) out = filter_table(x, out, filter, this, 2);
    return out;
  }
};

struct LimitExec : PNode {
  PNodeP input; int64_t fetch = 0;
  std::vector<PNode*> children() override { return {input.get()}; }
  PTable execute(int part, Exec& x) override {
    PTable t = input->execute(part, x);
    resolve(x, t);
    if (fetch < t.n) { t.n = fetch; for (auto& c : t.cols) if (!t.is_view() && c.c.length > fetch) c.c.length = fetch; }
    m.output_rows += t.n;
    return t;
  }
};

PTable concat_tables(Exec& x, std::vector<PTable> parts) {
  for (auto& p : parts) resolve(x, p);
  std::vector<PTable> live;
  for (auto& p : parts) if (p.n > 0) live.push_back(p);
  if (live.empty() && !parts.empty()) live.push_back(parts[0]);
  if (live.empty()) throw std::runtime_error("concat: no input partitions");
  if (live.size() == 1 && !live[0].is_view()) return live[0];
  for (auto& p : live) p = materialize(x, p);
  int64_t n = 0; for (auto& p : live) n += p.n;
  const size_t nc = live[0].cols.size();
  const size_t bm = (size_t)((n + 63) / 64) * 8 + 8;
  std::vector<size_t> doff(nc), voff(nc, 0), dbytes(nc);
  size_t off = 256;
  for (size_t i = 0; i < nc; ++i) {
    const PCol& c0 = live[0].cols[i];
    for (auto& p : live) if (p.cols[i].c.type != c0.c.type || p.cols[i].c.repr != c0.c.repr) throw std::runtime_error("concat: column '" + c0.name + "' has different layouts across partitions");
    DType dt; dt.id = c0.c.type; dt.p = c0.c.precision; dt.s = c0.c.scale;
    for (auto& p : live) if ((p.cols[i].c.offsets != nullptr) != (c0.c.offsets != nullptr)) throw std::runtime_error("concat: column '" + c0.name + "' has different layouts across partitions");
    if (c0.c.offsets) dbytes[i] = (size_t)(n + 4) * 4;
    else dbytes[i] = c0.c.type == T_BOOL ? bm : (size_t)std::max<int64_t>(n, 1) * (size_t)type_width(dt) + 16;
    doff[i] = off; off += (dbytes[i] + 255) & ~(size_t)255;
    bool any_valid = false; for (auto& p : live) any_valid = any_valid || p.cols[i].c.validity != nullptr;
    if (any_valid) { voff[i] = off; off += (bm + 255) & ~(size_t)255; }
  }
  BufP buf = dev_alloc(off);
  hipStream_t s = (hipStream_t)x.stream;
  PTable out; out.n = n; out.keep.push_back(buf); out.record_cap = std::max<int64_t>(n, 1);
  for (size_t i = 0; i < nc; ++i) {
    PCol c = live[0].cols[i];
    DType dt; dt.id = c.c.type; dt.p = c.c.precision; dt.s = c.c.scale;
    char* d = (char*)buf->p + doff[i];
    uint8_t* v = voff[i] ? (uint8_t*)buf->p + voff[i] : nullptr;
    if (c.c.type == T_BOOL) HIPCHECK(hipMemsetAsync(d, 0, bm, s));
    if (v) HIPCHECK(hipMemsetAsync(v, 0, bm, s));
    int64_t row = 0; bool nullable = false;
    if (c.c.offsets) {
      std::vector<int32_t> first(live.size()), last(live.size()); int64_t total = 0;
      for (size_t q = 0; q < live.size(); ++q) {
        const PCol& pc = live[q].cols[i];
        HIPCHECK(hipMemcpyAsync(&x.pin[0], pc.c.offsets, 4, hipMemcpyDeviceToHost, s));
        HIPCHECK(hipMemcpyAsync((char*)&x.pin[0] + 4, pc.c.offsets + live[q].n, 4, hipMemcpyDeviceToHost, s));
        HIPCHECK(hipStreamSynchronize(s));
        std::memcpy(&first[q], &x.pin[0], 4); std::memcpy(&last[q], (char*)&x.pin[0] + 4, 4);
        total += last[q] - first[q];
      }
      BufP bytes = dev_alloc((size_t)total + 16);
      int64_t base = 0;
      for (size_t q = 0; q < live.size(); ++q) {
        const PCol& pc = live[q].cols[i];
        nullable = nullable || pc.nullable;
        check(x, gpuq_offsets_rebase(x.ctx, x.stream, pc.c.offsets, live[q].n + 1, (int32_t)(base - first[q]), (int32_t*)d + row));
        if (last[q] > first[q]) HIPCHECK(hipMemcpyAsync((char*)bytes->p + base, (const char*)pc.c.data + first[q], (size_t)(last[q] - first[q]), hipMemcpyDeviceToDevice, s));
        if (v && live[q].n > 0) check(x, gpuq_copy_bits(x.ctx, x.stream, v, row, pc.c.validity, 0, live[q].n));
        row += live[q].n; base += last[q] - first[q];
      }
      c.nullable = nullable; c.c.offsets = (const int32_t*)d; c.c.data = bytes->p; c.c.validity = v; c.c.length = n;
      out.keep.push_back(bytes);
      out.cols.push_back(c); out.sides.push_back(0);
      continue;
    }
    for (auto& p : live) {
      const PCol& pc = p.cols[i];
      nullable = nullable || pc.nullable;
      if (p.n > 0) {
        if (c.c.type == T_BOOL) check(x, gpuq_copy_bits(x.ctx, x.stream, (uint8_t*)d, row, (const uint8_t*)pc.c.data, 0, p.n));
        else { const size_t w = (size_t)type_width(dt); HIPCHECK(hipMemcpyAsync(d + (size_t)row * w, pc.c.data, (size_t)p.n * w, hipMemcpyDeviceToDevice, s)); }
        if (v) check(x, gpuq_copy_bits(x.ctx, x.stream, v, row, pc.c.validity, 0, p.n));
      }
      row += p.n;
    }
    c.nullable = nullable; c.c.data = d; c.c.validity = v; c.c.offsets = nullptr; c.c.length = n;
    out.cols.push_back(c); out.sides.push_back(0);
  }
  for (auto& p : live) out.own(p);
  return out;
}

PTable slice_table(Exec& x, PTable t, int64_t skip, int64_t count) {
  resolve(x, t);
  skip = std::min(std::max<int64_t>(skip, 0), t.n);
  count = (count < 0 || skip + count > t.n) ? t.n - skip : count;
  if (skip == 0) { t.n = count; if (!t.is_view()) for (auto& c : t.cols) c.c.length = count; return t; }
  bool has0 = false; if (t.is_view()) for (int sd : t.sides) has0 = has0 || sd == 0;
  if (t.is_view() && !has0) { for (auto& v : t.via) v += skip; t.n = count; return t; }
  t = materialize(x, t, true);
  hipStream_t s = (hipStream_t)x.stream;
  const size_t bm = (size_t)((count + 63) / 64) * 8 + 8;
  for (auto& c : t.cols) {
    DType dt; dt.id = c.c.type; dt.p = c.c.precision; dt.s = c.c.scale;
    if (c.c.type == T_BOOL) {
      BufP b = dev_alloc(bm); HIPCHECK(hipMemsetAsync(b->p, 0, bm, s));
      check(x, gpuq_copy_bits(x.ctx, x.stream, (uint8_t*)b->p, 0, (const uint8_t*)c.c.data, skip, count));
      c.c.data = b->p; t.keep.push_back(b);
    } else c.c.data = (const char*)c.c.data + (size_t)skip * (size_t)type_width(dt);
    if (c.c.validity) {
      BufP b = dev_alloc(bm); HIPCHECK(hipMemsetAsync(b->p, 0, bm, s));
      check(x, gpuq_copy_bits(x.ctx, x.stream, (uint8_t*)b->p, 0, c.c.validity, skip, count));
      c.c.validity = (const uint8_t*)b->p; t.keep.push_back(b);
    }
    c.c.length = count;
  }
  t.n = count; t.record_cap = 0;
  return t;
}

struct CrossJoinExec : HashJoinExec {
  void require(const Names* need) override { left->require(need); right->require(need); }
  PSchema schema() override { PSchema l = left->schema(), r = right->schema(); l.insert(l.end(), r.begin(), r.end()); return l; }
  PTable execute(int part, Exec& x) override {
    std::vector<PTable> ls;
    for (int p = 0; p < left->partitions(); ++p) { ls.push_back(left->execute(p, x)); resolve(x, ls.back()); }
    PTable lt = ls.size() == 1 ? ls[0] : concat_tables(x, std::move(ls));
    PTable rt = right->execute(part, x); resolve(x, rt);
    auto t0 = std::chrono::steady_clock::now();
    const int64_t k = lt.n * rt.n;
    BufP ob = dev_alloc((size_t)std::max<int64_t>(k, 1) * 4 + 16), opb = dev_alloc((size_t)std::max<int64_t>(k, 1) * 4 + 16);
    check(x, gpuq_cross_pairs(x.ctx, x.stream, lt.n, rt.n, (uint32_t*)ob->p, (uint32_t*)opb->p));
    return timed(x, t0, join_view(x, lt, rt, (const uint32_t*)ob->p, (const uint32_t*)opb->p, k, ob, opb));
  }
};

struct UnionExec : PNode {
  std::vector<PNodeP> inputs;
  std::vector<PNode*> children() override { std::vector<PNode*> v; for (auto& i : inputs) v.push_back(i.get()); return v; }
  int partitions() override { int k = 0; for (auto& i : inputs) k += i->partitions(); return k; }
  PSchema schema() override {
    PSchema s0 = inputs.at(0)->schema();
    for (size_t k = 1; k < inputs.size(); ++k) { const PSchema sk = inputs[k]->schema(); for (size_t i = 0; i < s0.size() && i < sk.size(); ++i) s0[i].nullable = s0[i].nullable || sk[i].nullable; }
    return s0;
  }
  PTable execute(int part, Exec& x) override {
    for (auto& i : inputs) { const int k = i->partitions(); if (part < k) { PTable t = i->execute(part, x); return timed(x, std::chrono::steady_clock::now(), t); } part -= k; }
    throw std::runtime_error("UnionExec: partition out of range");
  }
};

struct CoalesceExec : PNode {
  PNodeP input; std::vector<int> parts; bool all = false; bool ordered = false; Json order_by;
  std::vector<PNode*> children() override { return {input.get()}; }
  int partitions() override { return 1; }
  PTable execute(int, Exec& x) override {
    if (!all && parts.size() == 1) return input->execute(parts[0], x);
    std::vector<PTable> in;
    if (all || ordered) for (int p = 0; p < input->partitions(); ++p) in.push_back(input->execute(p, x));
    else for (int p : parts) in.push_back(input->execute(p, x));
    std::vector<int64_t> offs{0};
    for (auto& t : in) { resolve(x, t); offs.push_back(offs.back() + t.n); }
    auto t0 = std::chrono::steady_clock::now();
    PTable out = concat_tables(x, std::move(in));
    if (ordered) out = merge_table(x, out, offs, order_by, -1, this, 0);
    return timed(x, t0, out);
  }
};

struct GlobalLimitExec : PNode {
  PNodeP input; int64_t skip = 0, fetch = -1;
  std::vector<PNode*> children() override { return {input.get()}; }
  int partitions() override { return 1; }
  PTable execute(int, Exec& x) override {
    if (input->partitions() != 1) throw std::runtime_error("GlobalLimitExec requires a single input partition");
    PTable t = input->execute(0, x);
// ... 790 lines not shown
```

Measured before the change: 162.7 billion rows/s.

## Group aggregates by unique build-row id and pack narrow keys into slot state

When an inner join's build side has unique keys and the group-by keys functionally depend on the build row, the aggregate groups on a single UInt32 build-row index and re-projects the original group columns from the build table afterwards. Separately, narrow integer group keys (total at most 62 bits) are packed into the slot's state word, so the hash table stores no key words and insertion is a single CAS. Extraction then writes keys and accumulators straight into the post-processing SoA buffers, skipping the raw intermediate. This cuts hash-table width and key hashing and comparison costs in q3's aggregate. In exchange it adds a gather-based projection step and more complex plumbing that could misfire if the functional-dependency detection is wrong.

```diff
diff --git a/arrow-ballista_amd/csrc/agg_compile.cpp b/arrow-ballista_amd/csrc/agg_compile.cpp
--- a/arrow-ballista_amd/csrc/agg_compile.cpp
+++ b/arrow-ballista_amd/csrc/agg_compile.cpp
@@ -431,6 +431,21 @@
     R.acc_bits.push_back(accs[i].arg ? R.prog.out_bits[acc_slots[i]] : 1);
   }
   R.keys = make_keyspec(kregs, R.key_types, any_null_key);
+  {
+    int total = 0; bool narrow = nk > 0;
+    for (int k = 0; k < nk && narrow; ++k) {
+      int bits = 0; bool sgn = false;
+      switch (keys.nodes[k]->type.id) {
+        case T_INT8: bits = 8; sgn = true; break;   case T_UINT8: bits = 8; break;
+        case T_INT16: bits = 16; sgn = true; break; case T_UINT16: bits = 16; break;
+        case T_INT32: case T_DATE32: bits = 32; sgn = true; break; case T_UINT32: bits = 32; break;
+        default: narrow = false;
+      }
+      R.keys.sk_bits[k] = bits; R.keys.sk_signed[k] = sgn; R.keys.sk_null[k] = keys.nodes[k]->nullable ? 1 : 0;
+      total += bits + R.keys.sk_null[k];
+    }
+    R.keys.state_key = narrow && total <= 62;
+  }
 
   for (int k = 0; k < nk; ++k) { Field f; f.name = keys.names[k]; f.type = keys.nodes[k]->type; f.nullable = keys.nodes[k]->nullable; f.raw128 = 1; R.post_schema.fields.push_back(f); }
   for (size_t i = 0; i < accs.size(); ++i) { Field f; f.name = "acc" + std::to_string(i); f.type = accs[i].type; f.nullable = false; f.raw128 = 1; R.post_schema.fields.push_back(f); }
diff --git a/arrow-ballista_amd/csrc/capi.cpp b/arrow-ballista_amd/csrc/capi.cpp
--- a/arrow-ballista_amd/csrc/capi.cpp
+++ b/arrow-ballista_amd/csrc/capi.cpp
@@ -422,7 +422,7 @@
       for (size_t i = 0; i < op->posts.size(); ++i) { if (i) r += ","; r += describe_program(op->posts[i].prog, op->post_schema); }
       r += "],\"acc_kinds\":[";
       for (int a = 0; a < op->agg.n_accs; ++a) { if (a) r += ","; r += std::to_string(op->agg.acc_kind[a]); }
-      r += "]";
+      r += std::string("],\"state_key\":") + (op->keys.state_key ? "true" : "false");
     }
     r += ",\"outputs\":[";
     for (size_t i = 0; i < op->out_fields.size(); ++i) {
@@ -589,22 +589,28 @@
     const int nk = op->agg.n_keys, na = op->agg.n_accs, kstride = nk > 0 ? nk : 1;
     uint32_t ng = 0;
     AggOut raw{};
+    KeySpec Krun = op->keys; Krun.state_key = 0;
     auto alloc_raw = [&](i64 rcap) {
       raw.cap = (int32_t)rcap;
-      raw.keys = (u64*)op->ws[0].ensure((size_t)rcap * kstride * 16);
-      raw.key_nulls = (uint32_t*)op->ws[1].ensure((size_t)rcap * 4);
-      raw.cells = (u64*)op->ws[2].ensure((size_t)rcap * na * 16);
+      if (!Krun.state_key) {
+        raw.keys = (u64*)op->ws[0].ensure((size_t)rcap * kstride * 16);
+        raw.key_nulls = (uint32_t*)op->ws[1].ensure((size_t)rcap * 4);
+        raw.cells = (u64*)op->ws[2].ensure((size_t)rcap * na * 16);
+      }
       raw.n_groups = op->flags_dev.as<uint32_t>() + 2;
       HIPCHECK(hipMemsetAsync(raw.n_groups, 0, 8, s));
     };
     auto read_ng = [&]() { uint32_t v[3] = {0, 0, 0}; read_status(op, s, v, 3); return v[2]; };
     if (n_outs != (int)op->out_fields.size()) throw std::runtime_error("expected " + std::to_string(op->out_fields.size()) + " output columns, got " + std::to_string(n_outs));
     bool posted = false;
-    auto run_post = [&](uint32_t rows, const uint32_t* rows_dev) {
+    AggSoA soa{}; std::vector<gpuq_column> pcols; bool soa_filled = false;
+    auto layout_soa = [&](uint32_t rows, const bool all_valid) {
       const size_t colbytes = (size_t)std::max<uint32_t>(rows, 1) * 16, vbytes = ((size_t)rows + 63) / 64 * 8 + 8;
       char* soa_mem = (char*)op->ws[6].ensure((size_t)(nk + na) * colbytes + (size_t)nk * vbytes);
-      AggSoA soa{};
-      std::vector<gpuq_column> pcols(nk + na);
+      bool any_null = false; for (int k = 0; k < nk; ++k) any_null = any_null || op->keys.sk_null[k];
+      if (all_valid && any_null) HIPCHECK(hipMemsetAsync(soa_mem + (size_t)(nk + na) * colbytes, 0xFF, (size_t)nk * vbytes, s));
+      soa = AggSoA{};
+      pcols.assign(nk + na, gpuq_column{});
       for (int k = 0; k < nk; ++k) {
         soa.key_col[k] = (ulonglong2*)(soa_mem + (size_t)k * colbytes);
         soa.key_valid[k] = (u64*)(soa_mem + (size_t)(nk + na) * colbytes + (size_t)k * vbytes);
@@ -616,7 +622,10 @@
         const DType& t = op->acc_types[a];
         pcols[nk + a] = gpuq_column{t.id, t.p, t.s, 0, soa.acc_col[a], nullptr, nullptr, (int64_t)rows};
       }
-      launch_agg_emit(s, raw, nk, na, rows, soa, rows_dev);
+    };
+    auto run_post = [&](uint32_t rows, const uint32_t* rows_dev) {
+      if (!soa_filled) { layout_soa(rows, false); launch_agg_emit(s, raw, nk, na, rows, soa, rows_dev); }
+      else for (auto& c : pcols) c.length = (int64_t)rows;
       gpuq_input pin{}; pin.cols = pcols.data(); pin.n_cols = nk + na; pin.n_rows = rows; pin.n_via = 0;
       for (auto& pc : op->posts) {
         DevProgram PP = bind_program(pc.prog, op->post_schema, pc.code.as<DevCode>(), op->flags_dev.as<uint32_t>(), &pin);
@@ -639,6 +648,9 @@
     HashTable T{};
     T.key_words = op->keys.key_words; T.slot_words = 1 + T.key_words + 2 * na;
     auto launch_table = [&](const u64 est, const u64 slot_pct, const bool use_lds, const bool reset) {
+      Krun.state_key = (op->keys.state_key && !use_lds) ? 1 : 0;
+      Krun.key_words = Krun.state_key ? 0 : op->keys.key_words;
+      T.key_words = Krun.state_key ? 0 : op->keys.key_words; T.slot_words = 1 + T.key_words + 2 * na;
       T.n_slots = next_pow2(est * slot_pct / 100);
       T.slots = (u64*)op->ws[5].ensure((size_t)T.n_slots * T.slot_words * 8);
       launch_ht_init(s, T, &op->agg);
@@ -650,7 +662,12 @@
         if (n_fsum > 0 && fbytes <= ((size_t)256 << 20)) { fstage = (u64*)op->ws[8].ensure(fbytes); HIPCHECK(hipMemsetAsync(fstage, 0, fbytes, s)); }
         SinkJit jit(op, op->prog, GPUQ_SINK_AGG_LDS, n); ProfScope ps(op, s); launch_agg_lds(s, jit.fn, P, n, op->keys, op->agg, T, fstage, n_fsum);
       }
-      else { SinkJit jit(op, op->prog, GPUQ_SINK_AGG_HASH, n); ProfScope ps(op, s); launch_agg_hash(s, jit.fn, P, n, op->keys, op->agg, T); }
+      else { SinkJit jit(op, op->prog, GPUQ_SINK_AGG_HASH, n); ProfScope ps(op, s); launch_agg_hash(s, jit.fn, P, n, Krun, op->agg, T); }
+    };
+    auto extract = [&]() {
+      const bool direct = Krun.state_key && raw.cap > 0;
+      if (direct) { layout_soa((uint32_t)raw.cap, true); soa_filled = true; }
+      launch_agg_hash_extract(s, Krun, op->agg, T, raw, op->flags_dev.as<uint32_t>(), direct ? &soa : nullptr);
     };
     auto run_radix = [&](const std::string& strat, const i64 known_groups) -> bool {
       const int slot_words = 1 + op->keys.key_words + 2 * na;
@@ -706,7 +723,7 @@
         if (rcap >= 1 && rcap <= 0x7FFFFFFFll) {
           launch_table(est, agg_slot_pct(true), L.ag.use_lds, false);
           alloc_raw(rcap);
-          launch_agg_hash_extract(s, op->keys, op->agg, T, raw, op->flags_dev.as<uint32_t>());
+          extract();
           finish_on_device();
           return;
         }
@@ -785,7 +802,7 @@
       path_done = 2; est_done = est; lds_done = use_lds;
       if (n <= (1ll << 20)) {
         alloc_raw(std::max<i64>(n, 1));
-        launch_agg_hash_extract(s, op->keys, op->agg, T, raw, op->flags_dev.as<uint32_t>());
+        extract();
         HIPCHECK(hipGetLastError());
         const bool ahead = (i64)raw.cap <= cap;
         if (ahead) run_post((uint32_t)raw.cap, raw.n_groups);
@@ -798,7 +815,7 @@
         bool done = false;
         if (L.ag.groups > 0) {
           alloc_raw(L.ag.groups + L.ag.groups / 4 + 1024);
-          launch_agg_hash_extract(s, op->keys, op->agg, T, raw, op->flags_dev.as<uint32_t>());
+          extract();
           HIPCHECK(hipGetLastError());
           uint32_t fw[4] = {0, 0, 0, 0};
           read_status(op, s, fw, 4);
@@ -809,13 +826,13 @@
         } else {
           alloc_raw(1);
           raw.cap = 0;
-          launch_agg_hash_extract(s, op->keys, op->agg, T, raw, op->flags_dev.as<uint32_t>());
+          extract();
           ng = read_ng();
           reset_flags(op, s);
         }
         if (!done) {
           alloc_raw(std::max<i64>(ng, 1));
-          launch_agg_hash_extract(s, op->keys, op->agg, T, raw, op->flags_dev.as<uint32_t>());
+          extract();
           HIPCHECK(hipGetLastError());
           ng = read_ng();
         }
diff --git a/arrow-ballista_amd/csrc/gpuq_kernels.h b/arrow-ballista_amd/csrc/gpuq_kernels.h
--- a/arrow-ballista_amd/csrc/gpuq_kernels.h
+++ b/arrow-ballista_amd/csrc/gpuq_kernels.h
@@ -41,6 +41,8 @@
   int32_t key_words;
   int32_t word_reg[MAX_KW];
   int32_t word_half[MAX_KW];
+  int32_t state_key;
+  int32_t sk_bits[MAX_KEYS], sk_signed[MAX_KEYS], sk_null[MAX_KEYS];
 };
 struct HashTable {
   u64* slots;
@@ -264,7 +266,7 @@
 void launch_bucket_bounds(hipStream_t s, const u64* sorted_bid, i64 n, u64 nbuckets, uint32_t* bounds, int shift);
 void launch_agg_bucket(hipStream_t s, void* jit_fn, const DevProgram& P, const KeySpec& K, const AggSpec& A, const uint32_t* ids, const uint32_t* bounds, uint32_t nbuckets,
                        uint32_t cap, int slot_words, const AggOut& out);
-void launch_agg_hash_extract(hipStream_t s, const KeySpec& K, const AggSpec& A, const HashTable& T, const AggOut& out, uint32_t* flags);
+void launch_agg_hash_extract(hipStream_t s, const KeySpec& K, const AggSpec& A, const HashTable& T, const AggOut& out, uint32_t* flags, const AggSoA* soa = nullptr);
 bool launch_join_build(hipStream_t s, void* jit_fn, const DevProgram& P, i64 n, const KeySpec& K, const HashTable& T, uint32_t* next, uint32_t* present,
                        int payload_via, int null_equals_null, const SemiProbe* semi = nullptr);
 void launch_join_keyrange(hipStream_t s, void* jit_fn, const DevProgram& P, i64 n, const KeySpec& K, int null_equals_null, u64* out, i64 wstep = 1);
diff --git a/arrow-ballista_amd/csrc/kernels_hash.hip b/arrow-ballista_amd/csrc/kernels_hash.hip
--- a/arrow-ballista_amd/csrc/kernels_hash.hip
+++ b/arrow-ballista_amd/csrc/kernels_hash.hip
@@ -82,6 +82,51 @@
   }
   return ~0ull;
 }
+
+__device__ __forceinline__ u64 pack_state_key(const KeySpec& K, GPUQ_REGS_CPARAM) {
+  u64 p = 0; int shift = 0;
+#pragma unroll
+  for (int k = 0; k < MAX_KEYS; ++k) {
+    if (k < K.n_keys) {
+      const int r = __builtin_amdgcn_readfirstlane(K.key_reg[k]);
+      const int b = __builtin_amdgcn_readfirstlane(K.sk_bits[k]), nb = __builtin_amdgcn_readfirstlane(K.sk_null[k]);
+      const bool isn = nb && ((rnulls >> r) & 1);
+      const u64 f = isn ? (1ull << b) : (rlo[r] & ((1ull << b) - 1));
+      p |= f << shift;
+      shift += b + nb;
+    }
+  }
+  return p;
+}
+__device__ __forceinline__ u64 ht_state_find_or_insert(const HashTable& T, const u64 key, const u64 h) {
+  const u64 mask = T.n_slots - 1, want = (key << 2) | 2ull;
+  u64 s = h & mask;
+  for (u64 probes = 0; probes < T.n_slots; ++probes) {
+    const u64 old = a_cas(T.slots + s * (u64)T.slot_words, 0ull, want);
+    if (old == 0ull || old == want) return s;
+    s = (s + 1) & mask;
+  }
+  return ~0ull;
+}
+#ifndef GPUQ_JIT
+__device__ __forceinline__ void emit_state_group(const u64* slot, const KeySpec& K, const AggSpec& A, const AggSoA& soa, const uint32_t g) {
+  const u64 st = slot[0] >> 2;
+  int shift = 0;
+  for (int k = 0; k < K.n_keys; ++k) {
+    const int b = K.sk_bits[k];
+    u64 lo = (st >> shift) & ((1ull << b) - 1);
+    const bool isn = K.sk_null[k] && ((st >> (shift + b)) & 1);
+    if (K.sk_signed[k]) lo = (u64)((i64)(lo << (64 - b)) >> (64 - b));
+    shift += b + K.sk_null[k];
+    soa.key_col[k][g] = make_ulonglong2(lo, (u64)((i64)lo >> 63));
+    if (isn) atomicAnd((unsigned long long*)(soa.key_valid[k] + (g >> 6)), ~(1ull << (g & 63)));
+  }
+  for (int a = 0; a < A.n_accs; ++a) {
+    const u64 lo = slot[1 + 2 * a];
+    soa.acc_col[a][g] = make_ulonglong2(lo, acc_result_hi(A.acc_kind[a], lo, slot[2 + 2 * a]));
+  }
+}
+#endif
 
 __device__ __forceinline__ bool ht_find(const HashTable& T, const u64 (&kw)[MAX_KW], u64 h, uint32_t& payload) {
   const u64 mask = T.n_slots - 1;
@@ -164,6 +209,8 @@
   const i64 n = rows_of(P, n_arg);
   const i64 nwords = (n + 63) >> 6;
   const int cell0 = 1 + T.key_words;
+  const bool state_key = K.state_key != 0;
+  const int cmp_words = state_key ? 1 : T.key_words;
   bool combine = true;
   for (int a = 0; a < A.n_accs; ++a) combine = combine && A.acc_kind[a] != ACC_FMIN && A.acc_kind[a] != ACC_FMAX;
   const int lane = hlane();
@@ -172,14 +219,17 @@
     u64 kw[MAX_KW]; u64 h = 0;
 #pragma unroll
     for (int q = 0; q < MAX_KW; ++q) kw[q] = 0;
-    if (active) make_key(K, GPUQ_REGS, kw, h);
+    if (active) {
+      make_key(K, GPUQ_REGS, kw, h);
+      if (state_key) kw[0] = pack_state_key(K, GPUQ_REGS);
+    }
     bool head = true;
     if (combine) {
       const int pa = __shfl_up((int)active, 1);
       const u64 ph = __shfl_up(h, 1);
       bool eq = (pa != 0) & (lane > 0) & (ph == h);
 #pragma unroll
-      for (int q = 0; q < MAX_KW; ++q) { const u64 pk = __shfl_up(kw[q], 1); if (q < T.key_words) eq = eq & (pk == kw[q]); }
+      for (int q = 0; q < MAX_KW; ++q) { const u64 pk = __shfl_up(kw[q], 1); if (q < cmp_words) eq = eq & (pk == kw[q]); }
       head = !(active & eq);
     }
     const int nh = __shfl_down((int)head, 1);
@@ -188,7 +238,7 @@
     u64 s = ~0ull;
     if (tail) {
       bool inserted;
-      s = ht_find_or_insert(T, kw, h, 0u, inserted);
+      s = state_key ? ht_state_find_or_insert(T, kw[0], h) : ht_find_or_insert(T, kw, h, 0u, inserted);
       if (s == ~0ull) atomicOr(P.flags, FLAG_TABLE_FULL);
     }
     u64* cells = T.slots + (s == ~0ull ? 0 : s) * (u64)T.slot_words + cell0;
@@ -226,7 +276,7 @@
 
 #ifndef GPUQ_JIT
 __global__ void __launch_bounds__(HBLOCK) k_agg_hash_extract(const KeySpec K, const AggSpec A, const HashTable T, const AggOut out,
-                                                             uint32_t* __restrict__ flags) {
+                                                             uint32_t* __restrict__ flags, const AggSoA soa) {
   constexpr int XSUB = 16;
   const int cell0 = 1 + T.key_words;
   const u64 chunk_slots = 64ull * XSUB;
@@ -254,7 +304,7 @@
         const u64 s = c * chunk_slots + (u64)j * 64 + hlane();
         const u64* slot = T.slots + s * (u64)T.slot_words;
         const uint32_t g = base + (uint32_t)__popcll(m & ltmask);
-        if (g < (uint32_t)out.cap) emit_group(slot, cell0, K, A, out, g);
+        if (g < (uint32_t)out.cap) { if (K.state_key) emit_state_group(slot, K, A, soa, g); else emit_group(slot, cell0, K, A, out, g); }
       }
       base += (uint32_t)__popcll(m);
     }
@@ -1304,11 +1354,12 @@
     hipLaunchKernelGGL(k_fsum_stage_reduce, dim3((unsigned)(need < cap ? (need ? need : 1) : cap)), dim3(HBLOCK), 0, s, T, A, (const u64*)fstage, n_fsum, (uint32_t)grid);
   }
 }
-void launch_agg_hash_extract(hipStream_t s, const KeySpec& K, const AggSpec& A, const HashTable& T, const AggOut& out, uint32_t* flags) {
+void launch_agg_hash_extract(hipStream_t s, const KeySpec& K, const AggSpec& A, const HashTable& T, const AggOut& out, uint32_t* flags, const AggSoA* soa) {
+  AggSoA none{};
   u64 need = (T.n_slots + (u64)HBLOCK * 16 - 1) / ((u64)HBLOCK * 16);
   const u64 cap = (u64)num_cus() * 16;
   const int grid = (int)(need < cap ? (need ? need : 1) : cap);
-  hipLaunchKernelGGL(k_agg_hash_extract, dim3(grid), dim3(HBLOCK), 0, s, K, A, T, out, flags);
+  hipLaunchKernelGGL(k_agg_hash_extract, dim3(grid), dim3(HBLOCK), 0, s, K, A, T, out, flags, soa ? *soa : none);
 }
 void launch_agg_bucket_id(hipStream_t s, void* jit_fn, const DevProgram& P, i64 n, const KeySpec& K, u64 bucket_mask, u64* bid, uint32_t* ids) {
   if (n <= 0) return;
diff --git a/arrow-ballista_amd/csrc/plan_exec.cpp b/arrow-ballista_amd/csrc/plan_exec.cpp
--- a/arrow-ballista_amd/csrc/plan_exec.cpp
+++ b/arrow-ballista_amd/csrc/plan_exec.cpp
@@ -50,15 +50,24 @@
 }
 
 struct PCol { std::string name; Json type; bool nullable = true; gpuq_column c{}; };
+struct BuildRows;
 struct PTable {
   std::vector<PCol> cols; int64_t n = 0;
   std::vector<const uint32_t*> via; std::vector<int> sides; bool dense = false;
   std::vector<BufP> keep;
   int64_t record_cap = 0;
   const uint64_t* n_dev = nullptr; BufP n_keep;
+  std::shared_ptr<const BuildRows> by_build;
   bool is_view() const { return !via.empty(); }
   void own(const PTable& o) { keep.insert(keep.end(), o.keep.begin(), o.keep.end()); }
   void count_from(const PTable& o) { n_dev = o.n_dev; n_keep = o.n_keep; }
+};
+
+struct BuildRows {
+  const uint32_t* rows = nullptr; BufP rows_keep;
+  PTable build;
+  std::vector<std::string> build_keys, probe_keys;
+  size_t n_build_cols = 0, n_cols = 0;
 };
 
 Json table_fields(const PTable& t) {
@@ -459,6 +468,7 @@
 PTable materialize(Exec& x, const PTable& t, bool force = false);
 
 void prune_columns(PTable& t, const std::set<std::string>& keep) {
+  t.by_build = nullptr;
   for (size_t i = t.cols.size(); i-- > 0;)
     if (!keep.count(t.cols[i].name)) { t.cols.erase(t.cols.begin() + (long)i); t.sides.erase(t.sides.begin() + (long)i); t.record_cap = 0; }
 }
@@ -725,6 +735,7 @@
   virtual ~PNode() {}
   virtual std::vector<PNode*> children() { return {}; }
   virtual int partitions() { auto c = children(); return c.empty() ? 1 : c[0]->partitions(); }
+  virtual bool is_hash_join() const { return false; }
   virtual PSchema schema() { auto c = children(); if (c.empty()) throw std::runtime_error("plan: node without a schema"); return c[0]->schema(); }
   virtual PTable execute(int part, Exec& x) = 0;
   typedef std::set<std::string> Names;
@@ -882,6 +893,10 @@
   return timed(x, t0, project(x, t, ex, names, this, 1));
 }
 
+bool is_bare_column(const Json& e, std::string& name) {
+  if (!(e.is_obj() && e.o.size() == 1 && e.o[0].first == "column" && e.o[0].second.is_obj() && e.o[0].second.find("name"))) return false;
+  name = e.o[0].second.at("name").str(); return true;
+}
 struct AggregateExec : PNode {
   PNodeP input; std::string mode, strategy = "auto"; Json group_expr, aggr_expr; int64_t expected_groups = 0, output_capacity = 0;
   std::vector<PNode*> children() override { return {input.get()}; }
@@ -911,6 +926,7 @@
     const bool final_ = mode == "Final" || mode == "FinalPartitioned";
     Fused f; if (final_) f.src = input.get(); else f = fuse(input.get());
     PTable t = f.src->execute(part, x);
+    if (final_ || !f.src->is_hash_join()) t.by_build = nullptr;
     auto t0 = std::chrono::steady_clock::now();
     bool many_string_keys = false;
     if (group_expr.a.size() > 4) {
@@ -928,12 +944,71 @@
     PTable t2 = filter_table(x, t, f.pred, this, 9);
     return timed(x, t0, run(x, t2, f2, true));
   }
+  const BuildRows* build_row_grouping(const PTable& t, const ColMap* cm, std::vector<Json>& over_build) const {
+    const BuildRows* br = t.by_build.get();
+    if (!br || mode != "Single" || group_expr.a.empty() || t.cols.size() != br->n_cols || br->build.cols.size() != br->n_build_cols) return nullptr;
+    auto first_named = [](const PTable& tt, const std::string& n) { for (size_t i = 0; i < tt.cols.size(); ++i) if (tt.cols[i].name == n) return (int)i; return -1; };
+    const size_t nkeys = br->build_keys.size();
+    std::vector<bool> got_build(nkeys, false), got_probe(nkeys, false);
+    for (auto& g : group_expr.a) {
+      const Json e = inline_projection(g.at("expr"), cm);
+      std::string bare; const bool is_bare = is_bare_column(e, bare);
+      if (is_bare) {
+        const int ci = first_named(t, bare);
+        if (ci < 0) return nullptr;
+        if ((size_t)ci >= br->n_build_cols) {
+          size_t k = 0; while (k < nkeys && br->probe_keys[k] != bare) ++k;
+          if (k == nkeys) return nullptr;
+          const int bi = first_named(br->build, br->build_keys[k]);
+          if (bi < 0 || first_named(t, br->build_keys[k]) != bi || br->build.cols[(size_t)bi].type.dump() != t.cols[(size_t)ci].type.dump()) return nullptr;
+          switch (t.cols[(size_t)ci].c.type) {
+            case T_INT8: case T_INT16: case T_INT32: case T_INT64: case T_UINT8: case T_UINT16: case T_UINT32: case T_UINT64: case T_DATE32: case T_DATE64: case T_TIMESTAMP: break;
+            default: return nullptr;
+          }
+          got_probe[k] = true;
+          over_build.push_back(jobj({{"column", jobj({{"name", jstr(br->build_keys[k])}})}}));
+          continue;
+        }
+        for (size_t k = 0; k < nkeys; ++k) if (br->build_keys[k] == bare) got_build[k] = true;
+      }
+      std::set<std::string> used; collect_columns(e, used);
+      for (auto& n : used) {
+        const int ci = first_named(t, n);
+        if (ci < 0 || (size_t)ci >= br->n_build_cols || first_named(br->build, n) != ci || t.cols[(size_t)ci].c.type == T_UTF8) return nullptr;
+      }
+      over_build.push_back(e);
+    }
+    const bool all_build = std::find(got_build.begin(), got_build.end(), false) == got_build.end();
+    const bool all_probe = std::find(got_probe.begin(), got_probe.end(), false) == got_probe.end();
+    return (all_build || all_probe) ? br : nullptr;
+  }
+  PTable with_group_columns(Exec& x, const PTable& out, const BuildRows& br, const std::vector<Json>& over_build) {
+    std::vector<std::string> names; for (auto& g : group_expr.a) names.push_back(g.at("name").str());
+    PTable v = select_view(x, br.build, (const uint32_t*)out.cols[0].c.data, out.n, nullptr, out.n_dev ? &out : nullptr);
+    v.own(out);
+    PTable keys = project(x, v, over_build, names, this, 11);
+    PTable r; r.n = keys.n; r.count_from(keys); r.own(keys); r.own(v);
+    r.cols = keys.cols; r.sides.assign(keys.cols.size(), 0);
+    for (size_t i = 1; i < out.cols.size(); ++i) { PCol c = out.cols[i]; c.c.length = keys.n; r.cols.push_back(c); r.sides.push_back(0); }
+    return r;
+  }
   PTable run(Exec& x, PTable t, const Fused& f, const bool long_keys) {
     const ColMap* cm0 = f.has_map ? &f.map : nullptr;
+    std::vector<Json> over_build;
+    const BuildRows* br = long_keys ? nullptr : build_row_grouping(t, cm0, over_build);
+    const std::shared_ptr<const BuildRows> br_keep = br ? t.by_build : nullptr;
+    if (br) {
+      PCol c; c.name = "__build_row"; c.type = jstr("UInt32"); c.nullable = false;
+      c.c.type = T_UINT32; c.c.repr = GPUQ_REPR_ARROW; c.c.data = br->rows; c.c.length = t.n;
+      t.cols.push_back(c); t.sides.push_back(0); t.keep.push_back(br->rows_keep); t.record_cap = 0; t.by_build = nullptr;
+    }
     std::vector<Json> gexprs; std::vector<int> coded;
     Utf8DictGuard dicts[8]; int nd = 0;
     const PTable t_src = t;
-    for (auto& g : group_expr.a) {
+    std::vector<std::string> gnames;
+    if (br) { gexprs.push_back(jobj({{"column", jobj({{"name", jstr("__build_row")}})}})); coded.push_back(-1); gnames.push_back("__build_row"); }
+    else for (auto& g : group_expr.a) {
+      gnames.push_back(g.at("name").str());
       Json e = inline_projection(g.at("expr"), cm0); int ci = -1;
       if (long_keys && (ci = long_key_column(t_src, e)) >= 0 && nd < 8) {
         const std::string nm = "__code_" + std::to_string(gexprs.size());
@@ -944,11 +1019,11 @@
       } else ci = -1;
       gexprs.push_back(e); coded.push_back(ci);
     }
-    gpuq_op* op = cached_op(x, this, long_keys ? 6 : 0, table_sig(t), [&]() {
+    gpuq_op* op = cached_op(x, this, long_keys ? 6 : (br ? 10 : 0), table_sig(t), [&]() {
     const auto nm = names_of(t);
     const ColMap* cm = f.has_map ? &f.map : nullptr;
     Json ge = jarr(), ae = jarr();
-    for (size_t k = 0; k < group_expr.a.size(); ++k) ge.a.push_back(jobj({{"expr", rebind(gexprs[k], nm)}, {"name", group_expr.a[k].at("name")}}));
+    for (size_t k = 0; k < gexprs.size(); ++k) ge.a.push_back(jobj({{"expr", rebind(gexprs[k], nm)}, {"name", jstr(gnames[k])}}));
     for (auto& a : aggr_expr.a) {
       std::vector<std::pair<std::string, Json>> o = {{"fn", a.at("fn")}, {"name", a.at("name")}};
       for (const char* k : {"expr", "expr2", "filter"}) if (a.has(k)) o.push_back({k, rebind(inline_projection(a.at(k), cm), nm)});
@@ -958,6 +1033,7 @@
                                                    {"strategy", jstr(strategy)}, {"group_expr", ge}, {"aggr_expr", ae}};
     if (f.has_pred) d.push_back({"predicate", rebind(f.pred, nm)});
     if (expected_groups) d.push_back({"expected_groups", jnum(expected_groups)});
+    if (br) d.push_back({"group_by", jstr("build_row")});
     return jobj(d);
     });
     const bool deferred = !long_keys && prep(x, op, t);
@@ -976,6 +1052,7 @@
         HIPCHECK(hipMemcpyAsync(cnt->p, ndev, 8, hipMemcpyDeviceToDevice, (hipStream_t)x.stream));
         out.n_dev = (const uint64_t*)cnt->p; out.n_keep = cnt;
       }
+      if (br) { out.own(t); return with_group_columns(x, out, *br, over_build); }
       return out;
     }
     for (;;) {
@@ -996,6 +1073,7 @@
         sc.name = out.cols[k].name; out.cols[k] = sc; out.record_cap = 0;
         HIPCHECK(hipStreamSynchronize((hipStream_t)x.stream));
       }
+      if (br) return with_group_columns(x, out, *br, over_build);
       return out;
     }
   }
@@ -1024,6 +1102,7 @@
 struct HashJoinExec : PNode {
   PNodeP left, right; Json on; std::string join_type = "Inner", partition_mode = "CollectLeft"; bool null_equals_null = false; bool has_filter = false; Json filter;
   std::vector<PNode*> children() override { return {left.get(), right.get()}; }
+  bool is_hash_join() const override { return true; }
   bool out_need_all = true; Names out_need;
   void require(const Names* need) override {
     out_need_all = need == nullptr; if (need) out_need = *need;
@@ -1053,10 +1132,13 @@
     return s;
   }
   int64_t last_pairs = -1;
-  PTable join_view(Exec& x, const PTable& lt, const PTable& rt, const uint32_t* ob, const uint32_t* opb, int64_t k, const BufP& ob_own, const BufP& opb_own, const PTable* count = nullptr) {
+  PTable join_view(Exec& x, const PTable& lt, const PTable& rt, const uint32_t* ob, const uint32_t* opb, int64_t k, const BufP& ob_own, const BufP& opb_own, const PTable* count = nullptr,
+                   bool* materialised = nullptr) {
     PTable lv = select_view(x, lt, ob, k, ob_own, count), rv = select_view(x, rt, opb, k, opb_own, count);
+    if (materialised) *materialised = false;
     if (lv.via.size() + rv.via.size() > 3) {
       if (lv.via.size() >= rv.via.size()) lv = materialize(x, lv); else rv = materialize(x, rv);
+      if (materialised) *materialised = true;
     }
     PTable out; out.n = k; out.own(lv); out.own(rv);
     if (count) out.count_from(*count);
@@ -1065,6 +1147,17 @@
     for (size_t i = 0; i < rv.cols.size(); ++i) { out.cols.push_back(rv.cols[i]); out.sides.push_back(rv.sides[i] == 0 ? 0 : rv.sides[i] + shift); }
     for (auto v : rv.via) out.via.push_back(v);
     return out;
+  }
+  void mark_build_rows(PTable& out, const PTable& lt, const uint32_t* ob, const BufP& ob_own) const {
+    auto m = std::make_shared<BuildRows>();
+    for (auto& o : on.a) {
+      std::string l, r;
+      if (!is_plain_column(o.at("left"), l) || !is_plain_column(o.at("right"), r)) return;
+      m->build_keys.push_back(l); m->probe_keys.push_back(r);
+    }
+    m->rows = ob; m->rows_keep = ob_own; m->build = lt; m->build.by_build = nullptr;
+    m->n_build_cols = lt.cols.size(); m->n_cols = out.cols.size();
+    out.by_build = m;
   }
   int64_t marked_rows(Exec& x, const uint32_t* rows, int64_t k, int64_t n, bool want_marked, int tag, BufP& out) {
     const size_t nb = (size_t)((n + 63) / 64) * 8 + 8;
@@ -1278,6 +1371,7 @@
       return jobj(pd);
     });
     const bool plain = !long_keys && !residual && !has_filter && (jt == "Inner" || jt == "Right" || jt == "RightSemi" || jt == "RightAnti");
+    const bool by_rows = join_type == "Inner" && !has_filter && !long_keys && !null_equals_null;
     bool deferred = false;
     if (chain) deferred = chain->deferred && plain && use_deferred(x, pop);
     else if (plain && x.deferred && last_pairs >= 0 && gpuq_op_can_defer(bop)) deferred = use_deferred(x, bop) && use_deferred(x, pop);
@@ -1301,7 +1395,10 @@
       check(x, gpuq_join_probe_run(pop, x.stream, jtab, &ric.in, 0, pairs ? (uint32_t*)ob->p : nullptr, (uint32_t*)opb->p, (uint64_t)cap, (uint64_t*)cnt->p));
       PTable c; c.n_dev = (const uint64_t*)cnt->p; c.n_keep = cnt;
       if (!pairs) return select_view(x, R.t, (const uint32_t*)opb->p, cap, opb, &c);
-      return join_view(x, L.t, R.t, (const uint32_t*)ob->p, (const uint32_t*)opb->p, cap, ob, opb, &c);
+      bool mat = false;
+      PTable out = join_view(x, L.t, R.t, (const uint32_t*)ob->p, (const uint32_t*)opb->p, cap, ob, opb, &c, &mat);
+      if (by_rows && !mat && !gpuq_join_table_has_duplicates(jtab)) mark_build_rows(out, L.t, (const uint32_t*)ob->p, ob);
+      return out;
     }
     for (;;) {
       ob = dev_alloc((size_t)cap * 4 + 16); opb = dev_alloc((size_t)cap * 4 + 16);
@@ -1328,7 +1425,9 @@
       k += mrows;
     }
     if (jt == "RightSemi" || jt == "RightAnti") return select_view(x, R.t, (const uint32_t*)opb->p, k, opb);
-    PTable out = join_view(x, L.t, R.t, (const uint32_t*)ob->p, (const uint32_t*)opb->p, k, ob, opb);
+    bool mat = false;
+    PTable out = join_view(x, L.t, R.t, (const uint32_t*)ob->p, (const uint32_t*)opb->p, k, ob, opb, nullptr, &mat);
+    if (by_rows && !mat && !gpuq_join_table_has_duplicates(jtab)) mark_build_rows(out, L.t, (const uint32_t*)ob->p, ob);
     if (residual) return residual_join(x, L.t, R.t, out, ob, opb, k);
     if (has_filter) out = filter_table(x, out, filter, this, 2);
     return out;
@@ -1425,6 +1524,7 @@
 }
 
 PTable slice_table(Exec& x, PTable t, int64_t skip, int64_t count) {
+  t.by_build = nullptr;
   resolve(x, t);
   skip = std::min(std::max<int64_t>(skip, 0), t.n);
   count = (count < 0 || skip + count > t.n) ? t.n - skip : count;
```

Result: faster. 169.1 billion rows/s (median of 6 runs) (+3.9%).
